# changhaonan/A3VLM

Measured on AMD Instinct MI355X. Metric: image-text samples/sec (train) + articulation-decode tok/s, higher is better.
Workload: dtype bf16

## Files before the change

### a3vlm_amd/csrc/a3v_attn_bwd.hip

```cpp
#include "a3v_common.h"
#include <type_traits>

namespace {

struct BwdArgs {
  const bf16_t* q; const bf16_t* k; const bf16_t* v; const bf16_t* dout;
  const float* lse; const float* D;
  bf16_t* dq; bf16_t* dk; bf16_t* dv;
  bf16_t* dqkv; int64_t ld_qkv; const float* cos_sin; int rope_pos0;
  int64_t k_sb, k_sh, v_sb, v_ss, v_sh;
  int B, S, Sp, H, Hkv, causal;
  float scale;
  int group_q, group_kv;
#ifdef AB_STAMP
  unsigned long long* stamps;
#endif
};
#ifdef AB_STAMP
#define AB_ST(kern, it, k) do { if (stamps && (it) < 64) stamps[((kern) * 64 + (it)) * 8 + (k)] = __builtin_amdgcn_s_memtime(); } while (0)
#else
#define AB_ST(kern, it, k) do {} while (0)
#endif

template <int HD>
__device__ __forceinline__ int tile_swz(int row) {
  return (HD == 128) ? (((row & 3) << 2) | ((row >> 2) & 3)) : ((row >> 1) & 7);
}

__device__ __forceinline__ void buf_dma16(__amdgpu_buffer_rsrc_t rs, char* lds_dst, unsigned voff) {
  __builtin_amdgcn_raw_ptr_buffer_load_lds(rs, (__attribute__((address_space(3))) void*)lds_dst, 16, voff, 0, 0, 0);
}
__device__ __forceinline__ void buf_dma4(__amdgpu_buffer_rsrc_t rs, void* lds_dst, unsigned voff) {
  __builtin_amdgcn_raw_ptr_buffer_load_lds(rs, (__attribute__((address_space(3))) void*)lds_dst, 4, voff, 0, 0, 0);
}
template <int HD>
__device__ __forceinline__ unsigned dma_lane_offset0(int64_t row_stride, int tid) {
  constexpr int KCH = HD / 8;
  const int row = tid / KCH, pc = tid % KCH;
  return (unsigned)((row * row_stride + ((pc ^ tile_swz<HD>(row)) << 3)) * 2);
}
template <int HD>
__device__ __forceinline__ unsigned dma_step(int64_t row_stride) { return (unsigned)((256 / (HD / 8)) * row_stride * 2); }
template <int HD>
__device__ __forceinline__ void stage_rows_dma(const bf16_t* base, int64_t row_stride, int row0, int nrows, char* lds, unsigned voff0, int wave) {
  const int64_t left = ((int64_t)(nrows - 1 - row0) * row_stride + HD) * 2;
  const auto rs = __builtin_amdgcn_make_buffer_rsrc((void*)(base + (int64_t)row0 * row_stride), 0, (int)(left < 0x7fffffff ? left : 0x7fffffff), 0x00020000);
  const unsigned step = dma_step<HD>(row_stride);
#pragma unroll
  for (int i = 0; i < 64 * (HD / 8) / 256; ++i) buf_dma16(rs, lds + (wave * 64 + i * 256) * 16, voff0 + i * step);
}

template <int HD>
__device__ __forceinline__ int frag_rows_base(int ql, int hh) { return ql * (HD * 2) + ((hh ^ tile_swz<HD>(ql)) << 4); }
template <int HD>
__device__ __forceinline__ bf16x8 frag_rows(const char* lds, int fbase, int tb, int ks) {
  return *reinterpret_cast<const bf16x8*>(lds + tb * 32 * (HD * 2) + (fbase ^ (ks << 5)));
}

typedef __attribute__((ext_vector_type(4))) short s16x4_t;
struct TrBase { int lo, hi; };
template <int HD>
__device__ __forceinline__ TrBase tr_bases(int lane) {
  const int hh = lane >> 5, ql = lane & 31, i = lane & 15;
  const int chunk16 = 2 * (ql >> 4) + ((i & 3) >> 1);
  const int row0 = 4 * hh + (i >> 2), row1 = row0 + 8;
  TrBase b;
  b.lo = row0 * (HD * 2) + ((chunk16 ^ tile_swz<HD>(row0)) << 4) + (i & 1) * 8;
  b.hi = row1 * (HD * 2) + ((chunk16 ^ tile_swz<HD>(row1)) << 4) + (i & 1) * 8;
  return b;
}
template <int HD>
__device__ __forceinline__ bf16x8 frag_rows_tr(const char* lds, TrBase tb0, int db, int tb, int c) {
  const char* blk = lds + (32 * tb + 16 * c) * (HD * 2);
  const s16x4_t lo = __builtin_amdgcn_ds_read_tr16_b64_v4i16((s16x4_t __attribute__((address_space(3)))*)(blk + (tb0.lo ^ (db << 6))));
  const s16x4_t hi = __builtin_amdgcn_ds_read_tr16_b64_v4i16((s16x4_t __attribute__((address_space(3)))*)(blk + (tb0.hi ^ (db << 6))));
  bf16x8 f;
  const short v[8] = {lo[0], lo[1], lo[2], lo[3], hi[0], hi[1], hi[2], hi[3]};
  __builtin_memcpy(&f, v, 16);
  return f;
}

template <int HD>
__device__ __forceinline__ void store_patch_rows(const char* patch, bf16_t* base, int64_t ld, int row0, int nrows, int lane) {
  constexpr int ROWB = HD * 2, NPAIR = HD / 8, RPI = 64 / NPAIR;
  asm volatile("s_waitcnt lgkmcnt(0)" ::: "memory");
  const int pr = lane % NPAIR, rr = lane / NPAIR;
#pragma unroll
  for (int it = 0; it < 32 / RPI; ++it) {
    const int r = it * RPI + rr;
    const bf16x8 v = *reinterpret_cast<const bf16x8*>(patch + r * ROWB + ((pr ^ (r & (NPAIR - 1))) << 4));
    if (row0 + r < nrows) *reinterpret_cast<bf16x8*>(base + (int64_t)(row0 + r) * ld + pr * 8) = v;
  }
}

template <int HD, bool PACKED>
__device__ __forceinline__ void store_grad_rows(const BwdArgs& p, f32x16 (&acc)[HD / 32], bf16_t* plain, int64_t prow, int slot, int pos,
                                                bool rotate, int hh) {
  if constexpr (!PACKED) {
    bf16_t* O = plain;
#pragma unroll
    for (int d = 0; d < HD / 32; ++d)
#pragma unroll
      for (int g4 = 0; g4 < 4; ++g4) {
        bf16x4 ov;
#pragma unroll
        for (int e = 0; e < 4; ++e) ov[e] = f2bf(acc[d][g4 * 4 + e]);
        *reinterpret_cast<bf16x4*>(O + d * 32 + g4 * 8 + hh * 4) = ov;
      }
    return;
  }
  bf16_t* O = p.dqkv + prow * p.ld_qkv + (int64_t)slot * HD;
  const float* CS = p.cos_sin + (int64_t)pos * HD;
#pragma unroll
  for (int d = 0; d < HD / 32; ++d)
#pragma unroll
    for (int g4 = 0; g4 < 4; ++g4) {
      const int dc = d * 32 + g4 * 8 + hh * 4;
      float v0 = acc[d][g4 * 4 + 0], v1 = acc[d][g4 * 4 + 1], v2 = acc[d][g4 * 4 + 2], v3 = acc[d][g4 * 4 + 3];
      if (rotate) {
        const f32x4 cs = *reinterpret_cast<const f32x4*>(CS + dc);
        const float a0 = v0 * cs[0] + v1 * cs[1], a1 = -v0 * cs[1] + v1 * cs[0];
        const float a2 = v2 * cs[2] + v3 * cs[3], a3 = -v2 * cs[3] + v3 * cs[2];
        v0 = a0; v1 = a1; v2 = a2; v3 = a3;
      }
      bf16x4 ov;
      ov[0] = f2bf(v0); ov[1] = f2bf(v1); ov[2] = f2bf(v2); ov[3] = f2bf(v3);
      *reinterpret_cast<bf16x4*>(O + dc) = ov;
    }
}

__device__ __forceinline__ void xcd_head_tile(int nt, int& head_slot, int& t, int G = 1) {
  const int total = gridDim.x, id = blockIdx.x;
  const int xcd = id & 7, q = total >> 3, r = total & 7;
  const int vb = (xcd < r ? xcd * (q + 1) : r * (q + 1) + (xcd - r) * q) + (id >> 3);
  if (G > 1) {
    const int per = G * nt, grp = vb / per, rr = vb - grp * per;
    head_slot = grp * G + rr % G;
    t = rr / G;
    return;
  }
  head_slot = vb / nt;
  t = vb - head_slot * nt;
}

template <int HD, bool PACKED>
__global__ __launch_bounds__(256, 2) void attn_bwd_dq_kernel(BwdArgs p) {
  constexpr int TILE = 64 * HD * 2;
  __shared__ __attribute__((aligned(1024))) char lds[4 * TILE];
  const int tid = threadIdx.x, lane = tid & 63, wave = __builtin_amdgcn_readfirstlane(tid >> 6);
  const int nqt = (p.S + 127) / 128;
  int head_slot, ti;
  xcd_head_tile(nqt, head_slot, ti, p.group_q);
  const int qt = nqt - 1 - ti, b = head_slot / p.H, h = head_slot - b * p.H;
  const int hk = h / (p.H / p.Hkv);
  const int ql = lane & 31, hh = lane >> 5;
  const int qrow = qt * 128 + wave * 32 + ql;
  const int qc = qrow < p.S ? qrow : p.S - 1;
  const bf16_t* Q = p.q + (((int64_t)b * p.S + qc) * p.H + h) * HD;
  const bf16_t* DO = p.dout + (((int64_t)b * p.S + qc) * p.H + h) * HD;
  const bf16_t* K = p.k + b * p.k_sb + hk * p.k_sh;
  const bf16_t* V = p.v + b * p.v_sb + hk * p.v_sh;
  bf16x8 qf[HD / 16], dof[HD / 16];
#pragma unroll
  for (int ks = 0; ks < HD / 16; ++ks) {
    qf[ks] = *reinterpret_cast<const bf16x8*>(Q + ks * 16 + hh * 8);
    dof[ks] = *reinterpret_cast<const bf16x8*>(DO + ks * 16 + hh * 8);
  }
  const float lse2 = p.lse[((int64_t)b * p.H + h) * p.S + qc] * 1.4426950408889634f;
  const float sl2 = p.scale * 1.4426950408889634f;
// ... 189 lines not shown
#pragma unroll
        for (int r = 0; r < 16; ++r) { s[r] = 0.f; dp[r] = 0.f; }
#pragma unroll
        for (int ks = 0; ks < HD / 16; ++ks) {
          s = __builtin_amdgcn_mfma_f32_32x32x16_bf16(frag_rows<HD>(Qs, fbase, tb, ks), kf[ks], s, 0, 0, 0);
          if (WHICH == 1) dp = __builtin_amdgcn_mfma_f32_32x32x16_bf16(frag_rows<HD>(T1, fbase, tb, ks), vf[ks], dp, 0, 0, 0);
        }
#pragma unroll
        for (int g4 = 0; g4 < 4; ++g4) {
          const int qb = tb * 32 + 8 * g4 + 4 * hh;
          f32x4 l4 = *reinterpret_cast<const f32x4*>(lse_s + qb);
#pragma unroll
          for (int e = 0; e < 4; ++e) l4[e] *= 1.4426950408889634f;
          f32x4 d4 = {0.f, 0.f, 0.f, 0.f};
          if (WHICH == 1) d4 = *reinterpret_cast<const f32x4*>(D_s + qb);
          if (interior) {
#pragma unroll
            for (int e = 0; e < 4; ++e) {
              const int r = g4 * 4 + e;
              const float pr = __builtin_amdgcn_exp2f(fmaf(s[r], sl2, -l4[e]));
              bf[tb][r >> 3][r & 7] = WHICH == 0 ? f2bf(pr) : f2bf(pr * (dp[r] - d4[e]));
            }
          } else {
#pragma unroll
            for (int e = 0; e < 4; ++e) {
              const int r = g4 * 4 + e;
              const int qg = q0 + qb + e;
              const bool ok = (qg < p.S) && (kvrow < p.S) && (!p.causal || kvrow <= qg);
              const float ev = __builtin_amdgcn_exp2f(fmaf(s[r], sl2, -l4[e]));
              const float val = WHICH == 0 ? ev : ev * (dp[r] - d4[e]);
              bf[tb][r >> 3][r & 7] = f2bf(ok ? val : 0.f);
            }
          }
        }
      }
      AB_ST(1 + WHICH, it, 4);
      const char* At = WHICH == 0 ? T1 : Qs;
#pragma unroll
      for (int tb = 0; tb < 2; ++tb)
#pragma unroll
        for (int c = 0; c < 2; ++c)
#pragma unroll
          for (int d = 0; d < HD / 32; ++d)
            acc[d] = __builtin_amdgcn_mfma_f32_32x32x16_bf16(frag_rows_tr<HD>(At, trb, d, tb, c), bf[tb][c], acc[d], 0, 0, 0);
      AB_ST(1 + WHICH, it, 5);
    }
  };
  {
    int it = 0;
    for (; it + 1 < total; it += 2) {
      body(it, std::integral_constant<int, 0>{});
      body(it + 1, std::integral_constant<int, 1>{});
    }
    if (it < total) body(it, std::integral_constant<int, 0>{});
  }
  if (WHICH == 1) {
#pragma unroll
    for (int d = 0; d < HD / 32; ++d)
#pragma unroll
      for (int r = 0; r < 16; ++r) acc[d][r] *= p.scale;
  }
  if (kvrow < p.S) {
    if constexpr (!PACKED) {
      bf16_t* O = (WHICH == 0 ? p.dv : p.dk) + (((int64_t)b * p.Hkv + hk) * p.S + kvrow) * HD;
#pragma unroll
      for (int d = 0; d < HD / 32; ++d)
#pragma unroll
        for (int g4 = 0; g4 < 4; ++g4) {
          bf16x4 a;
#pragma unroll
          for (int e = 0; e < 4; ++e) a[e] = f2bf(acc[d][g4 * 4 + e]);
          *reinterpret_cast<bf16x4*>(O + d * 32 + g4 * 8 + hh * 4) = a;
        }
    }
  }
  if constexpr (PACKED) {
    __syncthreads();
    char* patch = lds + wave * (32 * HD * 2);
    char* wrow = patch + kl * (HD * 2);
    const int wx = (kl & (HD / 8 - 1)) << 1;
    const float* CS = p.cos_sin + (int64_t)(p.rope_pos0 + kc) * HD;
#pragma unroll
    for (int d = 0; d < HD / 32; ++d)
#pragma unroll
      for (int g4 = 0; g4 < 4; ++g4) {
        const int dc = d * 32 + g4 * 8 + hh * 4;
        float v0 = acc[d][g4 * 4 + 0], v1 = acc[d][g4 * 4 + 1], v2 = acc[d][g4 * 4 + 2], v3 = acc[d][g4 * 4 + 3];
        if (WHICH == 1) {
          const f32x4 cs = *reinterpret_cast<const f32x4*>(CS + dc);
          const float a0 = v0 * cs[0] + v1 * cs[1], a1 = -v0 * cs[1] + v1 * cs[0];
          const float a2 = v2 * cs[2] + v3 * cs[3], a3 = -v2 * cs[3] + v3 * cs[2];
          v0 = a0; v1 = a1; v2 = a2; v3 = a3;
        }
        bf16x4 ov;
        ov[0] = f2bf(v0); ov[1] = f2bf(v1); ov[2] = f2bf(v2); ov[3] = f2bf(v3);
        *reinterpret_cast<bf16x4*>(wrow + (((d * 8 + g4 * 2 + hh) ^ wx) << 3)) = ov;
      }
    store_patch_rows<HD>(patch, p.dqkv + (int64_t)b * p.S * p.ld_qkv + (int64_t)(WHICH == 0 ? p.H + p.Hkv + hk : p.H + hk) * HD, p.ld_qkv,
                         kt_ * 128 + wave * 32, p.S, lane);
  }
}

template <int I, int N, typename F>
__device__ __forceinline__ void sfor(F&& f) {
  if constexpr (I < N) { f(std::integral_constant<int, I>{}); sfor<I + 1, N>(f); }
}
#define A3V_A16(b) "a" #b
#define A3V_CL8(p) "a" #p "0", "a" #p "1", "a" #p "2", "a" #p "3", "a" #p "4", "a" #p "5", "a" #p "6", "a" #p "7", "a" #p "8", "a" #p "9"
#define A3V_AGPR_0_255 "a0", "a1", "a2", "a3", "a4", "a5", "a6", "a7", "a8", "a9", A3V_CL8(1), A3V_CL8(2), A3V_CL8(3), A3V_CL8(4), A3V_CL8(5), A3V_CL8(6), \
    A3V_CL8(7), A3V_CL8(8), A3V_CL8(9), A3V_CL8(10), A3V_CL8(11), A3V_CL8(12), A3V_CL8(13), A3V_CL8(14), A3V_CL8(15), A3V_CL8(16), A3V_CL8(17), \
    A3V_CL8(18), A3V_CL8(19), A3V_CL8(20), A3V_CL8(21), A3V_CL8(22), A3V_CL8(23), A3V_CL8(24), "a250", "a251", "a252", "a253", "a254", "a255"
template <int ACC>
__device__ __forceinline__ void mfma_vv(const bf16x8& a, const bf16x8& b) {
  asm volatile("s_nop 1\n\tv_mfma_f32_32x32x16_bf16 a[%c2:%c3], %0, %1, a[%c2:%c3]" ::"v"(a), "v"(b), "i"(ACC), "i"(ACC + 15) : A3V_AGPR_0_255);
}
template <int ACC, int BR, bool ZERO>
__device__ __forceinline__ void mfma_va(const bf16x8& a) {
  if constexpr (ZERO)
    asm volatile("v_mfma_f32_32x32x16_bf16 a[%c1:%c2], %0, a[%c3:%c4], 0" ::"v"(a), "i"(ACC), "i"(ACC + 15), "i"(BR), "i"(BR + 3) : A3V_AGPR_0_255);
  else
    asm volatile("v_mfma_f32_32x32x16_bf16 a[%c1:%c2], %0, a[%c3:%c4], a[%c1:%c2]" ::"v"(a), "i"(ACC), "i"(ACC + 15), "i"(BR), "i"(BR + 3) : A3V_AGPR_0_255);
}
template <int BR, bool ZERO>
__device__ __forceinline__ void mfma_va_v(f32x16& acc, const bf16x8& a) {
  if constexpr (ZERO)
    asm volatile("v_mfma_f32_32x32x16_bf16 %0, %1, a[%c2:%c3], 0" : "=&v"(acc) : "v"(a), "i"(BR), "i"(BR + 3) : A3V_AGPR_0_255);
  else
    asm volatile("v_mfma_f32_32x32x16_bf16 %0, %1, a[%c2:%c3], %0" : "+v"(acc) : "v"(a), "i"(BR), "i"(BR + 3) : A3V_AGPR_0_255);
}
template <int R>
__device__ __forceinline__ float agpr_read() {
  float v;
  asm volatile("v_accvgpr_read_b32 %0, a[%c1]" : "=v"(v) : "i"(R) : A3V_AGPR_0_255);
  return v;
}
template <int R>
__device__ __forceinline__ void agpr_write(unsigned v) {
  asm volatile("v_accvgpr_write_b32 a[%c1], %0" ::"v"(v), "i"(R) : A3V_AGPR_0_255);
}
template <int R0>
__device__ __forceinline__ f32x16 agpr_read16() {
  f32x16 v;
  sfor<0, 16>([&](auto i) { v[decltype(i)::value] = agpr_read<R0 + decltype(i)::value>(); });
  return v;
}

typedef __attribute__((ext_vector_type(4))) int i32x4_t;
__device__ __forceinline__ void dma16_asm(i32x4_t rs, unsigned lds_addr, unsigned voff) {
  asm volatile("s_nop 4\n\ts_mov_b32 m0, %0\n\ts_nop 0\n\tbuffer_load_dwordx4 %1, %2, 0 offen lds" ::"s"(lds_addr), "v"(voff), "s"(rs) : "memory", A3V_AGPR_0_255);
}
__device__ __forceinline__ void dma4_asm(i32x4_t rs, unsigned lds_addr, unsigned voff) {
  asm volatile("s_nop 4\n\ts_mov_b32 m0, %0\n\ts_nop 0\n\tbuffer_load_dword %1, %2, 0 offen lds" ::"s"(lds_addr), "v"(voff), "s"(rs) : "memory", A3V_AGPR_0_255);
}
__device__ __forceinline__ i32x4_t make_rsrc(const void* base, int bytes) {
  const uint64_t a = (uint64_t)base;
  i32x4_t r;
  r[0] = __builtin_amdgcn_readfirstlane((int)(unsigned)a);
  r[1] = __builtin_amdgcn_readfirstlane((int)(unsigned)(a >> 32) & 0xffff);
  r[2] = __builtin_amdgcn_readfirstlane(bytes);
  r[3] = 0x00020000;
  return r;
}
template <int HD>
__device__ __forceinline__ void stage_rows_dma_asm(const bf16_t* base, int64_t row_stride, int row0, int nrows, unsigned lds_addr, unsigned voff0, int wave) {
  int64_t left = ((int64_t)(nrows - 1 - row0) * row_stride + HD) * 2;
  if (left < 0) left = 0;
  const i32x4_t rs = make_rsrc(base + (int64_t)(left ? row0 : 0) * row_stride, (int)(left < 0x7fffffff ? left : 0x7fffffff));
  const unsigned step = dma_step<HD>(row_stride);
#pragma unroll
  for (int i = 0; i < 64 * (HD / 8) / 256; ++i) dma16_asm(rs, lds_addr + (wave * 64 + i * 256) * 16, voff0 + i * step);
}
typedef __attribute__((ext_vector_type(8))) short s16x8_t;
template <int HD>
__device__ __forceinline__ bf16x8 frag_rows_tr2(const char* lds, TrBase tb0, int db, int tb, int c) {
  const char* blk = lds + (32 * tb + 16 * c) * (HD * 2);
  const s16x4_t lo = __builtin_amdgcn_ds_read_tr16_b64_v4i16((s16x4_t __attribute__((address_space(3)))*)(blk + (tb0.lo ^ (db << 6))));
  const s16x4_t hi = __builtin_amdgcn_ds_read_tr16_b64_v4i16((s16x4_t __attribute__((address_space(3)))*)(blk + (tb0.hi ^ (db << 6))));
  const s16x8_t v = __builtin_shufflevector(lo, hi, 0, 1, 2, 3, 4, 5, 6, 7);
  return __builtin_bit_cast(bf16x8, v);
}

template <int HD, bool PACKED>
__global__ __launch_bounds__(256, 1) void attn_bwd_dkv2_kernel(BwdArgs p) {
  constexpr int TILE = 64 * HD * 2;
  constexpr int BUFB = 2 * TILE + 1024;
  constexpr int NKS = HD / 16, NDB = HD / 32;
  constexpr int RV = 0, RK = 64, RKF = 128, RVF = 160, RS = 192, RDP = 208;
  constexpr int NB = 4;
  __shared__ __attribute__((aligned(1024))) char lds[NB * BUFB + 4096];
  const int tid = threadIdx.x, lane = tid & 63, wave = __builtin_amdgcn_readfirstlane(tid >> 6);
#ifdef AB_STAMP
  unsigned long long* tl = (p.stamps && tid == 0) ? p.stamps + 4096 + 8 * blockIdx.x : nullptr;
  if (tl) { tl[0] = __builtin_amdgcn_s_memrealtime(); tl[4] = __builtin_amdgcn_s_getreg(0x0004 | (0 << 6) | (31 << 11)); tl[5] = __builtin_amdgcn_s_getreg(20 | (0 << 6) | (31 << 11)); }
#endif
  int head_slot, kt_;
  xcd_head_tile((p.S + 127) / 128, head_slot, kt_, p.group_kv);
  const int b = head_slot / p.Hkv, hk = head_slot - b * p.Hkv;
  const int nrep = p.H / p.Hkv;
  const int kl = lane & 31, hh = lane >> 5;
  const int kv_lo = kt_ * 128 + wave * 32;
  const int kvrow = kv_lo + kl;
  const int kc = kvrow < p.S ? kvrow : p.S - 1;
  asm volatile("" ::: A3V_AGPR_0_255);
  const float sl2 = p.scale * 1.4426950408889634f;
  const int q_begin = p.causal ? kt_ * 2 : 0;
  const int n_qt = (p.S + 63) / 64;
  const int n_it = n_qt - q_begin, total = nrep * n_it;
  const unsigned qoff = dma_lane_offset0<HD>((int64_t)p.H * HD, tid);
  const int fbase = frag_rows_base<HD>(kl, hh);
  const TrBase trb = tr_bases<HD>(lane);

  int rep_n = 0, qi_n = 0, buf_n = 0;
  const unsigned lds0 = (unsigned)(size_t)((__attribute__((address_space(3))) char*)lds);
  constexpr int PP = HD / 16;
  i32x4_t rsQ, rsO, rsX;
  unsigned dmaQ, dmaO, dmaX, dma_step_i, voffX;
  const unsigned qstep = dma_step<HD>((int64_t)p.H * HD);
  const int64_t rstride = (int64_t)p.H * HD;
  const uint64_t pairB = (uint64_t)(64 * rstride * 2);
  uint64_t aQ = (uint64_t)(p.q + ((int64_t)b * p.S * p.H + hk * nrep) * HD + (int64_t)q_begin * 64 * rstride);
  uint64_t aO = (uint64_t)(p.dout + ((int64_t)b * p.S * p.H + hk * nrep) * HD + (int64_t)q_begin * 64 * rstride);
  uint64_t aL = (uint64_t)(p.lse + ((int64_t)b * p.H + hk * nrep) * p.S + q_begin * 64);
  uint64_t aD = (uint64_t)(p.D + ((int64_t)b * p.S + q_begin * 64) * p.H + hk * nrep);
  int64_t leftQ = ((int64_t)(p.S - 1 - q_begin * 64) * rstride + HD) * 2;
  int rowsL = p.S - q_begin * 64;
  voffX = (wave == 1) ? lane * p.H * 4 : lane * 4;
  auto mk = [&](uint64_t a, int bytes) __attribute__((always_inline)) {
    i32x4_t r;
    r[0] = (int)(unsigned)a; r[1] = (int)(unsigned)(a >> 32) & 0xffff; r[2] = bytes; r[3] = 0x00020000;
    return r;
  };
  auto prep_issue = [&](bool real) __attribute__((always_inline)) {
    const unsigned buf = lds0 + buf_n * BUFB, patch = lds0 + NB * BUFB + wave * 1024;
    const int nb = real ? (int)(leftQ < 0x7fffffff ? leftQ : 0x7fffffff) : 0;
    rsQ = mk(aQ, nb);
    rsO = mk(aO, nb);
    dmaQ = real ? buf + wave * 1024 : patch;
    dmaO = real ? buf + TILE + wave * 1024 : patch;
    dma_step_i = real ? 4096u : 0u;
    if (wave == 0) { rsX = mk(aL, real ? rowsL * 4 : 0); dmaX = real ? buf + 2 * TILE : patch; }
    else if (wave == 1) { rsX = mk(aD, real ? ((rowsL - 1) * p.H + 1) * 4 : 0); dmaX = real ? buf + 2 * TILE + 256 : patch; }
    else { rsX = mk(aL, 0); dmaX = patch; }
    if (real) {
      if (++buf_n == NB) buf_n = 0;
      if (++qi_n == n_it) {
        qi_n = 0; ++rep_n;
        const int64_t back = (int64_t)(n_it - 1) * 64;
        aQ += (uint64_t)(HD * 2) - (uint64_t)(back * rstride * 2); aO += (uint64_t)(HD * 2) - (uint64_t)(back * rstride * 2);
        aL += (uint64_t)((int64_t)p.S * 4) - (uint64_t)(back * 4); aD += 4 - (uint64_t)(back * p.H * 4);
        leftQ += back * rstride * 2; rowsL += (int)back;
      } else {
        aQ += pairB; aO += pairB; aL += 256; aD += (uint64_t)(64 * p.H * 4);
        leftQ -= (int64_t)pairB; rowsL -= 64;
      }
    }
  };
  auto piece = [&](auto i_) __attribute__((always_inline)) {
    constexpr int i = decltype(i_)::value;
    if constexpr (i < PP / 2) dma16_asm(rsQ, dmaQ + i * dma_step_i, qoff + i * qstep);
    else if constexpr (i < PP) dma16_asm(rsO, dmaO + (i - PP / 2) * dma_step_i, qoff + (i - PP / 2) * qstep);
    else dma4_asm(rsX, dmaX, voffX);
  };
  auto issue = [&](bool real) __attribute__((always_inline)) {
    prep_issue(real);
    sfor<0, PP + 1>([&](auto i_) { piece(i_); });
  };

  bf16x8 qa[NKS], da[NKS];
  auto fetch = [&](const char* buf, int tb) __attribute__((always_inline)) {
#pragma unroll
    for (int ks = 0; ks < NKS; ++ks) {
      qa[ks] = frag_rows<HD>(buf, fbase, tb, ks);
      da[ks] = frag_rows<HD>(buf + TILE, fbase, tb, ks);
    }
  };
  auto dead = [&](int qr0) { return qr0 >= p.S || (p.causal && qr0 + 31 < kv_lo); };
  auto interior = [&](int qr0) { return qr0 + 32 <= p.S && kv_lo + 31 < p.S && (!p.causal || qr0 >= kv_lo + 31); };

#ifdef AB_STAMP
  unsigned long long* stamps = (p.stamps && blockIdx.x == AB_STAMP && tid == 0) ? p.stamps : nullptr;
  int cur_it = 0;
#endif
  f32x16 dpv[2];
  auto step = [&](auto DA_, auto DBC_, auto MASK_, auto TBC_, const char* cb, int qr0, const char* fb, int tbf) __attribute__((always_inline)) {
    constexpr bool DA = decltype(DA_)::value, DBC = decltype(DBC_)::value, MASK = decltype(MASK_)::value;
    constexpr int tbc = decltype(TBC_)::value;
    constexpr int RSC = RS + 16 * tbc, RSN = RS + 16 * (1 - tbc);
    constexpr int EPK = 16 / NKS;
    bf16x8 trO[2][NDB], trQ[2][NDB], bP[2], bS[2];
    f32x4 l4[4], d4[4];
    float ex[EPK], dd[EPK];
    const float* sm = reinterpret_cast<const float*>(cb + 2 * TILE) + tbc * 32 + 4 * hh;
    if constexpr (DBC) {
      l4[0] = *reinterpret_cast<const f32x4*>(sm);
      d4[0] = *reinterpret_cast<const f32x4*>(sm + 64);
    }
    auto finish = [&](auto kp_) __attribute__((always_inline)) {
      constexpr int kp = decltype(kp_)::value;
#pragma unroll
      for (int j = 0; j < EPK; ++j) {
        const int r = kp * EPK + j;
        bP[r >> 3][r & 7] = f2bf(ex[j]);
        bS[r >> 3][r & 7] = f2bf(ex[j] * dd[j]);
      }
      u32x4 wP, wS;
      __builtin_memcpy(&wP, &bP[(kp * EPK) >> 3], 16);
      __builtin_memcpy(&wS, &bS[(kp * EPK) >> 3], 16);
      constexpr int w0 = ((kp * EPK) & 7) / 2;
      if constexpr (EPK == 2) asm volatile("" : "+v"(wP[w0]), "+v"(wS[w0]));
      else asm volatile("" : "+v"(wP[w0]), "+v"(wP[w0 + 1]), "+v"(wS[w0]), "+v"(wS[w0 + 1]));
      __builtin_memcpy(&bP[(kp * EPK) >> 3], &wP, 16);
      __builtin_memcpy(&bS[(kp * EPK) >> 3], &wS, 16);
    };
    sfor<0, NKS>([&](auto ks_) {
      constexpr int ks = decltype(ks_)::value;
      if constexpr (DA) mfma_va<RSN, RKF + 4 * ks, ks == 0>(qa[ks]);
      if constexpr (tbc == 0) piece(ks_);
      float en[EPK], dn[EPK];
      if constexpr (DBC) {
        constexpr int g4 = (ks * EPK) >> 2;
        sfor<0, EPK>([&](auto j_) {
          constexpr int j = decltype(j_)::value, r = ks * EPK + j, e = r & 3;
          const float sv = agpr_read<RSC + r>();
          const float dv = dpv[tbc][r];
          float a = fmaf(sv, sl2, l4[g4][e]);
          if constexpr (MASK) {
            const int qg = qr0 + 8 * g4 + 4 * hh + e;
            const bool ok = (qg < p.S) && (kvrow < p.S) && (!p.causal || kvrow <= qg);
            a = ok ? a : -INFINITY;
          }
          en[j] = __builtin_amdgcn_exp2f(a);
          dn[j] = dv - d4[g4][e];
        });
        if constexpr (EPK == 2) asm volatile("" : "+v"(en[0]), "+v"(en[1]), "+v"(dn[0]), "+v"(dn[1]));
        else asm volatile("" : "+v"(en[0]), "+v"(en[1]), "+v"(en[2]), "+v"(en[3]), "+v"(dn[0]), "+v"(dn[1]), "+v"(dn[2]), "+v"(dn[3]));
      }
      if constexpr (DA) mfma_va_v<RVF + 4 * ks, ks == 0>(dpv[1 - tbc], da[ks]);
      if constexpr (DBC) {
        if constexpr (ks > 0) finish(std::integral_constant<int, ks - 1>{});
#pragma unroll
        for (int j = 0; j < EPK; ++j) { ex[j] = en[j]; dd[j] = dn[j]; }
        if constexpr (ks < NDB) {
          trO[0][ks] = frag_rows_tr2<HD>(cb + TILE, trb, ks, tbc, 0);
          trQ[0][ks] = frag_rows_tr2<HD>(cb, trb, ks, tbc, 0);
        }
        constexpr int gn = ((ks * EPK) >> 2) + 1;
        if constexpr (((ks * EPK) & 3) == 0 && gn < 4) {
          l4[gn] = *reinterpret_cast<const f32x4*>(sm + 8 * gn);
          d4[gn] = *reinterpret_cast<const f32x4*>(sm + 64 + 8 * gn);
        }
        asm volatile("" ::: "memory");
      }
    });
    if constexpr (tbc == 0) piece(std::integral_constant<int, PP>{});
    if constexpr (DBC) finish(std::integral_constant<int, NKS - 1>{});
    asm volatile("" ::: "memory");
#ifdef AB_STAMP
    if (stamps && cur_it < 64) stamps[(64 + cur_it) * 8 + 6 + tbc] = __builtin_amdgcn_s_memtime();
#endif
    constexpr int FPD = NKS / NDB;
    sfor<0, NDB>([&](auto d_) {
      constexpr int d = decltype(d_)::value;
      if constexpr (DBC) {
        mfma_vv<RV + 16 * d>(trO[0][d], bP[0]);
        trO[1][d] = frag_rows_tr2<HD>(cb + TILE, trb, d, tbc, 1);
      }
      qa[d * FPD] = frag_rows<HD>(fb, fbase, tbf, d * FPD);
      asm volatile("" ::: "memory");
      if constexpr (DBC) {
        mfma_vv<RK + 16 * d>(trQ[0][d], bS[0]);
        trQ[1][d] = frag_rows_tr2<HD>(cb, trb, d, tbc, 1);
      }
      da[d * FPD] = frag_rows<HD>(fb + TILE, fbase, tbf, d * FPD);
      asm volatile("" ::: "memory");
    });
    sfor<0, NDB>([&](auto d_) {
      constexpr int d = decltype(d_)::value;
      if constexpr (DBC) mfma_vv<RV + 16 * d>(trO[1][d], bP[1]);
#pragma unroll
      for (int ks = d * FPD + 1; ks < (d + 1) * FPD; ++ks) qa[ks] = frag_rows<HD>(fb, fbase, tbf, ks);
      asm volatile("" ::: "memory");
      if constexpr (DBC) mfma_vv<RK + 16 * d>(trQ[1][d], bS[1]);
#pragma unroll
      for (int ks = d * FPD + 1; ks < (d + 1) * FPD; ++ks) da[ks] = frag_rows<HD>(fb + TILE, fbase, tbf, ks);
      asm volatile("" ::: "memory");
    });
    if constexpr (DA && !DBC) asm volatile("s_nop 15\n\ts_nop 15" ::: "memory", A3V_AGPR_0_255);
  };
  using T_ = std::true_type; using F_ = std::false_type;
  auto run = [&](bool lc, bool ln, bool mk, auto tbc, const char* cb, int qr0, const char* fb, int tbf) __attribute__((always_inline)) {
    if (lc) {
      if (mk) step(T_{}, T_{}, T_{}, tbc, cb, qr0, fb, tbf);
      else step(T_{}, T_{}, F_{}, tbc, cb, qr0, fb, tbf);
    } else if (ln) {
      step(T_{}, F_{}, F_{}, tbc, cb, qr0, fb, tbf);
    } else {
      step(F_{}, F_{}, F_{}, tbc, cb, qr0, fb, tbf);
    }
  };

  auto prescale_lse = [&](const char* buf) __attribute__((always_inline)) {
    if (wave == 3) {
      float* sm = const_cast<float*>(reinterpret_cast<const float*>(buf + 2 * TILE));
      sm[lane] = -1.4426950408889634f * sm[lane];
    }
  };
#ifdef AB_STAMP
#define AB_PE(k) do { if (stamps) stamps[2 * 64 * 8 + (k)] = __builtin_amdgcn_s_memtime(); } while (0)
#else
#define AB_PE(k) do {} while (0)
#endif
  AB_PE(0);
#ifdef AB_STAMP
  if (tl) tl[6] = __builtin_amdgcn_s_memrealtime();
#endif
  issue(true);
#ifdef AB_STAMP
  if (tl) tl[7] = __builtin_amdgcn_s_memrealtime();
#endif
  {
    const bf16_t* Kb = p.k + b * p.k_sb + hk * p.k_sh;
    const bf16_t* Vb = p.v + b * p.v_sb + hk * p.v_sh;
    const unsigned kvoffK = dma_lane_offset0<HD>(HD, tid), kvoffV = dma_lane_offset0<HD>(p.v_ss, tid);
#pragma unroll
    for (int t = 0; t < 2; ++t) {
      stage_rows_dma_asm<HD>(Kb, HD, kt_ * 128 + 64 * t, p.S, lds0 + 2 * BUFB + t * TILE, kvoffK, wave);
      stage_rows_dma_asm<HD>(Vb, p.v_ss, kt_ * 128 + 64 * t, p.S, lds0 + 3 * BUFB + t * TILE, kvoffV, wave);
    }
    sfor<0, 128>([&](auto i) { agpr_write<decltype(i)::value>(0u); });
    asm volatile("s_waitcnt vmcnt(0)" ::: "memory", A3V_AGPR_0_255);
    __syncthreads();
    prescale_lse(lds);
    const char* Kt = lds + 2 * BUFB + (wave >> 1) * TILE;
    const char* Vt = lds + 3 * BUFB + (wave >> 1) * TILE;
    sfor<0, NKS>([&](auto ks_) {
      constexpr int ks = decltype(ks_)::value;
      const bf16x8 kq = frag_rows<HD>(Kt, fbase, wave & 1, ks), vq = frag_rows<HD>(Vt, fbase, wave & 1, ks);
      u32x4 ku, vu;
      __builtin_memcpy(&ku, &kq, 16);
      __builtin_memcpy(&vu, &vq, 16);
      sfor<0, 4>([&](auto j) {
        agpr_write<RKF + 4 * ks + decltype(j)::value>(ku[decltype(j)::value]);
        agpr_write<RVF + 4 * ks + decltype(j)::value>(vu[decltype(j)::value]);
      });
    });
    __syncthreads();
  }
  AB_PE(1);
  AB_PE(2);
  issue(total > 1);
  AB_PE(3);
  fetch(lds, 0);
  prep_issue(total > 2);
  sfor<0, NKS>([&](auto ks_) {
    constexpr int ks = decltype(ks_)::value;
    mfma_va<RS, RKF + 4 * ks, ks == 0>(qa[ks]);
    piece(ks_);
    mfma_va_v<RVF + 4 * ks, ks == 0>(dpv[0], da[ks]);
  });
  piece(std::integral_constant<int, PP>{});
  asm volatile("s_nop 15\n\ts_nop 15" ::: "memory", A3V_AGPR_0_255);
  fetch(lds, 1);
  AB_PE(4);
  int qi_c = 0, buf_c = 0;
#ifdef AB_STAMP
  if (tl) tl[1] = __builtin_amdgcn_s_memrealtime();
#endif
  for (int it = 0; it < total; ++it) {
    const int q0 = (q_begin + qi_c) * 64;
    if (++qi_c == n_it) qi_c = 0;
    const int q0x = (q_begin + qi_c) * 64;
    const char* cb = lds + buf_c * BUFB;
    if (++buf_c == NB) buf_c = 0;
    const char* xb = lds + buf_c * BUFB;
    const bool more = it + 1 < total;
#ifdef AB_STAMP
    cur_it = it;
#endif
    AB_ST(1, it, 0);
    if constexpr (PP == 8) asm volatile("s_waitcnt vmcnt(9)" ::: "memory", A3V_AGPR_0_255); else asm volatile("s_waitcnt vmcnt(5)" ::: "memory", A3V_AGPR_0_255);
    AB_ST(1, it, 1);
    __syncthreads();
    AB_ST(1, it, 2);
    prep_issue(it + 3 < total);
    if (more) prescale_lse(xb);
    AB_ST(1, it, 3);
    const bool l0 = !dead(q0), l1 = !dead(q0 + 32), lx = more && !dead(q0x);
    run(l0, l1, !interior(q0), std::integral_constant<int, 0>{}, cb, q0, xb, 0);
    AB_ST(1, it, 4);
    run(l1, lx, !interior(q0 + 32), std::integral_constant<int, 1>{}, cb, q0 + 32, xb, 1);
    AB_ST(1, it, 5);
  }
#ifdef AB_STAMP
  if (tl) tl[2] = __builtin_amdgcn_s_memrealtime();
#endif
  asm volatile("s_nop 15\n\ts_nop 15" ::: "memory", A3V_AGPR_0_255);
  AB_PE(5);
  const float* CS = PACKED ? p.cos_sin + (int64_t)(p.rope_pos0 + kc) * HD : nullptr;
  f32x4 cs[NDB][4];
  if constexpr (PACKED) {
#pragma unroll
    for (int d = 0; d < NDB; ++d)
#pragma unroll
      for (int g4 = 0; g4 < 4; ++g4) cs[d][g4] = *reinterpret_cast<const f32x4*>(CS + d * 32 + g4 * 8 + hh * 4);
  }
  __syncthreads();
  AB_PE(6);
  char* patchV = lds + wave * (32 * HD * 2);
  char* patchK = lds + 4 * (32 * HD * 2) + wave * (32 * HD * 2);
  const int wx = (kl & (HD / 8 - 1)) << 1;
  sfor<0, NDB>([&](auto d_) {
    constexpr int d = decltype(d_)::value;
    const f32x16 av = agpr_read16<RV + 16 * d>();
#pragma unroll
    for (int g4 = 0; g4 < 4; ++g4) {
      bf16x4 ov;
#pragma unroll
      for (int e = 0; e < 4; ++e) ov[e] = f2bf(av[g4 * 4 + e]);
      *reinterpret_cast<bf16x4*>(patchV + kl * (HD * 2) + (((d * 8 + g4 * 2 + hh) ^ wx) << 3)) = ov;
    }
  });
  bf16_t* baseV = PACKED ? p.dqkv + (int64_t)b * p.S * p.ld_qkv + (int64_t)(p.H + p.Hkv + hk) * HD : p.dv + ((int64_t)b * p.Hkv + hk) * p.S * HD;
  bf16_t* baseK = PACKED ? p.dqkv + (int64_t)b * p.S * p.ld_qkv + (int64_t)(p.H + hk) * HD : p.dk + ((int64_t)b * p.Hkv + hk) * p.S * HD;
  const int64_t ldo = PACKED ? p.ld_qkv : HD;
  store_patch_rows<HD>(patchV, baseV, ldo, kv_lo, p.S, lane);
  AB_PE(7);
  sfor<0, NDB>([&](auto d_) {
    constexpr int d = decltype(d_)::value;
    f32x16 ak = agpr_read16<RK + 16 * d>();
#pragma unroll
    for (int r = 0; r < 16; ++r) ak[r] *= p.scale;
#pragma unroll
    for (int g4 = 0; g4 < 4; ++g4) {
      float v0 = ak[g4 * 4 + 0], v1 = ak[g4 * 4 + 1], v2 = ak[g4 * 4 + 2], v3 = ak[g4 * 4 + 3];
      bf16x4 ok;
      if constexpr (PACKED) {
        const f32x4 c4 = cs[d][g4];
        ok[0] = f2bf(v0 * c4[0] + v1 * c4[1]); ok[1] = f2bf(-v0 * c4[1] + v1 * c4[0]);
        ok[2] = f2bf(v2 * c4[2] + v3 * c4[3]); ok[3] = f2bf(-v2 * c4[3] + v3 * c4[2]);
      } else {
        ok[0] = f2bf(v0); ok[1] = f2bf(v1); ok[2] = f2bf(v2); ok[3] = f2bf(v3);
      }
      *reinterpret_cast<bf16x4*>(patchK + kl * (HD * 2) + (((d * 8 + g4 * 2 + hh) ^ wx) << 3)) = ok;
    }
  });
  store_patch_rows<HD>(patchK, baseK, ldo, kv_lo, p.S, lane);
  AB_PE(8);
#ifdef AB_STAMP
  if (tl) { asm volatile("s_waitcnt vmcnt(0)" ::: "memory"); tl[3] = __builtin_amdgcn_s_memrealtime(); }
#endif
}

}

extern "C" int a3v_transpose(const void* src, int64_t ld_src, int64_t bs_src, void* dst, int64_t ld_dst, int64_t bs_dst,
                             int R, int C, int Rpad, int batch, int dtype, void* stream);

extern "C" int64_t a3v_attention_bwd_workspace_bytes(int B, int S, int H, int Hkv, int hd) {
  (void)B; (void)S; (void)H; (void)Hkv; (void)hd;
  return 256;
}

#ifdef AB_STAMP
static unsigned long long* g_ab_stamps = nullptr;
extern "C" void a3v_debug_set_bwd_stamps(void* ptr) { g_ab_stamps = (unsigned long long*)ptr; }
#endif
static int attention_bwd_mfma_impl(const void* q, const void* k, int64_t k_sb, int64_t k_sh, const void* v, int64_t v_sb,
                                   int64_t v_ss, int64_t v_sh, const void* dout, const float* lse, const float* D, void* dq,
                                   void* dk, void* dv, void* dqkv, int64_t ld_qkv, const float* cos_sin, int rope_pos0, int B, int S, int H,
                                   int Hkv, int hd, int causal, void* stream) {
  if (hd != 64 && hd != 128) return A3V_ERR_ARG;
  if ((k_sb % 8) || (k_sh % 8) || (v_sb % 8) || (v_ss % 8) || (v_sh % 8)) return A3V_ERR_SHAPE;
  hipStream_t st = (hipStream_t)stream;
  const int Sp = (S + 63) / 64 * 64;
  BwdArgs p;
  p.q = (const bf16_t*)q; p.k = (const bf16_t*)k; p.v = (const bf16_t*)v; p.dout = (const bf16_t*)dout;
  p.lse = lse; p.D = D;
  p.dq = (bf16_t*)dq; p.dk = (bf16_t*)dk; p.dv = (bf16_t*)dv;
  p.dqkv = (bf16_t*)dqkv; p.ld_qkv = ld_qkv; p.cos_sin = cos_sin; p.rope_pos0 = rope_pos0;
  p.k_sb = k_sb; p.k_sh = k_sh; p.v_sb = v_sb; p.v_ss = v_ss; p.v_sh = v_sh;
  p.B = B; p.S = S; p.Sp = Sp; p.H = H; p.Hkv = Hkv; p.causal = causal;
  p.scale = 1.0f / sqrtf((float)hd);
#ifdef AB_STAMP
  p.stamps = g_ab_stamps;
#endif
  dim3 gq(((S + 127) / 128) * H * B), gk(((S + 127) / 128) * Hkv * B);
  auto group_of = [&](int heads, unsigned blocks) {
    if (!causal || (blocks & 7) || (heads & 7)) return 1;
    const int ge = A3V_ENV_INT("A3V_ATTN_HEAD_GROUP", 0);
    int want = 16;
    while (want > 1 && (int64_t)want * S * hd * 4 > (9 << 19)) want >>= 1;
    if (ge > 0) want = ge;
    int G = want < 1 ? 1 : want;
    while (G > 1 && (heads / 8) % G) G >>= 1;
    return G;
  };
  p.group_q = group_of(B * H, gq.x);
  p.group_kv = group_of(B * Hkv, gk.x);
  const int v2 = A3V_ENV_INT("A3V_ATTN_BWD_V2", 1);
#define A3V_BWD_LAUNCH(HDV, PK)                                                                  \
  do {                                                                                           \
    hipLaunchKernelGGL((attn_bwd_dq_kernel<HDV, PK>), gq, dim3(256), 0, st, p);                  \
    if (v2 & 1) {                                                                                \
      hipLaunchKernelGGL((attn_bwd_dkv2_kernel<HDV, PK>), gk, dim3(256), 0, st, p);              \
    } else {                                                                                     \
      hipLaunchKernelGGL((attn_bwd_dkv_kernel<HDV, 0, PK>), gk, dim3(256), 0, st, p);            \
      hipLaunchKernelGGL((attn_bwd_dkv_kernel<HDV, 1, PK>), gk, dim3(256), 0, st, p);            \
    }                                                                                            \
  } while (0)
  if (hd == 128) {
    if (dqkv) A3V_BWD_LAUNCH(128, true); else A3V_BWD_LAUNCH(128, false);
  } else {
    if (dqkv) A3V_BWD_LAUNCH(64, true); else A3V_BWD_LAUNCH(64, false);
  }
#undef A3V_BWD_LAUNCH
  A3V_LAUNCH_CHECK();
  return A3V_OK;
}

extern "C" int a3v_attention_bwd_mfma(const void* q, const void* k, int64_t k_sb, int64_t k_sh, const void* v, int64_t v_sb,
                                      int64_t v_ss, int64_t v_sh, const void* dout, const float* lse, const float* D, void* dq,
                                      void* dk, void* dv, void* workspace, int B, int S, int H, int Hkv, int hd, int causal,
                                      void* stream) {
  if (!workspace || !dq || !dk || !dv) return A3V_ERR_ARG;
  return attention_bwd_mfma_impl(q, k, k_sb, k_sh, v, v_sb, v_ss, v_sh, dout, lse, D, dq, dk, dv, nullptr, 0, nullptr, 0, B, S, H, Hkv, hd,
                                 causal, stream);
}

extern "C" __attribute__((visibility("hidden"))) int a3v_attention_bwd_mfma_packed(const void* q, const void* k, int64_t k_sb, int64_t k_sh, const void* v, int64_t v_sb,
                                             int64_t v_ss, int64_t v_sh, const void* dout, const float* lse, const float* D, void* dqkv,
                                             int64_t ld_qkv, const float* cos_sin, int rope_pos0, int B, int S, int H, int Hkv, int hd,
                                             int causal, void* stream) {
  if (!dqkv || !cos_sin || ld_qkv % 4 || rope_pos0 < 0) return A3V_ERR_ARG;
  return attention_bwd_mfma_impl(q, k, k_sb, k_sh, v, v_sb, v_ss, v_sh, dout, lse, D, nullptr, nullptr, nullptr, dqkv, ld_qkv, cos_sin, rope_pos0,
                                 B, S, H, Hkv, hd, causal, stream);
}
```

### a3vlm_amd/csrc/a3v_train.hip

```cpp
#include "a3v_common.h"

namespace {

template <typename T>
__global__ __launch_bounds__(256) void transpose_kernel(const T* __restrict__ src, int64_t lds_, int64_t bs_s,
                                                        T* __restrict__ dst, int64_t ldd, int64_t bs_d, int R, int C, int Rpad) {
  __shared__ T tile[64][64 + 2];
  const T* s = src + blockIdx.z * bs_s;
  T* d = dst + blockIdx.z * bs_d;
  const int r0 = blockIdx.y * 64, c0 = blockIdx.x * 64;
  const int tx = threadIdx.x & 63, ty = threadIdx.x >> 6;
  for (int i = ty; i < 64; i += 4) {
    const int r = r0 + i, c = c0 + tx;
    tile[i][tx] = (r < R && c < C) ? s[(int64_t)r * lds_ + c] : (T)0.f;
  }
  __syncthreads();
  for (int i = ty; i < 64; i += 4) {
    const int c = c0 + i, r = r0 + tx;
    if (c < C && r < Rpad) d[(int64_t)c * ldd + r] = tile[tx][i];
  }
}

__global__ __launch_bounds__(256) void transpose_bf16_vec_kernel(const bf16_t* __restrict__ src, int64_t lds_, int64_t bs_s,
                                                                 bf16_t* __restrict__ dst, int64_t ldd, int64_t bs_d, int R, int C, int Rpad,
// ... 701 lines not shown
    A3V_LAUNCH_CHECK();
    if (part) {
      hipLaunchKernelGGL(colsum_add_kernel, dim3((dim + 255) / 256, 16), dim3(256), 0, ST, dw_scratch, nb, dim, dw);
      A3V_LAUNCH_CHECK();
    }
    return A3V_OK;
  }
  constexpr int RPB = 16;
  dim3 g((rows + RPB - 1) / RPB);
  if (act_dtype == A3V_BF16) hipLaunchKernelGGL((rmsnorm_bwd_kernel<bf16_t, RPB, TS>), g, dim3(256), 0, ST, x, ldx, w, (const bf16_t*)dy, lddy, dh, lddh, dw, rows, dim, eps);
  else if (act_dtype == A3V_F32) hipLaunchKernelGGL((rmsnorm_bwd_kernel<float, RPB, TS>), g, dim3(256), 0, ST, x, ldx, w, (const float*)dy, lddy, dh, lddh, dw, rows, dim, eps);
  else return A3V_ERR_DTYPE;
  A3V_LAUNCH_CHECK();
  if (dh_bf) {
    if (sizeof(TS) != 4) return A3V_ERR_ARG;
    return a3v_cast(dh, lddh, A3V_F32, dh_bf, ld_bf, A3V_BF16, rows, dim, stream);
  }
  return A3V_OK;
}

extern "C" int a3v_rmsnorm_bwd(const float* x, int64_t ldx, const float* w, const void* dy, int64_t lddy, float* dh, int64_t lddh,
                               float* dw, float* dw_scratch, int rows, int dim, float eps, int act_dtype, void* stream) {
  return rmsnorm_bwd_impl<float>(x, ldx, w, dy, lddy, dh, lddh, dw, dw_scratch, rows, dim, eps, act_dtype, stream, nullptr, 0);
}

extern "C" int a3v_rmsnorm_bwd_cast(const float* x, int64_t ldx, const float* w, const void* dy, int64_t lddy, float* dh, int64_t lddh,
                                    float* dw, float* dw_scratch, int rows, int dim, float eps, int act_dtype, void* dh_bf16,
                                    int64_t ld_bf16, void* stream) {
  if (!dh_bf16 || (ld_bf16 & 3) || (reinterpret_cast<uintptr_t>(dh_bf16) & 7)) return A3V_ERR_ARG;
  return rmsnorm_bwd_impl<float>(x, ldx, w, dy, lddy, dh, lddh, dw, dw_scratch, rows, dim, eps, act_dtype, stream, (bf16_t*)dh_bf16, ld_bf16);
}

extern "C" int a3v_rmsnorm_bwd_bf16(const void* x, int64_t ldx, const float* w, const void* dy, int64_t lddy, void* dh, int64_t lddh,
                                    float* dw, float* dw_scratch, int rows, int dim, float eps, void* stream) {
  return rmsnorm_bwd_impl<bf16_t>((const bf16_t*)x, ldx, w, dy, lddy, (bf16_t*)dh, lddh, dw, dw_scratch, rows, dim, eps, A3V_BF16, stream, nullptr, 0);
}

static int layernorm_bwd_impl(const void* x, int64_t ldx, const float* w, const void* dy, int dy_dtype, int64_t lddy, const int32_t* row_map,
                              void* dx, int64_t lddx, float* dw, float* db, int rows, int dim, float eps, int act_dtype, void* stream) {
  if (!x || !w || !dy || !dx || !dw || !db || rows <= 0) return A3V_ERR_ARG;
  if (dim > 8192) return A3V_ERR_SHAPE;
  constexpr int RPB = 16;
  dim3 g((rows + RPB - 1) / RPB);
  if (dy_dtype == A3V_F32) {
    if (act_dtype == A3V_BF16) hipLaunchKernelGGL((layernorm_bwd_kernel<bf16_t, RPB, float>), g, dim3(256), 0, ST, (const bf16_t*)x, ldx, w, (const float*)dy, lddy, row_map, (bf16_t*)dx, lddx, dw, db, rows, dim, eps);
    else if (act_dtype == A3V_F32) hipLaunchKernelGGL((layernorm_bwd_kernel<float, RPB, float>), g, dim3(256), 0, ST, (const float*)x, ldx, w, (const float*)dy, lddy, row_map, (float*)dx, lddx, dw, db, rows, dim, eps);
    else return A3V_ERR_DTYPE;
  } else if (dy_dtype == A3V_BF16 && act_dtype == A3V_BF16) {
    hipLaunchKernelGGL((layernorm_bwd_kernel<bf16_t, RPB, bf16_t>), g, dim3(256), 0, ST, (const bf16_t*)x, ldx, w, (const bf16_t*)dy, lddy, row_map, (bf16_t*)dx, lddx, dw, db, rows, dim, eps);
  } else return A3V_ERR_DTYPE;
  A3V_LAUNCH_CHECK();
  return A3V_OK;
}

extern "C" int a3v_layernorm_bwd(const void* x, int64_t ldx, const float* w, const float* dy, int64_t lddy, const int32_t* row_map,
                                 void* dx, int64_t lddx, float* dw, float* db, int rows, int dim, float eps, int act_dtype, void* stream) {
  return layernorm_bwd_impl(x, ldx, w, dy, A3V_F32, lddy, row_map, dx, lddx, dw, db, rows, dim, eps, act_dtype, stream);
}

extern "C" int a3v_layernorm_bwd_bf16(const void* x, int64_t ldx, const float* w, const void* dy, int64_t lddy, const int32_t* row_map,
                                      void* dx, int64_t lddx, float* dw, float* db, int rows, int dim, float eps, void* stream) {
  return layernorm_bwd_impl(x, ldx, w, dy, A3V_BF16, lddy, row_map, dx, lddx, dw, db, rows, dim, eps, A3V_BF16, stream);
}

static int stream_nt() {
  return A3V_ENV_INT("A3V_STREAM_NT", 3) & 3;
}

extern "C" int a3v_swiglu_fwd(const void* gu, int64_t ldg, void* act, int64_t lda, int rows, int F, int interleaved, int dtype, void* stream) {
  const int inter = interleaved;
  if (!gu || !act || rows <= 0 || F <= 0 || (F % 16)) return A3V_ERR_ARG;
  if ((ldg % 8) || (lda % 8)) return A3V_ERR_SHAPE;
  int64_t n = (int64_t)rows * (F / 8);
  int blocks = (int)((n + 255) / 256 > 16384 ? 16384 : (n + 255) / 256);
  const int nt = stream_nt();
  if (dtype == A3V_BF16 && nt == 3) hipLaunchKernelGGL((swiglu_fwd_kernel<bf16_t, 3>), dim3(blocks), dim3(256), 0, ST, (const bf16_t*)gu, ldg, (bf16_t*)act, lda, rows, F, inter);
  else if (dtype == A3V_BF16 && nt == 1) hipLaunchKernelGGL((swiglu_fwd_kernel<bf16_t, 1>), dim3(blocks), dim3(256), 0, ST, (const bf16_t*)gu, ldg, (bf16_t*)act, lda, rows, F, inter);
  else if (dtype == A3V_BF16) hipLaunchKernelGGL(swiglu_fwd_kernel<bf16_t>, dim3(blocks), dim3(256), 0, ST, (const bf16_t*)gu, ldg, (bf16_t*)act, lda, rows, F, inter);
  else if (dtype == A3V_F32) hipLaunchKernelGGL(swiglu_fwd_kernel<float>, dim3(blocks), dim3(256), 0, ST, (const float*)gu, ldg, (float*)act, lda, rows, F, inter);
  else return A3V_ERR_DTYPE;
  A3V_LAUNCH_CHECK();
  return A3V_OK;
}

extern "C" int a3v_swiglu_bwd(const void* gu, int64_t ldg, const void* dact, int64_t lda, void* dgu, int64_t lddg, int rows, int F,
                              int interleaved, int dtype, void* stream) {
  const int inter = interleaved;
  if (!gu || !dact || !dgu || rows <= 0 || F <= 0 || (F % 16)) return A3V_ERR_ARG;
  if ((ldg % 8) || (lda % 8) || (lddg % 8)) return A3V_ERR_SHAPE;
  int64_t n = (int64_t)rows * (F / 8);
  int blocks = (int)((n + 255) / 256 > 16384 ? 16384 : (n + 255) / 256);
  const int nt = stream_nt();
  if (dtype == A3V_BF16 && nt == 3) hipLaunchKernelGGL((swiglu_bwd_kernel<bf16_t, 3>), dim3(blocks), dim3(256), 0, ST, (const bf16_t*)gu, ldg, (const bf16_t*)dact, lda, (bf16_t*)dgu, lddg, rows, F, inter);
  else if (dtype == A3V_BF16 && nt == 1) hipLaunchKernelGGL((swiglu_bwd_kernel<bf16_t, 1>), dim3(blocks), dim3(256), 0, ST, (const bf16_t*)gu, ldg, (const bf16_t*)dact, lda, (bf16_t*)dgu, lddg, rows, F, inter);
  else if (dtype == A3V_BF16) hipLaunchKernelGGL(swiglu_bwd_kernel<bf16_t>, dim3(blocks), dim3(256), 0, ST, (const bf16_t*)gu, ldg, (const bf16_t*)dact, lda, (bf16_t*)dgu, lddg, rows, F, inter);
  else if (dtype == A3V_F32) hipLaunchKernelGGL(swiglu_bwd_kernel<float>, dim3(blocks), dim3(256), 0, ST, (const float*)gu, ldg, (const float*)dact, lda, (float*)dgu, lddg, rows, F, inter);
  else return A3V_ERR_DTYPE;
  A3V_LAUNCH_CHECK();
  return A3V_OK;
}

extern "C" int a3v_rope_bwd_pack(const void* dq, const void* dk, const void* dv, void* dqkv, int64_t ld, const float* cos_sin,
                                 int B, int S, int H, int Hkv, int hd, int rope_pos0, int dtype, void* stream) {
  if (!dq || !dk || !dv || !dqkv || !cos_sin || B <= 0 || S <= 0 || (hd & 1)) return A3V_ERR_ARG;
  if (dtype == A3V_BF16) hipLaunchKernelGGL(rope_bwd_pack_kernel<bf16_t>, dim3(B * S), dim3(256), 0, ST, (const bf16_t*)dq, (const bf16_t*)dk, (const bf16_t*)dv, (bf16_t*)dqkv, ld, cos_sin, S, H, Hkv, hd, rope_pos0);
  else if (dtype == A3V_F32) hipLaunchKernelGGL(rope_bwd_pack_kernel<float>, dim3(B * S), dim3(256), 0, ST, (const float*)dq, (const float*)dk, (const float*)dv, (float*)dqkv, ld, cos_sin, S, H, Hkv, hd, rope_pos0);
  else return A3V_ERR_DTYPE;
  A3V_LAUNCH_CHECK();
  return A3V_OK;
}

extern "C" int a3v_attention_bwd_mfma(const void* q, const void* k, int64_t k_sb, int64_t k_sh, const void* v, int64_t v_sb,
                                      int64_t v_ss, int64_t v_sh, const void* dout, const float* lse, const float* D, void* dq,
                                      void* dk, void* dv, void* workspace, int B, int S, int H, int Hkv, int hd, int causal,
                                      void* stream);

extern "C" int a3v_attention_bwd(const void* q, const void* k, int64_t k_sb, int64_t k_sh, const void* v, int64_t v_sb, int64_t v_ss, int64_t v_sh,
                                 const void* out, const void* dout, const float* lse, float* D, void* dq, void* dk, void* dv,
                                 void* workspace, int B, int S, int H, int Hkv, int hd, int causal, int dtype, void* stream) {
  if (!q || !k || !v || !out || !dout || !lse || !D || !dq || !dk || !dv || B <= 0 || S <= 0) return A3V_ERR_ARG;
  if (hd > 256 || (H % Hkv)) return A3V_ERR_SHAPE;
  AttnBwdArgs p;
  p.q = q; p.k = k; p.v = v; p.dout = dout; p.lse = lse; p.D = D; p.dq = dq; p.dk = dk; p.dv = dv;
  p.v_sb = v_sb; p.v_ss = v_ss; p.v_sh = v_sh;
  p.k_sb = k_sb; p.k_sh = k_sh;
  p.B = B; p.S = S; p.H = H; p.Hkv = Hkv; p.hd = hd; p.causal = causal;
  p.scale = 1.0f / sqrtf((float)hd);
  if (dtype == A3V_BF16 && workspace && (hd == 64 || hd == 128)) {
    const int64_t rows = (int64_t)B * S * H;
    if (((reinterpret_cast<uintptr_t>(out) | reinterpret_cast<uintptr_t>(dout)) & 15) != 0)
      hipLaunchKernelGGL(attn_rowdot_kernel<bf16_t>, dim3(B * S * H), dim3(64), 0, ST, (const bf16_t*)out, (const bf16_t*)dout, D, hd);
    else if (hd == 128)
      hipLaunchKernelGGL(attn_rowdot_vec_kernel<128>, dim3((unsigned)((rows + 15) / 16)), dim3(256), 0, ST, (const bf16_t*)out, (const bf16_t*)dout, D, rows);
    else
      hipLaunchKernelGGL(attn_rowdot_vec_kernel<64>, dim3((unsigned)((rows + 31) / 32)), dim3(256), 0, ST, (const bf16_t*)out, (const bf16_t*)dout, D, rows);
    A3V_LAUNCH_CHECK();
    return a3v_attention_bwd_mfma(q, k, k_sb, k_sh, v, v_sb, v_ss, v_sh, dout, lse, D, dq, dk, dv, workspace, B, S, H, Hkv, hd, causal, stream);
  }
  if (dtype == A3V_BF16) {
    hipLaunchKernelGGL(attn_rowdot_kernel<bf16_t>, dim3(B * S * H), dim3(64), 0, ST, (const bf16_t*)out, (const bf16_t*)dout, D, hd);
    hipLaunchKernelGGL(attn_bwd_dq_generic<bf16_t>, dim3(S, H, B), dim3(64), 0, ST, p);
    hipLaunchKernelGGL(attn_bwd_dkv_generic<bf16_t>, dim3(S, Hkv, B), dim3(64), 0, ST, p);
  } else if (dtype == A3V_F32) {
    hipLaunchKernelGGL(attn_rowdot_kernel<float>, dim3(B * S * H), dim3(64), 0, ST, (const float*)out, (const float*)dout, D, hd);
    hipLaunchKernelGGL(attn_bwd_dq_generic<float>, dim3(S, H, B), dim3(64), 0, ST, p);
    hipLaunchKernelGGL(attn_bwd_dkv_generic<float>, dim3(S, Hkv, B), dim3(64), 0, ST, p);
  } else return A3V_ERR_DTYPE;
  A3V_LAUNCH_CHECK();
  return A3V_OK;
}

extern "C" __attribute__((visibility("hidden"))) int a3v_attention_bwd_mfma_packed(const void* q, const void* k, int64_t k_sb, int64_t k_sh, const void* v, int64_t v_sb,
                                             int64_t v_ss, int64_t v_sh, const void* dout, const float* lse, const float* D, void* dqkv,
                                             int64_t ld_qkv, const float* cos_sin, int rope_pos0, int B, int S, int H, int Hkv, int hd,
                                             int causal, void* stream);

extern "C" int a3v_attention_bwd_packed(const void* q, const void* k, int64_t k_sb, int64_t k_sh, const void* v, int64_t v_sb, int64_t v_ss,
                                        int64_t v_sh, const void* out, int64_t ld_out, const void* dout, const float* lse, float* D, void* dqkv,
                                        int64_t ld_qkv, const float* cos_sin, int rope_pos0, int B, int S, int H, int Hkv, int hd, int causal,
                                        int dtype, void* stream) {
  if (!q || !k || !v || !out || !dout || !lse || !D || !dqkv || !cos_sin || B <= 0 || S <= 0) return A3V_ERR_ARG;
  if (dtype != A3V_BF16) return A3V_ERR_DTYPE;
  if ((hd != 64 && hd != 128) || (H % Hkv) || ld_out < (int64_t)H * hd || ld_out % 8) return A3V_ERR_SHAPE;
  if (((reinterpret_cast<uintptr_t>(out) | reinterpret_cast<uintptr_t>(dout)) & 15) != 0) return A3V_ERR_SHAPE;
  const int64_t rows = (int64_t)B * S * H;
  if (hd == 128)
    hipLaunchKernelGGL(attn_rowdot_vec_kernel<128>, dim3((unsigned)((rows + 15) / 16)), dim3(256), 0, ST, (const bf16_t*)out, (const bf16_t*)dout, D, rows, H, ld_out);
  else
    hipLaunchKernelGGL(attn_rowdot_vec_kernel<64>, dim3((unsigned)((rows + 31) / 32)), dim3(256), 0, ST, (const bf16_t*)out, (const bf16_t*)dout, D, rows, H, ld_out);
  A3V_LAUNCH_CHECK();
  return a3v_attention_bwd_mfma_packed(q, k, k_sb, k_sh, v, v_sb, v_ss, v_sh, dout, lse, D, dqkv, ld_qkv, cos_sin, rope_pos0, B, S, H, Hkv, hd, causal,
                                       stream);
}

extern "C" int a3v_embed_bwd(const int64_t* tokens, int64_t ld_tok, const float* dh, float* dtable, int B, int T, int W, int dim,
                             int vocab, void* stream) {
  if (!tokens || !dh || !dtable || B <= 0 || T <= 0) return A3V_ERR_ARG;
  hipLaunchKernelGGL(embed_bwd_kernel<float>, dim3(B * (T + W)), dim3(256), 0, ST, tokens, ld_tok, dh, dtable, T, W, dim, vocab);
  A3V_LAUNCH_CHECK();
  return A3V_OK;
}

extern "C" int a3v_embed_bwd_bf16(const int64_t* tokens, int64_t ld_tok, const void* dh, float* dtable, int B, int T, int W, int dim,
                                  int vocab, void* stream) {
  if (!tokens || !dh || !dtable || B <= 0 || T <= 0) return A3V_ERR_ARG;
  hipLaunchKernelGGL(embed_bwd_kernel<bf16_t>, dim3(B * (T + W)), dim3(256), 0, ST, tokens, ld_tok, (const bf16_t*)dh, dtable, T, W, dim, vocab);
  A3V_LAUNCH_CHECK();
  return A3V_OK;
}

extern "C" int a3v_rows_sum(const void* src, int64_t ld, const int32_t* row_idx, int n_rows, int dim, float* out, int dtype, void* stream) {
  if (!src || !out || n_rows <= 0 || dim <= 0) return A3V_ERR_ARG;
  dim3 g((dim + 255) / 256, (n_rows + 63) / 64);
  if (dtype == A3V_BF16) hipLaunchKernelGGL(rows_sum_kernel<bf16_t>, g, dim3(256), 0, ST, (const bf16_t*)src, ld, row_idx, n_rows, dim, out);
  else if (dtype == A3V_F32) hipLaunchKernelGGL(rows_sum_kernel<float>, g, dim3(256), 0, ST, (const float*)src, ld, row_idx, n_rows, dim, out);
  else return A3V_ERR_DTYPE;
  A3V_LAUNCH_CHECK();
  return A3V_OK;
}

namespace {
template <int NT>
__global__ __launch_bounds__(256) void adamw_kernel(float* __restrict__ p, const float* __restrict__ g, float* __restrict__ m,
                                                    float* __restrict__ v, int64_t n4, int64_t n, float decay, float b1, float b2,
                                                    float step_size, float inv_bc2_sqrt, float eps, bf16_t* __restrict__ img,
                                                    const float* __restrict__ gscale) {
  const float gs = gscale ? *gscale : 1.f;
  if (!(gs >= 0.f)) return;
  const int64_t stride = (int64_t)gridDim.x * 256;
  for (int64_t i = (int64_t)blockIdx.x * 256 + threadIdx.x; i < n4; i += stride) {
    f32x4 pp = (NT & 1) ? __builtin_nontemporal_load(reinterpret_cast<const f32x4*>(p) + i) : reinterpret_cast<const f32x4*>(p)[i];
    f32x4 gg = (NT & 1) ? __builtin_nontemporal_load(reinterpret_cast<const f32x4*>(g) + i) : reinterpret_cast<const f32x4*>(g)[i];
#pragma unroll
    for (int e = 0; e < 4; ++e) gg[e] = __fmul_rn(gg[e], gs);
    f32x4 mm = (NT & 1) ? __builtin_nontemporal_load(reinterpret_cast<const f32x4*>(m) + i) : reinterpret_cast<const f32x4*>(m)[i];
    f32x4 vv = (NT & 1) ? __builtin_nontemporal_load(reinterpret_cast<const f32x4*>(v) + i) : reinterpret_cast<const f32x4*>(v)[i];
#pragma unroll
    for (int e = 0; e < 4; ++e) {
      pp[e] *= decay;
      mm[e] += (1.f - b1) * (gg[e] - mm[e]);
      vv[e] = b2 * vv[e] + (1.f - b2) * gg[e] * gg[e];
      pp[e] -= step_size * mm[e] / (sqrtf(vv[e]) * inv_bc2_sqrt + eps);
    }
    if (NT & 2) {
      __builtin_nontemporal_store(pp, reinterpret_cast<f32x4*>(p) + i);
      __builtin_nontemporal_store(mm, reinterpret_cast<f32x4*>(m) + i);
      __builtin_nontemporal_store(vv, reinterpret_cast<f32x4*>(v) + i);
    } else {
      reinterpret_cast<f32x4*>(p)[i] = pp;
      reinterpret_cast<f32x4*>(m)[i] = mm;
      reinterpret_cast<f32x4*>(v)[i] = vv;
    }
    if (img) {
      bf16x4 o;
#pragma unroll
      for (int e = 0; e < 4; ++e) o[e] = f2bf(pp[e]);
      if (NT & 2) __builtin_nontemporal_store(o, reinterpret_cast<bf16x4*>(img) + i);
      else reinterpret_cast<bf16x4*>(img)[i] = o;
    }
  }
  if (blockIdx.x == 0 && threadIdx.x < (int)(n - n4 * 4)) {
    const int64_t i = n4 * 4 + threadIdx.x;
    float pp = p[i] * decay;
    const float gg = __fmul_rn(g[i], gs);
    const float mm = m[i] + (1.f - b1) * (gg - m[i]);
    const float vv = b2 * v[i] + (1.f - b2) * gg * gg;
    pp -= step_size * mm / (sqrtf(vv) * inv_bc2_sqrt + eps);
    p[i] = pp; m[i] = mm; v[i] = vv;
    if (img) img[i] = f2bf(pp);
  }
}
}

extern "C" int a3v_adamw_scaled(float* param, const float* grad, float* exp_avg, float* exp_avg_sq, int64_t n, float lr, float beta1,
                                float beta2, float eps, float weight_decay, int64_t step, void* bf16_image, const float* grad_scale,
                                void* stream);
extern "C" int a3v_adamw(float* param, const float* grad, float* exp_avg, float* exp_avg_sq, int64_t n, float lr, float beta1,
                         float beta2, float eps, float weight_decay, int64_t step, void* bf16_image, void* stream) {
  return a3v_adamw_scaled(param, grad, exp_avg, exp_avg_sq, n, lr, beta1, beta2, eps, weight_decay, step, bf16_image, nullptr, stream);
}

extern "C" int a3v_adamw_scaled(float* param, const float* grad, float* exp_avg, float* exp_avg_sq, int64_t n, float lr, float beta1,
                                float beta2, float eps, float weight_decay, int64_t step, void* bf16_image, const float* grad_scale,
                                void* stream) {
  if (!param || !grad || !exp_avg || !exp_avg_sq || n <= 0 || step < 1) return A3V_ERR_ARG;
  if (((uintptr_t)param | (uintptr_t)grad | (uintptr_t)exp_avg | (uintptr_t)exp_avg_sq) & 15) return A3V_ERR_SHAPE;
  if (bf16_image && ((uintptr_t)bf16_image & 7)) return A3V_ERR_SHAPE;
  const double bc1 = 1.0 - pow((double)beta1, (double)step), bc2 = 1.0 - pow((double)beta2, (double)step);
  const float step_size = (float)((double)lr / bc1), inv_bc2_sqrt = (float)(1.0 / sqrt(bc2));
  const float decay = (float)(1.0 - (double)lr * (double)weight_decay);
  const int64_t n4 = n / 4;
  int64_t blocks = (n4 + 255) / 256;
  if (blocks > 256 * 16) blocks = 256 * 16;
  if (blocks < 1) blocks = 1;
  const int nt = A3V_ENV_INT("A3V_ADAMW_NT", 3);
#define A3V_ADAMW_LAUNCH(V) hipLaunchKernelGGL(adamw_kernel<V>, dim3((unsigned)blocks), dim3(256), 0, (hipStream_t)stream, param, grad, exp_avg, exp_avg_sq, n4, n, decay, \
                     beta1, beta2, step_size, inv_bc2_sqrt, eps, (bf16_t*)bf16_image, grad_scale)
  switch (nt & 3) {
    case 1: A3V_ADAMW_LAUNCH(1); break;
    case 2: A3V_ADAMW_LAUNCH(2); break;
    case 3: A3V_ADAMW_LAUNCH(3); break;
    default: A3V_ADAMW_LAUNCH(0); break;
  }
#undef A3V_ADAMW_LAUNCH
  A3V_LAUNCH_CHECK();
  return A3V_OK;
}

namespace {
template <int TR>
__global__ __launch_bounds__(256) void adamw_tile_t_kernel(float* __restrict__ p, const float* __restrict__ g, float* __restrict__ m,
                                                           float* __restrict__ v, int rows, int cols, float decay, float b1, float b2,
                                                           float step_size, float inv_bc2_sqrt, float eps, bf16_t* __restrict__ img,
                                                           bf16_t* __restrict__ imgt, int64_t ldt, const float* __restrict__ gscale) {
  const float gs = gscale ? *gscale : 1.f;
  if (!(gs >= 0.f)) return;
  constexpr int PITCH = TR + 2;
  __shared__ bf16_t patch2[2][64 * PITCH];
  int flip = 0;
  const int tid = threadIdx.x, tr = tid >> 4, tc = tid & 15;
  const int tiles_c = cols >> 6, ntiles = (rows / TR) * tiles_c;
  for (int t = blockIdx.x; t < ntiles; t += gridDim.x) {
    const int r0 = (t / tiles_c) * TR, c0 = (t % tiles_c) << 6;
    bf16_t* patch = patch2[flip];
    flip ^= 1;
#pragma unroll
    for (int ps = 0; ps < TR / 16; ++ps) {
      const int r = ps * 16 + tr;
      const int64_t i = ((int64_t)(r0 + r) * cols + c0 + tc * 4) >> 2;
      f32x4 pp = __builtin_nontemporal_load(reinterpret_cast<const f32x4*>(p) + i);
      f32x4 gg = __builtin_nontemporal_load(reinterpret_cast<const f32x4*>(g) + i);
#pragma unroll
      for (int e = 0; e < 4; ++e) gg[e] = __fmul_rn(gg[e], gs);
      f32x4 mm = __builtin_nontemporal_load(reinterpret_cast<const f32x4*>(m) + i);
      f32x4 vv = __builtin_nontemporal_load(reinterpret_cast<const f32x4*>(v) + i);
#pragma unroll
      for (int e = 0; e < 4; ++e) {
        pp[e] *= decay;
        mm[e] += (1.f - b1) * (gg[e] - mm[e]);
        vv[e] = b2 * vv[e] + (1.f - b2) * gg[e] * gg[e];
        pp[e] -= step_size * mm[e] / (sqrtf(vv[e]) * inv_bc2_sqrt + eps);
      }
      __builtin_nontemporal_store(pp, reinterpret_cast<f32x4*>(p) + i);
      __builtin_nontemporal_store(mm, reinterpret_cast<f32x4*>(m) + i);
      __builtin_nontemporal_store(vv, reinterpret_cast<f32x4*>(v) + i);
// ... 174 lines not shown
```

### a3vlm_amd/lib.py

```python
from __future__ import annotations

import ctypes
import os
from ctypes import c_float, c_int, c_int64, c_void_p

_HERE = os.path.dirname(os.path.abspath(__file__))
LIB_PATH = os.environ.get("A3V_LIB_PATH") or os.path.join(_HERE, "liba3vlm_hip.so")

BF16, F32 = 0, 1
EPI_NONE, EPI_BIAS, EPI_GELU, EPI_QUICKGELU, EPI_RESIDUAL, EPI_SWIGLU, EPI_OUT_F32, EPI_RES_F32 = 0, 1, 2, 4, 8, 16, 32, 64
EPI_SWIGLU_BWD = 128

EPI_TILE_128, EPI_TILE_256, EPI_TILE_256PP = 1 << 16, 1 << 17, 1 << 18
EPI_TILE_192PP = 1 << 23

P, I, L, F = c_void_p, c_int, c_int64, c_float

SIGNATURES = {
    "a3v_version": (I, []),
    "a3v_reload_env": (I, []),
    "a3v_gemm_nt": (I, [P, L, P, L, P, L, I, I, I, P, P, L, I, I, P]),
    "a3v_gemm_qkv_rope": (I, [P, L, P, L, I, P, L, P, P, P, L, P, L, P, I, I, I, I, I, I, I, I, P]),
    "a3v_gemm_nt_fp8": (I, [P, L, P, P, L, P, P, L, I, I, I, P, P, L, I, P]),
    "a3v_gemm_qkv_rope_fp8": (I, [P, L, P, P, L, P, I, P, L, P, P, P, I, I, I, I, I, I, I, I, P]),
    "a3v_quantize_rows_fp8": (I, [P, L, P, F, P, L, P, I, I, I, P]),
    "a3v_gemm_tn_splitk": (I, [P, L, P, L, P, I, I, I, I, P]),
    "a3v_attention_bwd_packed": (I, [P, P, L, L, P, L, L, L, P, L, P, P, P, P, L, P, I, I, I, I, I, I, I, I, P]),
    "a3v_lora_refresh": (I, [P, P, I, I, I, P, L, P, L, P, L, P, L, I, I, P]),
    "a3v_adamw": (I, [P, P, P, P, L, F, F, F, F, F, L, P, P]),
    "a3v_adamw_scaled": (I, [P, P, P, P, L, F, F, F, F, F, L, P, P, P]),
    "a3v_adamw_scaled_t": (I, [P, P, P, P, I, I, F, F, F, F, F, L, P, P, L, P, P]),
    "a3v_gemm_tn_strip": (I, [P, L, P, L, P, I, I, I, I, P]),
    "a3v_lora_gb_scatter": (I, [P, L, I, I, P, P, P, P]),
    "a3v_adamw_multi": (I, [P, I, L, F, F, F, F, F, L, P, P]),
    "a3v_scale_cast": (I, [P, I, P, I, L, F, P]),
    "a3v_sumsq_partials": (I, [P, L, P, P]),
    "a3v_grad_bucket_allreduce": (I, [P, P, L, P, I, P]),
    "a3v_grad_bucket_reduce_scatter": (I, [P, P, L, P, P, P, I, P]),
    "a3v_param_shard_all_gather": (I, [P, P, P, L, P]),
    "a3v_rccl_comm_count": (I, [P]),
    "a3v_rccl_available": (I, []),
    "a3v_gemm_nn": (I, [P, L, P, L, P, L, I, I, I, P, L, I, P]),
    "a3v_gemm_tn": (I, [P, L, P, L, P, L, I, I, I, P, L, I, P]),
    "a3v_gemm_tn_sumsq": (I, [P, L, P, L, P, L, I, I, I, P, L, I, P, L, P]),
    "a3v_gemm_tn_sumsq_slots": (L, [I, I]),
    "a3v_gemm_set_workspace": (I, [P, L]),
    "a3v_gemm_set_workspace_for": (I, [P, P, L]),
    "a3v_gemm_nt_splitk": (I, [P, L, P, L, P, I, I, I, I, P]),
    "a3v_splitk_reduce": (I, [P, I, I, I, P, L, I, I, P]),
    "a3v_gemm_skinny_split": (I, [I, I, I]),
    "a3v_gemm_skinny_ws_bytes": (L, [I, I, I]),
    "a3v_gemm_skinny_fp8": (I, [P, L, P, L, P, P, L, I, I, I, P, L, I, P, P]),
    "a3v_quantize_nf4_ws_bytes": (L, [I, I]),
    "a3v_quantize_nf4": (I, [P, I, I, P, P, P, P]),
    "a3v_dequantize_nf4": (I, [P, P, P, L, I, I, P]),
    "a3v_gemm_skinny_nf4": (I, [P, L, P, L, P, P, L, I, I, I, P, L, I, P, P]),
    "a3v_gemm_skinny": (I, [P, L, P, L, P, L, I, I, I, P, L, I, P, P]),
    "a3v_rmsnorm": (I, [P, L, P, P, L, I, I, F, I, I, I, P]),
    "a3v_layernorm": (I, [P, L, P, P, P, L, P, I, I, F, I, I, I, P]),
    "a3v_rope_kvcache": (I, [P, L, P, L, P, P, P, I, I, I, I, I, I, I, I, I, P]),
    "a3v_vt_pack": (I, [P, L, P, I, I, I, I, I, I, P]),
    "a3v_attention_scratch_floats": (L, [I, I, I, I]),
    "a3v_attention": (I, [P, P, P, P, I, I, I, I, I, I, ctypes.POINTER(c_int64), I, P, I, P]),
    "a3v_embed_assemble": (I, [P, L, P, P, I, I, I, I, I, I, I, P]),
    "a3v_fill_rows": (I, [P, P, L, P, I, I, I, I, P]),
    "a3v_patch_im2col": (I, [P, P, I, I, I, I, I, I, I, P]),
    "a3v_split_views": (I, [P, P, I, I, I, I, P]),
    "a3v_vit_embed": (I, [P, P, P, P, I, I, I, I, P]),
    "a3v_argmax": (I, [P, L, P, I, I, P]),
    "a3v_sample_top_p": (I, [P, L, I, I, F, F, P, P, P]),
    "a3v_preprocess_image": (I, [P, I, I, I, I, I, P, P, P, I, P, P, I, I, P, P, I, P, P, P]),
    "a3v_preprocess_batch": (I, [P, I, P, I, P, L, P, L, I, P, P, P]),
    "a3v_generate_step": (I, [P, L, P, I, I, P, L, P, L, I, P, P, I, P, P, P, P]),
    "a3v_count_valid": (I, [P, I, P, P]),
    "a3v_cross_entropy": (I, [P, L, P, P, P, L, P, F, I, I, I, P]),
    "a3v_attention_lse": (I, [P, P, P, P, P, I, I, I, I, I, I, ctypes.POINTER(c_int64), I, I, P]),
    "a3v_transpose": (I, [P, L, L, P, L, L, I, I, I, I, I, P]),
    "a3v_rmsnorm_bwd_scratch_floats": (L, [I, I]),
    "a3v_rmsnorm_bwd": (I, [P, L, P, P, L, P, L, P, P, I, I, F, I, P]),
    "a3v_rmsnorm_bwd_cast": (I, [P, L, P, P, L, P, L, P, P, I, I, F, I, P, L, P]),
    "a3v_rmsnorm_bwd_bf16": (I, [P, L, P, P, L, P, L, P, P, I, I, F, P]),
    "a3v_layernorm_bwd_bf16": (I, [P, L, P, P, L, P, P, L, P, P, I, I, F, P]),
    "a3v_embed_bwd_bf16": (I, [P, L, P, P, I, I, I, I, I, P]),
    "a3v_layernorm_bwd": (I, [P, L, P, P, L, P, P, L, P, P, I, I, F, I, P]),
    "a3v_swiglu_fwd": (I, [P, L, P, L, I, I, I, I, P]),
    "a3v_swiglu_bwd": (I, [P, L, P, L, P, L, I, I, I, I, P]),
    "a3v_cast": (I, [P, L, I, P, L, I, I, I, P]),
    "a3v_add2d": (I, [P, L, P, L, I, I, I, P]),
    "a3v_rope_bwd_pack": (I, [P, P, P, P, L, P, I, I, I, I, I, I, I, P]),
    "a3v_attention_bwd": (I, [P, P, L, L, P, L, L, L, P, P, P, P, P, P, P, P, I, I, I, I, I, I, I, P]),
    "a3v_attention_bwd_workspace_bytes": (L, [I, I, I, I, I]),
    "a3v_attention_bwd_mfma": (I, [P, P, L, L, P, L, L, L, P, P, P, P, P, P, P, I, I, I, I, I, I, P]),
    "a3v_embed_bwd": (I, [P, L, P, P, I, I, I, I, I, P]),
    "a3v_rows_sum": (I, [P, L, P, I, I, P, I, P]),
}

class LlamaLayer(ctypes.Structure):
    _fields_ = [(n, c_void_p) for n in ("attn_norm_w", "wqkv", "wo", "ffn_norm_w", "w13", "w2", "k_cache", "vt_cache",
                                        "wqkv_q", "wqkv_s", "wo_q", "wo_s", "w13_q", "w13_s", "w2_q", "w2_s",
                                        "wqkv_n4", "wqkv_n4s", "wo_n4", "wo_n4s", "w13_n4", "w13_n4s", "w2_n4", "w2_n4s")]


class ImageDesc(ctypes.Structure):
    _fields_ = [("src", c_void_p), ("coeffs", c_void_p), ("bounds", c_void_p), ("H", c_int), ("W", c_int), ("side", c_int), ("pad_x", c_int),
                ("pad_y", c_int), ("ksize", c_int)]


SIGNATURES["a3v_llama_decode_step"] = (I, [ctypes.POINTER(LlamaLayer), I, P, P, P, P, P, P, P, P, I, I, I, I, I, I, I, I, F, P])
SIGNATURES["a3v_llama_decode_step_form"] = (I, [I, I, I, I, I, I, I])

_lib = None


def load() -> ctypes.CDLL:
    global _lib
    if _lib is not None:
        return _lib
    if not os.path.isfile(LIB_PATH):
        raise RuntimeError(
            f"{LIB_PATH} not found: the HIP extension is not built. Run "
            "`python -c 'import __graft_entry__ as g; g.build()'` (or `make -C a3vlm_amd/csrc`). "
            "a3vlm_amd has no non-HIP fallback.")
    import torch
    lib = ctypes.CDLL(LIB_PATH)
    for name, (res, args) in SIGNATURES.items():
        fn = getattr(lib, name)
        fn.restype = res
        fn.argtypes = args
    _lib = lib
    return lib


class env:

    def __init__(self, **kw):
        self.kw = {k: str(v) for k, v in kw.items()}
        self.old = {}

    def __enter__(self):
        for k, v in self.kw.items():
            self.old[k] = os.environ.get(k)
            os.environ[k] = v
        load().a3v_reload_env()
        return self

    def __exit__(self, *exc):
        for k, v in self.old.items():
            if v is None:
                os.environ.pop(k, None)
            else:
                os.environ[k] = v
        load().a3v_reload_env()
        return False


class A3VError(RuntimeError):
    pass


_ERR = {-1: "A3V_ERR_SHAPE (unsupported size/alignment)", -2: "A3V_ERR_DTYPE", -3: "A3V_ERR_ARG"}


def check(rc: int, what: str) -> None:
    if rc != 0:
        raise A3VError(f"{what} failed: {_ERR.get(rc, f'hipError_t {rc}')}")
```

### a3vlm_amd/ops.py

```python
from __future__ import annotations

import ctypes
from typing import Optional

import torch

from . import lib as _l
from .lib import BF16, F32, EPI_BIAS, EPI_GELU, EPI_QUICKGELU, EPI_RESIDUAL, EPI_SWIGLU, EPI_OUT_F32, EPI_RES_F32, EPI_SWIGLU_BWD

_DT = {torch.bfloat16: BF16, torch.float32: F32}


def dt(t: torch.Tensor) -> int:
    try:
        return _DT[t.dtype]
    except KeyError:
        raise TypeError(f"a3vlm_amd supports bf16/fp32 tensors, got {t.dtype}")


def _p(t: Optional[torch.Tensor]):
    return None if t is None else t.data_ptr()


def _stream() -> int:
# ... 351 lines not shown
    _dev(logits, u, out)
    assert logits.dtype == torch.float32 and logits.stride(1) == 1 and u.dtype == torch.float32 and out.dtype == torch.int64
    B, V = logits.shape
    assert u.numel() >= B and out.numel() >= B and u.is_contiguous() and out.is_contiguous()
    rc = _l.load().a3v_sample_top_p(_p(logits), logits.stride(0), B, V, float(temperature), float(top_p), _p(u), _p(out), _stream())
    _l.check(rc, "a3v_sample_top_p")
    return out


def argmax(logits, out):
    _dev(logits, out)
    assert logits.dtype == torch.float32 and out.dtype == torch.int64
    B, V = logits.shape
    rc = _l.load().a3v_argmax(_p(logits), logits.stride(0), _p(out), B, V, _stream())
    _l.check(rc, "a3v_argmax")
    return out


def count_valid(labels, n_valid):
    _dev(labels, n_valid)
    rc = _l.load().a3v_count_valid(_p(labels), labels.numel(), _p(n_valid), _stream())
    _l.check(rc, "a3v_count_valid")


def cross_entropy(logits, labels, row_loss, dlogits=None, n_valid=None, grad_scale: float = 1.0):
    _dev(logits, labels, row_loss, dlogits, n_valid)
    rows, V = logits.shape
    rc = _l.load().a3v_cross_entropy(_p(logits), logits.stride(0), _p(labels), _p(row_loss), _p(dlogits),
                                     dlogits.stride(0) if dlogits is not None else 0, _p(n_valid), grad_scale,
                                     rows, V, dt(logits), _stream())
    _l.check(rc, "a3v_cross_entropy")


def attention_lse(q, k, vt, out, lse, B, Sq, Sk, H, Hkv, hd, strides, causal: bool):
    _dev(q, k, vt, out, lse)
    rc = _l.load().a3v_attention_lse(_p(q), _p(k), _p(vt), _p(out), _p(lse), B, Sq, Sk, H, Hkv, hd, _Strides(*strides),
                                     1 if causal else 0, dt(q), _stream())
    _l.check(rc, "a3v_attention_lse")


def transpose(src, dst, R, C, Rpad, batch=1, bs_src=0, bs_dst=0):
    _dev(src, dst)
    rc = _l.load().a3v_transpose(_p(src), src.stride(-2), bs_src, _p(dst), dst.stride(-2), bs_dst, R, C, Rpad, batch,
                                 dt(src), _stream())
    _l.check(rc, "a3v_transpose")
    return dst


def cast(src, dst):
    _dev(src, dst)
    rows, cols = src.shape
    rc = _l.load().a3v_cast(_p(src), src.stride(0), dt(src), _p(dst), dst.stride(0), dt(dst), rows, cols, _stream())
    _l.check(rc, "a3v_cast")
    return dst


def scale_cast(src, dst, scale: float = 1.0):
    _dev(src, dst)
    assert src.is_contiguous() and dst.is_contiguous() and src.numel() == dst.numel()
    rc = _l.load().a3v_scale_cast(_p(src), dt(src), _p(dst), dt(dst), src.numel(), float(scale), _stream())
    _l.check(rc, "a3v_scale_cast")
    return dst


SUMSQ_SLOTS = 1024


def sumsq_partials(x: torch.Tensor, out: torch.Tensor) -> torch.Tensor:
    _dev(x, out)
    assert x.dtype == torch.float32 and out.dtype == torch.float32 and out.numel() >= SUMSQ_SLOTS and x.is_contiguous() and out.is_contiguous()
    rc = _l.load().a3v_sumsq_partials(_p(x), x.numel(), _p(out), _stream())
    _l.check(rc, "a3v_sumsq_partials")
    return out


def add2d(dst, src):
    _dev(dst, src)
    assert dst.dtype == src.dtype and dst.shape == src.shape
    rows, cols = dst.shape
    rc = _l.load().a3v_add2d(_p(dst), dst.stride(0), _p(src), src.stride(0), rows, cols, dt(dst), _stream())
    _l.check(rc, "a3v_add2d")
    return dst


_rb_scratch = {}


def rmsnorm_bwd(x, w, dy, dh, dw, eps, dh_lowp=None):
    _dev(x, w, dy, dh, dw, dh_lowp)
    assert w.dtype == torch.float32 and x.dtype == dh.dtype and x.dtype in (torch.float32, torch.bfloat16)
    rows, dim = x.shape
    scratch = None
    if dw is not None:
        need = int(_l.load().a3v_rmsnorm_bwd_scratch_floats(rows, dim))
        scratch = _rb_scratch.get(x.device)
        if scratch is None or scratch.numel() < need:
            scratch = torch.empty(need, dtype=torch.float32, device=x.device)
            _rb_scratch[x.device] = scratch
    if x.dtype == torch.bfloat16:
        assert dh_lowp is None and dy.dtype == torch.bfloat16
        rc = _l.load().a3v_rmsnorm_bwd_bf16(_p(x), x.stride(0), _p(w), _p(dy), dy.stride(0), _p(dh), dh.stride(0), _p(dw), _p(scratch), rows,
                                            dim, eps, _stream())
        _l.check(rc, "a3v_rmsnorm_bwd_bf16")
        return
    if dh_lowp is not None:
        assert dh_lowp.dtype == torch.bfloat16 and dh_lowp.shape == dh.shape
        rc = _l.load().a3v_rmsnorm_bwd_cast(_p(x), x.stride(0), _p(w), _p(dy), dy.stride(0), _p(dh), dh.stride(0), _p(dw), _p(scratch), rows,
                                            dim, eps, dt(dy), _p(dh_lowp), dh_lowp.stride(0), _stream())
        _l.check(rc, "a3v_rmsnorm_bwd_cast")
        return
    rc = _l.load().a3v_rmsnorm_bwd(_p(x), x.stride(0), _p(w), _p(dy), dy.stride(0), _p(dh), dh.stride(0), _p(dw), _p(scratch), rows, dim,
                                   eps, dt(dy), _stream())
    _l.check(rc, "a3v_rmsnorm_bwd")


def layernorm_bwd(x, w, dy, row_map, dx, dw, db, eps=1e-5):
    _dev(x, w, dy, row_map, dx, dw, db)
    rows, dim = x.shape
    if dy.dtype == torch.bfloat16:
        rc = _l.load().a3v_layernorm_bwd_bf16(_p(x), x.stride(0), _p(w), _p(dy), dy.stride(0), _p(row_map), _p(dx), dx.stride(0),
                                              _p(dw), _p(db), rows, dim, eps, _stream())
        _l.check(rc, "a3v_layernorm_bwd_bf16")
        return
    rc = _l.load().a3v_layernorm_bwd(_p(x), x.stride(0), _p(w), _p(dy), dy.stride(0), _p(row_map), _p(dx), dx.stride(0),
                                     _p(dw), _p(db), rows, dim, eps, dt(x), _stream())
    _l.check(rc, "a3v_layernorm_bwd")


def swiglu_fwd(gu, act, F, interleaved: bool):
    _dev(gu, act)
    rc = _l.load().a3v_swiglu_fwd(_p(gu), gu.stride(0), _p(act), act.stride(0), gu.shape[0], F, 1 if interleaved else 0,
                                  dt(gu), _stream())
    _l.check(rc, "a3v_swiglu_fwd")


def swiglu_bwd(gu, dact, dgu, F, interleaved: bool):
    _dev(gu, dact, dgu)
    rc = _l.load().a3v_swiglu_bwd(_p(gu), gu.stride(0), _p(dact), dact.stride(0), _p(dgu), dgu.stride(0), gu.shape[0], F,
                                  1 if interleaved else 0, dt(gu), _stream())
    _l.check(rc, "a3v_swiglu_bwd")


def rope_bwd_pack(dq, dk, dv, dqkv, cos_sin, B, S, H, Hkv, hd, rope_pos0=0):
    _dev(dq, dk, dv, dqkv, cos_sin)
    rc = _l.load().a3v_rope_bwd_pack(_p(dq), _p(dk), _p(dv), _p(dqkv), dqkv.stride(0), _p(cos_sin), B, S, H, Hkv, hd,
                                     rope_pos0, dt(dq), _stream())
    _l.check(rc, "a3v_rope_bwd_pack")


def attention_bwd_workspace_bytes(B, S, H, Hkv, hd) -> int:
    return _l.load().a3v_attention_bwd_workspace_bytes(B, S, H, Hkv, hd)


def attention_bwd(q, k, k_sb, k_sh, v, v_sb, v_ss, v_sh, out, dout, lse, D, dq, dk, dv, B, S, H, Hkv, hd, causal: bool,
                  workspace=None):
    _dev(q, k, v, out, dout, lse, D, dq, dk, dv, workspace)
    rc = _l.load().a3v_attention_bwd(_p(q), _p(k), k_sb, k_sh, _p(v), v_sb, v_ss, v_sh, _p(out), _p(dout), _p(lse), _p(D),
                                     _p(dq), _p(dk), _p(dv), _p(workspace), B, S, H, Hkv, hd, 1 if causal else 0, dt(q), _stream())
    _l.check(rc, "a3v_attention_bwd")


def attention_bwd_packed(q, k, k_sb, k_sh, v, v_sb, v_ss, v_sh, out, dout, lse, D, dqkv, cos_sin, B, S, H, Hkv, hd, causal: bool,
                         rope_pos0: int = 0):
    _dev(q, k, v, out, dout, lse, D, dqkv, cos_sin)
    ld_out = out.stride(-2) if out.dim() == 2 else out.stride(1)
    rc = _l.load().a3v_attention_bwd_packed(_p(q), _p(k), k_sb, k_sh, _p(v), v_sb, v_ss, v_sh, _p(out), ld_out, _p(dout), _p(lse), _p(D),
                                            _p(dqkv), dqkv.stride(0), _p(cos_sin), rope_pos0, B, S, H, Hkv, hd, 1 if causal else 0,
                                            dt(q), _stream())
    _l.check(rc, "a3v_attention_bwd_packed")


def embed_bwd(tokens, dh, dtable, B, T, W, dim):
    _dev(tokens, dh, dtable)
    assert dh.is_contiguous()
    fn = _l.load().a3v_embed_bwd_bf16 if dh.dtype == torch.bfloat16 else _l.load().a3v_embed_bwd
    rc = fn(_p(tokens), tokens.stride(0), _p(dh), _p(dtable), B, T, W, dim, dtable.shape[0], _stream())
    _l.check(rc, "a3v_embed_bwd")


def rows_sum(src, row_idx, n_rows, out):
    _dev(src, row_idx, out)
    rc = _l.load().a3v_rows_sum(_p(src), src.stride(0), _p(row_idx), n_rows, src.shape[1], _p(out), dt(src), _stream())
    _l.check(rc, "a3v_rows_sum")


def lora_gb_scatter(gbt, r: int, views, row0s):
    import ctypes
    _dev(gbt, *views)
    n = len(views)
    assert gbt.dtype == torch.float32 and gbt.stride(1) == 1 and all(v.dtype == torch.float32 and v.is_contiguous() and v.shape[1] == r for v in views)
    dst = (ctypes.c_void_p * n)(*[v.data_ptr() for v in views])
    r0 = (ctypes.c_int * n)(*[int(x) for x in row0s])
    nj = (ctypes.c_int * n)(*[int(v.shape[0]) for v in views])
    rc = _l.load().a3v_lora_gb_scatter(_p(gbt), gbt.stride(0), int(r), n, ctypes.cast(dst, ctypes.c_void_p), ctypes.cast(r0, ctypes.c_void_p),
                                       ctypes.cast(nj, ctypes.c_void_p), _stream())
    _l.check(rc, "a3v_lora_gb_scatter")


def lora_refresh(wa, wb, A, At, B, Bt, col0: int, row0: int):
    _dev(wa, wb, A, At, B, Bt)
    assert wa.dtype == torch.float32 and wb.dtype == torch.float32 and wa.is_contiguous() and wb.is_contiguous()
    assert all(t.dtype == torch.bfloat16 and t.stride(1) == 1 for t in (A, At, B, Bt))
    r, in_f = wa.shape
    nj = wb.shape[0]
    assert wb.shape[1] == r and col0 + r <= A.shape[0] and in_f <= A.shape[1] and row0 + nj <= B.shape[0]
    rc = _l.load().a3v_lora_refresh(_p(wa), _p(wb), r, in_f, nj, _p(A), A.stride(0), _p(At), At.stride(0), _p(B), B.stride(0), _p(Bt),
                                    Bt.stride(0), col0, row0, _stream())
    _l.check(rc, "a3v_lora_refresh")
```

### a3vlm_amd/train.py

```python
from __future__ import annotations

import os

from typing import Callable, Dict, List, Optional, Tuple

import torch

from . import ops
from .util import install_param_epoch_hook, optimizer_steps, param_state_key


def _pad64(n: int) -> int:
    return (n + 63) // 64 * 64


def skinny_slices(M: int, N: int, K: int, cus: int) -> int:
    blocks = ((M + 127) // 128) * ((N + 127) // 128)
    nk = K // 64
    S = 1
    while blocks * S < 512 and S * 2 <= nk and S < 32:
        S *= 2
    if N <= 64 and M >= 2048 and cus > 0 and os.environ.get("A3V_SKINNY_LEGACY", "0") != "1":
        S = max(1, min(cus // ((M + 255) // 256), nk // 2, 32))
    elif N <= 64 and M >= 512 and S > 4:
# ... 562 lines not shown
        elif kx:
            self._skinny(xn, li[f"qkv.{i}.A"], t_qkv)
            ops.gemm_qkv_rope(xn_full, im[f"qkv.{i}.x"], qrot, kc, vc, m._cos_sin_dev(), B, S, H, Hkv, hd, 0, 0,
                              v_rows=qkv[:, (H + Hkv) * hd:])
            lt["qkv"] = t_qkv
        elif self.lora and self.act == torch.bfloat16 and hd in (64, 128) and rows > 16 and self.fuse_qkv_rope:
            li = self._lora_step_images()
            A, Bm = li[f"qkv.{i}.A"], li[f"qkv.{i}.B"]
            t = self._buf("lora_t.qkv" + tag, (rows, A.shape[0]))
            self._skinny(xn, A, t)
            ops.gemm_nt(t, Bm, qkv)
            ops.gemm_qkv_rope(xn, im[f"qkv.{i}"], qrot, kc, vc, m._cos_sin_dev(), B, S, H, Hkv, hd, 0, 0,
                              v_rows=qkv[:, (H + Hkv) * hd:], delta=qkv)
            lt["qkv"] = t
        else:
            ops.gemm_nt(xn, im[f"qkv.{i}"], qkv)
            if self.lora:
                lt["qkv"] = self._lora_fwd(f"qkv.{i}", xn, qkv, tag)
            ops.rope_kvcache(qkv, qrot, kc, vc, m._cos_sin_dev(), B, S, H, Hkv, hd, 0, 0)
        ldo = att.stride(0)
        strides = (S * H * hd, H * hd, hd, Hkv * spad * hd, spad * hd, hd, Hkv * hd * spad, hd * spad, spad, S * ldo, ldo, hd)
        ops.attention_lse(qrot, kc, vc, att, lse, B, S, S, H, Hkv, hd, strides, True)
        res_flag = ops.EPI_RES_F32 if (self.act == torch.bfloat16 and self.stream == torch.float32) else 0
        h_mid = self._buf("h_mid" + tag, (rows, dim), self.stream) if keep else h
        if kx:
            self._skinny(att, li[f"wo.{i}.A"], t_wo)
            ops.gemm_nt(att_full, im[f"wo.{i}.x"], h_mid, residual=h, epilogue=res_flag)
            lt["wo"] = t_wo
        else:
            ops.gemm_nt(att, im[f"wo.{i}"], h_mid, residual=h, epilogue=res_flag)
            if self.lora:
                lt["wo"] = self._lora_fwd(f"wo.{i}", att, h_mid, tag)
        gu = self._buf("gu" + tag, (rows, 2 * F))
        if kx:
            xn2_full, xn2, t_w13 = xbuf("xn2", dim, f"w13.{i}")
            act_full, actb, t_w2 = xbuf("act", F, f"w2.{i}")
        else:
            xn2 = self._buf("xn2" + tag, (rows, dim))
            actb = self._buf("act" + tag, (rows, F))
        ops.rmsnorm(h_mid, l.ffn_norm.weight, xn2, a.norm_eps)
        if kx:
            self._skinny(xn2, li[f"w13.{i}.A"], t_w13)
            ops.gemm_nt(xn2_full, im[f"w13.{i}.x"], gu)
            lt["w13"] = t_w13
        else:
            ops.gemm_nt(xn2, im[f"w13.{i}"], gu)
            if self.lora:
                lt["w13"] = self._lora_fwd(f"w13.{i}", xn2, gu, tag)
        ops.swiglu_fwd(gu, actb, F, interleaved=False)
        if kx:
            self._skinny(actb, li[f"w2.{i}.A"], t_w2)
            lt["w2"] = t_w2
        elif self.lora:
            li2 = self._lora_step_images()
            lt["w2"] = self._buf("lora_t.w2" + tag, (rows, li2[f"w2.{i}.A"].shape[0]))
            self._skinny(actb, li2[f"w2.{i}.A"], lt["w2"])
        kept = dict(xn=xn, qkv=qkv, qrot=qrot, kc=kc, att=att, lse=lse, h_mid=h_mid, xn2=xn2, gu=gu, act=actb, spad=spad, lt=lt)
        if keep and h_out is None:
            return kept
        out = h_out if keep else h
        if kx:
            ops.gemm_nt(act_full, im[f"w2.{i}.x"], out, residual=h_mid, epilogue=res_flag)
            return kept
        ops.gemm_nt(actb, im[f"w2.{i}"], out, residual=h_mid, epilogue=res_flag)
        if self.lora:
            f32 = out.dtype == torch.float32 and self.act == torch.bfloat16
            ops.gemm_nt(lt["w2"], self._lora_step_images()[f"w2.{i}.B"], out, residual=out, epilogue=ops.EPI_RES_F32 if f32 else 0)
        return kept

    def _block_backward(self, i: int, h_in: torch.Tensor, dh: torch.Tensor, B: int, S: int):
        m, a, im = self.m, self.m.args, self._images()
        H, Hkv, hd, dim, F = m.n_heads, m.n_kv_heads, m.head_dim, a.dim, m.ffn
        rows = B * S
        l = m.layers[i]
        pre = f"layers.{i}."
        k = self._saved["kept"][i] if self._saved.get("kept") else self._block_forward(i, h_in, B, S, keep=True)
        lt = k.get("lt", {})
        kx = self._kext() > 0 and rows > 16 and hd in (64, 128) and self.fuse_qkv_rope
        li = self._lora_step_images() if kx else None

        def ybuf(name, cols, key):
            full = self._buf(name, (rows, cols + li[key + ".A"].shape[0]))
            return full, full[:, :cols]
        stream_lp = self.stream == torch.bfloat16 and self.act == torch.bfloat16
        if stream_lp:
            dha = dh
            dha_full = self._dh_full if kx else None
        elif kx:
            dha_full, dha = ybuf("dh_act.x", dim, f"w2.{i}")
        else:
            dha = self._buf("dh_act", (rows, dim))
        fuse_cast = self.act == torch.bfloat16 and not stream_lp
        if not stream_lp and not (fuse_cast and getattr(self, "_dha_ready", False)):
            ops.cast(dh, dha)
        self._dha_ready = False
        if self._has(pre + "feed_forward.w2.weight"):
            self._wgrad(dha, k["act"], self._views[pre + "feed_forward.w2.weight"], "w2", (pre + "feed_forward.w2.weight",))
        if kx and self.fuse_swiglu_bwd and self._nt_dgrad(f"w2.{i}") and F % 8 == 0:
            dgu_full, dgu = ybuf("dgu.x", 2 * F, f"w13.{i}")
            self._kx_group_bwd(i, f"w2.{i}", dha_full, dim, k["act"], lt["w2"], dgu, swiglu_gu=k["gu"])
        elif (not self.lora and self.fuse_swiglu_bwd and self.nn_dgrad and self.act == torch.bfloat16 and dim % 64 == 0 and F % 8 == 0 and F >= 256
              and dha.stride(0) % 8 == 0 and 2 * rows * dha.stride(0) < 2 ** 31 and 2 * F * dim < 2 ** 31
              and tuple(im[f"w2.{i}"].shape) == (dim, F)):
            dgu = self._buf("dgu", (rows, 2 * F))
            ops.gemm_nn(dha, im[f"w2.{i}"], dgu, residual=k["gu"], epilogue=ops.EPI_SWIGLU_BWD)
        elif (not self.lora and self.fuse_swiglu_bwd and not self.nn_dgrad and self.act == torch.bfloat16 and dim % 64 == 0 and F % 8 == 0
              and dha.stride(0) % 8 == 0 and tuple(im[f"w2.{i}.t"].shape) == (F, dim)):
            dgu = self._buf("dgu", (rows, 2 * F))
            ops.gemm_nt(dha, im[f"w2.{i}.t"], dgu, residual=k["gu"], epilogue=ops.EPI_SWIGLU_BWD)
        else:
            dact = self._buf("dact", (rows, F))
            if kx:
                self._kx_group_bwd(i, f"w2.{i}", dha_full, dim, k["act"], lt["w2"], dact)
                dgu_full, dgu = ybuf("dgu.x", 2 * F, f"w13.{i}")
            else:
                self._dgrad_w(dha, f"w2.{i}", dact)
                if self.lora:
                    self._lora_bwd(i, f"w2.{i}", dha, k["act"], lt["w2"], dact)
                dgu = self._buf("dgu", (rows, 2 * F))
            ops.swiglu_bwd(k["gu"], dact, dgu, F, interleaved=False)
        if self._has(pre + "feed_forward.w1.weight", pre + "feed_forward.w3.weight"):
            self._wgrad(dgu, k["xn2"], self._gview(pre + "feed_forward.w1.weight", pre + "feed_forward.w3.weight"), "w13",
                        (pre + "feed_forward.w1.weight", pre + "feed_forward.w3.weight"))
        dxn = self._buf("dxn", (rows, dim))
        if kx:
            self._kx_group_bwd(i, f"w13.{i}", dgu_full, 2 * F, k["xn2"], lt["w13"], dxn)
        else:
            self._dgrad_w(dgu, f"w13.{i}", dxn)
            if self.lora:
                self._lora_bwd(i, f"w13.{i}", dgu, k["xn2"], lt["w13"], dxn)
        ops.rmsnorm_bwd(k["h_mid"], l.ffn_norm.weight, dxn, dh, self._views.get(pre + "ffn_norm.weight"), a.norm_eps,
                        dh_lowp=dha if fuse_cast else None)
        if not fuse_cast and not stream_lp:
            ops.cast(dh, dha)
        if self._has(pre + "attention.wo.weight"):
            self._wgrad(dha, k["att"], self._views[pre + "attention.wo.weight"], "wo", (pre + "attention.wo.weight",))
        datt = self._buf("datt", (rows, H * hd))
        if kx:
            self._kx_group_bwd(i, f"wo.{i}", dha_full, dim, k["att"], lt["wo"], datt)
        else:
            self._dgrad_w(dha, f"wo.{i}", datt)
            if self.lora:
                self._lora_bwd(i, f"wo.{i}", dha, k["att"], lt["wo"], datt)
        D = self._buf("attn_D", (B, S, H), torch.float32)
        qkv = k["qkv"]
        ld = qkv.stride(0)
        vrows = qkv[:, (H + Hkv) * hd:]
        spad = k["spad"]
        if kx:
            dqkv_full, dqkv = ybuf("dqkv.x", (H + 2 * Hkv) * hd, f"qkv.{i}")
        else:
            dqkv = self._buf("dqkv", (rows, (H + 2 * Hkv) * hd))
        if self.act == torch.bfloat16 and hd in (64, 128) and self.packed_attn_bwd:
            ops.attention_bwd_packed(k["qrot"], k["kc"], Hkv * spad * hd, spad * hd, vrows, S * ld, ld, hd, k["att"], datt, k["lse"], D,
                                     dqkv, m._cos_sin_dev(), B, S, H, Hkv, hd, True, 0)
        else:
            dq = self._buf("dq", (rows, H * hd))
            dk = self._buf("dk", (B, Hkv, S, hd))
            dv = self._buf("dv", (B, Hkv, S, hd))
            wsp = None
            if self.act == torch.bfloat16 and hd in (64, 128):
                wsp = self._buf("attn_bwd_ws", (ops.attention_bwd_workspace_bytes(B, S, H, Hkv, hd),), torch.uint8)
            att_c = k["att"] if k["att"].is_contiguous() else k["att"].contiguous()
            ops.attention_bwd(k["qrot"], k["kc"], Hkv * spad * hd, spad * hd, vrows, S * ld, ld, hd, att_c, datt, k["lse"], D,
                              dq, dk, dv, B, S, H, Hkv, hd, True, workspace=wsp)
            ops.rope_bwd_pack(dq, dk, dv, dqkv, m._cos_sin_dev(), B, S, H, Hkv, hd, 0)
        if self._has(pre + "attention.wq.weight", pre + "attention.wk.weight", pre + "attention.wv.weight"):
            self._wgrad(dqkv, k["xn"], self._gview(pre + "attention.wq.weight", pre + "attention.wv.weight"), "qkv",
                        (pre + "attention.wq.weight", pre + "attention.wk.weight", pre + "attention.wv.weight"))
        if kx:
            self._kx_group_bwd(i, f"qkv.{i}", dqkv_full, (H + 2 * Hkv) * hd, k["xn"], lt["qkv"], dxn)
        else:
            self._dgrad_w(dqkv, f"qkv.{i}", dxn)
            if self.lora:
                self._lora_bwd(i, f"qkv.{i}", dqkv, k["xn"], lt["qkv"], dxn)
        ops.rmsnorm_bwd(h_in, l.attention_norm.weight, dxn, dh, self._views.get(pre + "attention_norm.weight"), a.norm_eps,
                        dh_lowp=dha if fuse_cast else None)
        self._dha_ready = fuse_cast

    @torch.no_grad()
    def forward_loss(self, examples: torch.Tensor, labels: torch.Tensor, image: Optional[torch.Tensor] = None,
                     qformer_feats=None, extra_feats=None) -> torch.Tensor:
        self._check_dtypes()
        self._li_checked = False
        m, a = self.m, self.m.args
        im = self._images()
        B, T = examples.shape
        n_img = 0 if image is None else (len(image) if isinstance(image, (list, tuple)) else 1)
        W = m.words_per_image * n_img if n_img else 0
        S = T + W
        rows = B * S
        dim, V = a.dim, a.vocab_size
        h = self._buf("h", (rows, dim), self.stream)
        if self.lora or self.act != torch.bfloat16:
            self.sync_optimizer()
        self.await_weights("embed")
        ops.embed_assemble(examples.contiguous(), m.tok_embeddings.weight, h, B, T, W, dim)
        vis = None
        if image is not None:
            self.await_weights("vision_proj")
            vis = self._encode_image_train(h, image, B, S, qformer_feats, extra_feats)
        hs = self._buf("h_saved", (m.n_layers + 1, rows, dim), self.stream)
        if self.recompute is None:
            F_, Hq = m.ffn, (m.n_heads + 2 * m.n_kv_heads) * m.head_dim
            esz = 2 if self.act == torch.bfloat16 else 4
            need = m.n_layers * rows * ((2 * dim + Hq + 2 * m.n_heads * m.head_dim + 3 * F_) * esz + dim * (4 if self.stream == torch.float32 else 2)) * 1.1
            free, _ = torch.cuda.mem_get_info(m._device)
            self.recompute = need > 0.5 * free
        kept = []
        if self.recompute:
            for i in range(m.n_layers):
                hs[i].copy_(h)
                self.await_weights(f"layer{i}")
                self._block_forward(i, h, B, S, keep=False)
        else:
            hs[0].copy_(h)
            for i in range(m.n_layers):
                self.await_weights(f"layer{i}")
                kept.append(self._block_forward(i, hs[i], B, S, keep=True, tag=f".L{i}", h_out=hs[i + 1]))
            h = hs[m.n_layers]
        self.sync_optimizer()
        xt = self._buf("xn_text", (B * T, dim))
        hv = h.view(B, S, dim)
        for b in range(B):
            ops.rmsnorm(hv[b, W:], m.norm.weight, xt[b * T:(b + 1) * T], a.norm_eps)
        logits = self._buf("logits", (B * T, V))
        ops.gemm_nt(xt, im["out"], logits)
        lab = self._buf("lab", (B, T), torch.int64, zero=True)
        lab[:, :T - 1].copy_(labels[:, 1:])
        lab = lab.view(-1)
        n_valid = self._buf("n_valid", (1,), torch.int32)
        ops.count_valid(lab, n_valid)
        row_loss = self._buf("row_loss", (B * T,), torch.float32)
        ops.cross_entropy(logits, lab, row_loss)
        nv = n_valid.to(torch.float32)[0]
        loss = torch.where(nv > 0, row_loss.sum() / torch.clamp(nv, min=1.0), torch.zeros_like(nv))
        self._saved = dict(B=B, T=T, W=W, S=S, h=h, hs=hs, xt=xt, logits=logits, lab=lab, n_valid=n_valid, tokens=examples.contiguous(), vis=vis,
                           kept=kept if not self.recompute else None)
        return loss

    @torch.no_grad()
    def backward(self, grad_scale: float = 1.0) -> None:
        s = self._saved
        self._dha_ready = False
        self._li_checked = False
        assert s is not None, "backward() without forward_loss()"
        m, a = self.m, self.m.args
        self.sync_optimizer()
        im = self._images()
        self.ensure_grads()
        if not self.nn_dgrad and not self.lora and not getattr(self, "_nt_mem_checked", False):
            self._nt_mem_checked = True
            need = 2 * sum(q.numel() for g_ in im.groups() if g_ != "vp" for q in im._params(g_)[0])
            if not getattr(self, "_opt_stepped", False):
                need += 8 * sum(q.numel() for q in m.parameters() if q.requires_grad)
            free, _ = torch.cuda.mem_get_info(m._device)
            free += torch.cuda.memory_reserved(m._device) - torch.cuda.memory_allocated(m._device)
            if free - need < 8 * 2 ** 30 or (self.recompute and "A3V_NN_DGRAD" not in os.environ):
                self.nn_dgrad = True
        if self.lora and not getattr(self, "_nt_mem_checked", False):
            self._nt_mem_checked = True
            if not self.nn_dgrad or self.lora_nt_dgrad not in ("", "0"):
                need = 2 * sum(q.numel() for g_ in im.groups() if g_ != "vp" for q in im._params(g_)[0])
                free, _ = torch.cuda.mem_get_info(m._device)
                free += torch.cuda.memory_reserved(m._device) - torch.cuda.memory_allocated(m._device)
                if free - need < 8 * 2 ** 30:
                    self.nn_dgrad = True
                    self.lora_nt_dgrad = "0"
        if self.sumsq_sink is not None:
            self.sumsq_sink.begin_backward()
        B, T, W, S = s["B"], s["T"], s["W"], s["S"]
        rows, dim, V = B * S, a.dim, a.vocab_size
        dlog = self._buf("dlogits", (B * T, V))
        ops.cross_entropy(s["logits"], s["lab"], self._buf("row_loss", (B * T,), torch.float32), dlog, s["n_valid"], grad_scale)
        if self._has("output.weight"):
            self._wgrad(dlog, s["xt"], self._views["output.weight"], "out", ("output.weight",))
        dxt = self._buf("dxn_text", (B * T, dim))
        self._dgrad_w(dlog, "out", dxt)
        kx = self._kext() > 0 and rows > 16 and m.head_dim in (64, 128) and self.fuse_qkv_rope
        self._dh_full = None
        if self.stream == torch.bfloat16 and self.act == torch.bfloat16 and kx:
            self._dh_full = self._buf("dh.x", (rows, dim + self._kext_cols("w2.0")), self.stream, zero=True)
            dh = self._dh_full[:, :dim]
        else:
            dh = self._buf("dh", (rows, dim), self.stream, zero=True)
        hv, dhv = s["h"].view(B, S, dim), dh.view(B, S, dim)
        for b in range(B):
            ops.rmsnorm_bwd(hv[b, W:], m.norm.weight, dxt[b * T:(b + 1) * T], dhv[b, W:], self._views.get("norm.weight"), a.norm_eps)
        self._notify("head")
        for i in range(m.n_layers - 1, -1, -1):
            self._block_backward(i, s["hs"][i], dh, B, S)
            self._notify(f"layer{i}")
        if self._has("tok_embeddings.weight"):
            ops.embed_bwd(s["tokens"], dh, self._views["tok_embeddings.weight"], B, T, W, dim)
        self._notify("embed")
        if s["vis"] is not None:
            self._encode_image_backward(dh, s["vis"], B, S)
        self._notify("vision_proj")
        self._saved = None

    def _notify(self, bucket: str):
        if self.on_layer_grads_ready is None:
            return
        for name, st, en in self._ranges:
            if name == bucket:
                self.on_layer_grads_ready(name, st, en)

    def _encode_image_train(self, h, image, B, S, qformer_feats, extra_feats):
# ... 89 lines not shown
        v = self.eng._pview(list(ps)) if self.eng.zero1_world and not self.eng.lora else None
        if v is not None:
            return v
        return torch.cat(list(ps), dim=0) if len(ps) > 1 else ps[0]

    def _both(self, key, w):
        ext = self.eng._kext_cols(key)
        if ext:
            N, K = w.shape
            full = torch.zeros(N + ext, K + ext, dtype=self.eng.act, device=w.device)
            full[:N, :K] = w.to(self.eng.act)
            self.store[key] = full[:N, :K]
            self.store[key + ".x"] = full[:N]
            self.store[key + ".y"] = full[:, :K]
            if self.eng._nt_dgrad(key):
                ft = torch.zeros(K, N + ext, dtype=self.eng.act, device=w.device)
                ft[:, :N] = full[:N, :K].t()
                self.store[key + ".yT"] = ft
        else:
            self.store[key] = w.to(self.eng.act).contiguous()

    def _transposed(self, key: str, ver) -> torch.Tensor:
        if self.tver.get(key) != ver:
            act = self.eng.act
            wa = self.store[key[:-2]]
            N, K = wa.shape
            Np = _pad64(N)
            if Np != N:
                wp = torch.zeros(Np, K, dtype=act, device=wa.device)
                wp[:N] = wa
            else:
                wp = wa
            wt = self.store.get(key)
            if wt is None or wt.shape != (K, Np) or wt.dtype != act:
                ld = Np + 64 if (Np * wa.element_size()) % 4096 == 0 else Np
                wt = torch.empty(K, ld, dtype=act, device=wa.device)[:, :Np]
            ops.transpose(wp, wt, Np, K, Np)
            self.store[key] = wt
            self.tver[key] = ver
        return self.store[key]

    def _params(self, g: str):
        m = self.eng.m
        if g.startswith("L"):
            i = int(g[1:])
            a, f = m.layers[i].attention, m.layers[i].feed_forward
            H, Hkv, hd, F = m.n_heads, m.n_kv_heads, m.head_dim, m.ffn
            return ((a.wq.weight, a.wk.weight, a.wv.weight, a.wo.weight, f.w1.weight, f.w3.weight, f.w2.weight),
                    ((f"qkv.{i}", 0), (f"qkv.{i}", H * hd), (f"qkv.{i}", (H + Hkv) * hd), (f"wo.{i}", 0), (f"w13.{i}", 0), (f"w13.{i}", F),
                     (f"w2.{i}", 0)))
        if g == "out":
            return (m.output.weight,), (("out", 0),)
        vp0 = getattr(m.visual_proj, "0")
        if getattr(m.args, "qformer_tokens", 0):
            qp0 = getattr(m.qformer_proj, "0")
            return (vp0.weight, vp0.bias, qp0.weight, qp0.bias), (("vp", 0), ("vp.b", 0), ("vq", 0), ("vq.b", 0))
        return (vp0.weight, vp0.bias), (("vp", 0), ("vp.b", 0))

    def _key(self, ps) -> tuple:
        return tuple(param_state_key(q) for q in ps) + (self.eng.act, str(self.eng.m._device))

    def groups(self):
        m = self.eng.m
        return [f"L{i}" for i in range(m.n_layers)] + ["out"] + (["vp"] if getattr(m, "visual_proj", None) is not None else [])

    def sink(self, p) -> Optional[torch.Tensor]:
        if self.eng.act != torch.bfloat16:
            return None
        if self._sinks is None:
            self._sinks = {}
            for g in self.groups():
                ps, where = self._params(g)
                for q, (key, row) in zip(ps, where):
                    self._sinks[id(q)] = (key, row)
        ent = self._sinks.get(id(p))
        if ent is None:
            return None
        img = self.store.get(ent[0])
        if img is None or img.dtype != torch.bfloat16:
            return None
        return img[ent[1]:ent[1] + p.shape[0]] if img.dim() == 2 else img

    def sink_t(self, p):
        if self.eng.act != torch.bfloat16 or p.dim() != 2 or (p.shape[0] & 63) or (p.shape[1] & 63):
            return None
        self.sink(p)
        ent = self._sinks.get(id(p))
        if ent is None or ent[0].endswith(".b"):
            return None
        wt = self.store.get(ent[0] + ".t")
        if wt is None or wt.dtype != torch.bfloat16 or wt.dim() != 2 or wt.shape[0] != p.shape[1] or ent[1] + p.shape[0] > wt.shape[1] \
                or (ent[1] & 3) or self.tver.get(ent[0] + ".t") is None:
            return None
        return wt[:, ent[1]:ent[1] + p.shape[0]], int(wt.stride(0))

    def adopted(self, written_ids, written_t_ids=()) -> None:
        for g in self.groups():
            ps, where = self._params(g)
            if g in self.ver and all(id(q) in written_ids for q in ps):
                old = self.ver[g]
                self.ver[g] = self._key(ps)
                for key in {k for k, _ in where}:
                    if self.tver.get(key + ".t") == old and all(id(q) in written_t_ids for q, (k, _) in zip(ps, where) if k == key):
                        self.tver[key + ".t"] = self.ver[g]

    def __getitem__(self, key: str) -> torch.Tensor:
        eng, m = self.eng, self.eng.m
        g = self._group(key)
        ps, _ = self._params(g)
        if g.startswith("L"):
            i = int(g[1:])
        ver = self._key(ps)
        if self.ver.get(g) != ver:
            with torch.no_grad():
                if g.startswith("L"):
                    self._both(f"qkv.{i}", self._fused(ps[0:3]))
                    self._both(f"wo.{i}", self._fused(ps[3:4]))
                    self._both(f"w13.{i}", self._fused(ps[4:6]))
                    self._both(f"w2.{i}", self._fused(ps[6:7]))
                elif g == "out":
                    self._both("out", self._fused(ps[0:1]))
                else:
                    self._both("vp", ps[0])
                    self.store["vp.b"] = ps[1].to(eng.act)
                    if len(ps) == 4:
                        self._both("vq", ps[2])
                        self.store["vq.b"] = ps[3].to(eng.act)
            self.ver[g] = ver
        if key.endswith(".t"):
            return self._transposed(key, ver)
        return self.store[key]


class _StepLoss(torch.autograd.Function):

    @staticmethod
    def forward(ctx, anchor, engine, examples, labels, image):
        ctx.engine = engine
        return engine.forward_loss(examples, labels, image)

    @staticmethod
    def backward(ctx, grad_out):
        hint = getattr(ctx.engine, "static_grad_scale", None)
        ctx.engine.backward(float(grad_out) if hint is None else float(hint))
        return torch.zeros((), device=grad_out.device), None, None, None, None


def step_loss(engine: TrainEngine, anchor: torch.Tensor, examples, labels, image=None) -> torch.Tensor:
    return _StepLoss.apply(anchor, engine, examples, labels, image)


def hbm_budget(dim: int, n_layers: int, n_heads: int, ffn: int, vocab: int, batch: int, seq: int, text: int, n_kv_heads: Optional[int] = None,
               vit_params: int = 304_000_000, proj_in: int = 1024, world: int = 1, wire_bytes: int = 2, recompute: bool = False,
               stream_bytes: int = 2, zero1: bool = False, transposed_images: bool = False) -> Dict[str, int]:
    hkv = n_kv_heads or n_heads
    hd = dim // n_heads
    qkv = (n_heads + 2 * hkv) * hd
    p_layer = dim * qkv + dim * dim + 3 * dim * ffn
    p_mat = n_layers * p_layer + dim * vocab
    p_train = p_mat + dim * vocab + (2 * n_layers + 1) * dim + proj_in * dim + 4 * dim
    rows = batch * seq
    spad = (seq + 63) // 64 * 64
    sb = stream_bytes
    block = rows * (2 * dim * 2 + qkv * 2 + 2 * n_heads * hd * 2 + 3 * ffn * 2 + dim * sb) + batch * hkv * spad * hd * 2 + batch * n_heads * seq * 4
    bwd_ws = rows * ((dim * 2 if sb == 4 else 0) + ffn * 2 + 2 * ffn * 2 + dim * 2 + n_heads * hd * 2 + qkv * 2 + dim * sb) + batch * hkv * hd * spad * 2
    if zero1:
        p_big = p_mat + dim * vocab
        p_small = p_train - p_big
        layer_big = p_layer if n_layers else 0
        out = {"masters_fp32": 4 * p_small + 4 * p_big // world, "grads_fp32": 4 * p_train + 4 * p_big // world,
               "adamw_moments_fp32": 8 * p_small + 8 * p_big // world, "images_bf16": 2 * p_big + 2 * p_big // world,
               "vit_bf16": 2 * vit_params,
               "wire_buckets": (wire_bytes * max(layer_big, dim * vocab) + wire_bytes * max(layer_big, dim * vocab) // world) if wire_bytes != 4 else 0}
    else:
        out = {
            "masters_fp32": 4 * p_train, "grads_fp32": 4 * p_train, "adamw_moments_fp32": 8 * p_train, "images_bf16": 2 * p_mat,
            "vit_bf16": 2 * vit_params,
            "wire_buckets": wire_bytes * p_train if world > 1 and wire_bytes != 4 else 0}
    if transposed_images and not zero1:
        out["images_t_bf16"] = 2 * p_mat
    out.update({
        "stream_checkpoints": (n_layers + 1) * rows * dim * sb + rows * dim * sb,
        "block_activations": block * (1 if recompute else n_layers),
        "backward_workspace": bwd_ws,
        "ce_buffers": batch * text * vocab * 2 * 2 + batch * text * dim * 2 * 2,
    })
    out["total"] = sum(out.values())
    return out
```

### include/a3vlm_hip.h

```cpp
#ifndef A3VLM_HIP_H
#define A3VLM_HIP_H

#include <stdint.h>

#ifdef __cplusplus
extern "C" {
#endif

enum { A3V_BF16 = 0, A3V_F32 = 1 };

enum {
  A3V_OK = 0,
  A3V_ERR_SHAPE = -1,
  A3V_ERR_DTYPE = -2,
  A3V_ERR_ARG = -3
};

enum {
  A3V_EPI_NONE = 0,
  A3V_EPI_BIAS = 1,
  A3V_EPI_GELU = 2,
  A3V_EPI_QUICKGELU = 4,
  A3V_EPI_RESIDUAL = 8,
  A3V_EPI_SWIGLU = 16,
// ... 41 lines not shown
                       int S, void* stream);

int a3v_gemm_set_workspace_for(void* stream, void* ptr, int64_t bytes);
int a3v_gemm_set_workspace(void* ptr, int64_t bytes);

int a3v_gemm_nt_splitk(const void* A, int64_t lda, const void* W, int64_t ldw, float* partial, int M, int N,
                       int K, int S, void* stream);
int a3v_splitk_reduce(const float* partial, int S, int M, int N, void* out, int64_t ldo, int out_dtype,
                      int accumulate, void* stream);

int a3v_gemm_skinny_split(int M, int N, int K);
int64_t a3v_gemm_skinny_ws_bytes(int M, int N, int K);
int a3v_gemm_skinny_fp8(const void* A, int64_t lda, const void* Wq, int64_t ldw, const float* wscale, void* C,
                        int64_t ldc, int M, int N, int K, const void* residual, int64_t ldr, int epilogue,
                        void* workspace, void* stream);
int64_t a3v_quantize_nf4_ws_bytes(int N, int K);
int a3v_quantize_nf4(const void* W, int N, int K, void* q, float* scales, float* ws, void* stream);
int a3v_dequantize_nf4(const void* q, const float* scales, void* Wd, int64_t ldd, int N, int K, void* stream);
int a3v_gemm_skinny_nf4(const void* A, int64_t lda, const void* Wq, int64_t ldw, const float* scales, void* C, int64_t ldc,
                        int M, int N, int K, const void* residual, int64_t ldr, int epilogue, void* workspace, void* stream);
int a3v_gemm_skinny(const void* A, int64_t lda, const void* W, int64_t ldw, void* C, int64_t ldc,
                    int M, int N, int K, const void* residual, int64_t ldr, int epilogue,
                    void* partial, void* stream);

int a3v_rmsnorm(const void* x, int64_t ldx, const void* w, void* y, int64_t ldy, int rows, int dim,
                float eps, int x_dtype, int w_dtype, int y_dtype, void* stream);

int a3v_layernorm(const void* x, int64_t ldx, const void* w, const void* b, void* y, int64_t ldy,
                  const int32_t* row_map, int rows, int dim, float eps, int x_dtype, int p_dtype,
                  int y_dtype, void* stream);

int a3v_rope_kvcache(const void* qkv, int64_t ldqkv, void* q_out, int64_t ldq, void* k_cache,
                     void* vt_cache, const float* cos_sin, int B, int S, int H, int Hkv, int hd,
                     int Smax, int start_pos, int rope_pos0, int dtype, void* stream);

int a3v_vt_pack(const void* v, int64_t ldv, void* vt, int N, int L, int H, int hd, int Lpad,
                int dtype, void* stream);

int64_t a3v_attention_scratch_floats(int B, int H, int hd, int Sk);
int a3v_attention(const void* q, const void* k, const void* vt, void* out, int B, int Sq, int Sk,
                  int H, int Hkv, int hd, const int64_t* strides, int causal, float* scratch,
                  int dtype, void* stream);

int a3v_embed_assemble(const int64_t* tokens, int64_t ld_tok, const void* table, void* h, int B,
                       int T, int W, int dim, int vocab, int table_dtype, int h_dtype, void* stream);

int a3v_fill_rows(const void* src, void* dst, int64_t ldd, const int32_t* row_idx, int n_rows,
                  int dim, int src_dtype, int dst_dtype, void* stream);

int a3v_patch_im2col(const void* img, void* cols, int N, int Hi, int Wi, int P, int Kpad,
                     int in_dtype, int out_dtype, void* stream);

int a3v_split_views(const void* img, void* out, int B, int crop, int in_dtype, int out_dtype,
                    void* stream);

int a3v_vit_embed(const void* patch, const void* cls, const void* pos, void* x, int N, int T,
                  int width, int dtype, void* stream);

int a3v_preprocess_image(const uint8_t* src, int H, int W, int side, int pad_x, int pad_y, const int* fill_rgb,
                         const int32_t* kx, const int32_t* bx, int ksize_x, const int32_t* ky, const int32_t* by, int ksize_y,
                         int out_size, uint8_t* tmp, void* dst, int dst_dtype, const float* mean, const float* std, void* stream);

typedef struct {
  const uint8_t* src;
  const int32_t* coeffs;
  const int32_t* bounds;
  int H, W, side, pad_x, pad_y, ksize;
} a3v_image_desc;
int a3v_preprocess_batch(const a3v_image_desc* images, int n, const int* fill_rgb, int out_size, uint8_t* tmp, int64_t tmp_stride,
                         void* dst, int64_t dst_stride, int dst_dtype, const float* mean, const float* std, void* stream);

int a3v_generate_step(const float* logits, int64_t ld, const int64_t* sampled, int B, int V, int64_t* tokens, int64_t ld_tok,
                      const uint8_t* text_mask, int64_t ld_mask, int cur_pos, const int64_t* stop_seq, const int32_t* stop_off,
                      int n_stop, uint8_t* stopped, int64_t* stop_pos, int32_t* live, void* stream);

int a3v_sample_top_p(const float* logits, int64_t ld, int B, int V, float temperature, float top_p, const float* u,
                     int64_t* out, void* stream);

int a3v_argmax(const float* logits, int64_t ld, int64_t* out, int B, int V, void* stream);

int a3v_count_valid(const int64_t* labels, int rows, int32_t* n_valid_dev, void* stream);
int a3v_cross_entropy(const void* logits, int64_t ld, const int64_t* labels, float* row_loss,
                      void* dlogits, int64_t ldd, const int32_t* n_valid_dev, float grad_scale,
                      int rows, int V, int dtype, void* stream);

typedef struct a3v_llama_layer {
  const void* attn_norm_w;
  const void* wqkv;
  const void* wo;
  const void* ffn_norm_w;
  const void* w13;
  const void* w2;
  void* k_cache;
  void* vt_cache;
  const void* wqkv_q; const float* wqkv_s;
  const void* wo_q;   const float* wo_s;
  const void* w13_q;  const float* w13_s;
  const void* w2_q;   const float* w2_s;
  const void* wqkv_n4; const float* wqkv_n4s;
  const void* wo_n4;   const float* wo_n4s;
  const void* w13_n4;  const float* w13_n4s;
  const void* w2_n4;   const float* w2_n4s;
} a3v_llama_layer;
int a3v_llama_decode_step(const a3v_llama_layer* layers, int n_layers, void* h, void* xn, void* qkv,
                          void* att, void* act, float* attn_scratch, void* skinny_ws, const float* cos_sin, int B,
                          int dim, int H, int Hkv, int hd, int ffn, int Smax, int pos, float eps,
                          void* stream);
int a3v_llama_decode_step_form(int B, int dim, int H, int Hkv, int hd, int ffn, int w8);


int a3v_attention_lse(const void* q, const void* k, const void* vt, void* out, float* lse, int B,
                      int Sq, int Sk, int H, int Hkv, int hd, const int64_t* strides, int causal,
                      int dtype, void* stream);

int a3v_transpose(const void* src, int64_t ld_src, int64_t bs_src, void* dst, int64_t ld_dst,
                  int64_t bs_dst, int R, int C, int Rpad, int batch, int dtype, void* stream);

int64_t a3v_rmsnorm_bwd_scratch_floats(int rows, int dim);
int a3v_rmsnorm_bwd(const float* x, int64_t ldx, const float* w, const void* dy, int64_t lddy,
                    float* dh, int64_t lddh, float* dw, float* dw_scratch, int rows, int dim, float eps,
                    int act_dtype, void* stream);
int a3v_rmsnorm_bwd_cast(const float* x, int64_t ldx, const float* w, const void* dy, int64_t lddy,
                         float* dh, int64_t lddh, float* dw, float* dw_scratch, int rows, int dim, float eps,
                         int act_dtype, void* dh_bf16, int64_t ld_bf16, void* stream);

int a3v_rmsnorm_bwd_bf16(const void* x, int64_t ldx, const float* w, const void* dy, int64_t lddy, void* dh, int64_t lddh,
                         float* dw, float* dw_scratch, int rows, int dim, float eps, void* stream);
int a3v_layernorm_bwd_bf16(const void* x, int64_t ldx, const float* w, const void* dy, int64_t lddy, const int32_t* row_map,
                           void* dx, int64_t lddx, float* dw, float* db, int rows, int dim, float eps, void* stream);
int a3v_embed_bwd_bf16(const int64_t* tokens, int64_t ld_tok, const void* dh, float* dtable, int B, int T, int W, int dim,
                       int vocab, void* stream);

int a3v_layernorm_bwd(const void* x, int64_t ldx, const float* w, const float* dy, int64_t lddy,
                      const int32_t* row_map, void* dx, int64_t lddx, float* dw, float* db, int rows,
                      int dim, float eps, int act_dtype, void* stream);

int a3v_swiglu_fwd(const void* gu, int64_t ldg, void* act, int64_t lda, int rows, int F,
                   int interleaved, int dtype, void* stream);
int a3v_swiglu_bwd(const void* gu, int64_t ldg, const void* dact, int64_t lda, void* dgu,
                   int64_t lddg, int rows, int F, int interleaved, int dtype, void* stream);

int a3v_rope_bwd_pack(const void* dq, const void* dk, const void* dv, void* dqkv, int64_t ld,
                      const float* cos_sin, int B, int S, int H, int Hkv, int hd, int rope_pos0,
                      int dtype, void* stream);

int a3v_attention_bwd(const void* q, const void* k, int64_t k_sb, int64_t k_sh, const void* v,
                      int64_t v_sb, int64_t v_ss, int64_t v_sh, const void* out, const void* dout,
                      const float* lse, float* D, void* dq, void* dk, void* dv, void* workspace,
                      int B, int S, int H, int Hkv, int hd, int causal, int dtype, void* stream);
int a3v_attention_bwd_packed(const void* q, const void* k, int64_t k_sb, int64_t k_sh, const void* v, int64_t v_sb,
                             int64_t v_ss, int64_t v_sh, const void* out, int64_t ld_out, const void* dout, const float* lse, float* D,
                             void* dqkv, int64_t ld_qkv, const float* cos_sin, int rope_pos0, int B, int S, int H, int Hkv,
                             int hd, int causal, int dtype, void* stream);
int64_t a3v_attention_bwd_workspace_bytes(int B, int S, int H, int Hkv, int hd);
int a3v_attention_bwd_mfma(const void* q, const void* k, int64_t k_sb, int64_t k_sh, const void* v,
                           int64_t v_sb, int64_t v_ss, int64_t v_sh, const void* dout, const float* lse,
                           const float* D, void* dq, void* dk, void* dv, void* workspace, int B, int S,
                           int H, int Hkv, int hd, int causal, void* stream);

int a3v_add2d(void* dst, int64_t ld_dst, const void* src, int64_t ld_src, int rows, int cols, int dtype, void* stream);
int a3v_cast(const void* src, int64_t ld_src, int src_dtype, void* dst, int64_t ld_dst, int dst_dtype,
             int rows, int cols, void* stream);

int a3v_embed_bwd(const int64_t* tokens, int64_t ld_tok, const float* dh, float* dtable, int B, int T,
                  int W, int dim, int vocab, void* stream);

int a3v_rows_sum(const void* src, int64_t ld, const int32_t* row_idx, int n_rows, int dim, float* out,
                 int dtype, void* stream);

int a3v_adamw(float* param, const float* grad, float* exp_avg, float* exp_avg_sq, int64_t n, float lr, float beta1, float beta2,
              float eps, float weight_decay, int64_t step, void* bf16_image, void* stream);

int a3v_adamw_scaled(float* param, const float* grad, float* exp_avg, float* exp_avg_sq, int64_t n, float lr, float beta1, float beta2,
                     float eps, float weight_decay, int64_t step, void* bf16_image, const float* grad_scale, void* stream);

int a3v_lora_gb_scatter(const float* gbt, int64_t ld, int r, int n_mods, float* const* dst, const int* row0, const int* nj, void* stream);

int a3v_gemm_tn_strip(const void* T, int64_t ldt, const void* X, int64_t ldx, float* partial, int R, int N, int Kt, int S, void* stream);

int a3v_adamw_scaled_t(float* param, const float* grad, float* exp_avg, float* exp_avg_sq, int rows, int cols, float lr, float beta1,
                       float beta2, float eps, float weight_decay, int64_t step, void* bf16_image, void* bf16_image_t, int64_t ldt,
                       const float* grad_scale, void* stream);

typedef struct {
  float* p; const float* g; float* m; float* v;
  int64_t n, cols;
  void* d1; int64_t s1r, s1c;
  void* d2; int64_t s2r, s2c;
} a3v_adamw_tensor;
int a3v_adamw_multi(const a3v_adamw_tensor* table, int n_tensors, int64_t max_n, float lr, float beta1, float beta2, float eps,
                    float weight_decay, int64_t step, const float* grad_scale, void* stream);

int a3v_scale_cast(const void* src, int src_dtype, void* dst, int dst_dtype, int64_t n, float scale, void* stream);

int a3v_grad_bucket_allreduce(void* comm, float* grad, int64_t n, void* wire_bf16, int average, void* stream);

int a3v_grad_bucket_reduce_scatter(void* comm, const float* grad, int64_t n_per_rank, float* shard, void* wire_bf16, void* wire_shard_bf16,
                                   int average, void* stream);
int a3v_param_shard_all_gather(void* comm, const void* shard_bf16, void* flat_bf16, int64_t n_per_rank, void* stream);
int a3v_rccl_comm_count(void* comm);
int a3v_rccl_available(void);

#define A3V_SUMSQ_SLOTS 1024
int a3v_sumsq_partials(const float* x, int64_t n, float* out, void* stream);

int a3v_lora_refresh(const float* lora_a, const float* lora_b, int r, int in_f, int nj, void* A, int64_t lda, void* At, int64_t ldat,
                     void* B, int64_t ldb, void* Bt, int64_t ldbt, int col0, int row0, void* stream);

#ifdef __cplusplus
}
#endif
#endif
```

Before: 35.38.

## Hand dS tiles from dK/dV kernel to a dQ kernel via workspace

The dK/dV backward kernel body moves into a shared include, and a new variant writes the computed dS tiles to a global workspace at head dim 128. A separate dQ kernel then reads K and the stored dS tiles and accumulates dQ with MFMA, so dQ no longer has to recompute P and dS. The workspace is plumbed through a new _ws API entry point and allocated in the training step. This adds a large per-head dS buffer (extra HBM traffic and memory) in exchange for avoiding the recomputation.

```diff
diff --git a/a3vlm_amd/csrc/a3v_attn_bwd.hip b/a3vlm_amd/csrc/a3v_attn_bwd.hip
--- a/a3vlm_amd/csrc/a3v_attn_bwd.hip
+++ b/a3vlm_amd/csrc/a3v_attn_bwd.hip
@@ -15,6 +15,10 @@
 #ifdef AB_STAMP
   unsigned long long* stamps;
 #endif
+};
+struct DsArgs {
+  char* ws;
+  int64_t head_bytes, qt_bytes;
 };
 #ifdef AB_STAMP
 #define AB_ST(kern, it, k) do { if (stamps && (it) < 64) stamps[((kern) * 64 + (it)) * 8 + (k)] = __builtin_amdgcn_s_memtime(); } while (0)
@@ -510,6 +514,10 @@
 __device__ __forceinline__ void dma4_asm(i32x4_t rs, unsigned lds_addr, unsigned voff) {
   asm volatile("s_nop 4\n\ts_mov_b32 m0, %0\n\ts_nop 0\n\tbuffer_load_dword %1, %2, 0 offen lds" ::"s"(lds_addr), "v"(voff), "s"(rs) : "memory", A3V_AGPR_0_255);
 }
+template <int OFF>
+__device__ __forceinline__ void ds_store16(uint64_t base, unsigned voff, const bf16x8& v) {
+  asm volatile("global_store_dwordx4 %0, %1, %2 offset:%c3" ::"v"(voff), "v"(v), "s"(base), "i"(OFF) : "memory", A3V_AGPR_0_255);
+}
 __device__ __forceinline__ i32x4_t make_rsrc(const void* base, int bytes) {
   const uint64_t a = (uint64_t)base;
   i32x4_t r;
@@ -540,373 +548,134 @@
 
 template <int HD, bool PACKED>
 __global__ __launch_bounds__(256, 1) void attn_bwd_dkv2_kernel(BwdArgs p) {
-  constexpr int TILE = 64 * HD * 2;
-  constexpr int BUFB = 2 * TILE + 1024;
-  constexpr int NKS = HD / 16, NDB = HD / 32;
-  constexpr int RV = 0, RK = 64, RKF = 128, RVF = 160, RS = 192, RDP = 208;
-  constexpr int NB = 4;
-  __shared__ __attribute__((aligned(1024))) char lds[NB * BUFB + 4096];
+  constexpr bool EMIT_DS = false;
+  const DsArgs dsa{};
+#include "a3v_attn_bwd_dkv2.inc"
+}
+template <int HD, bool PACKED>
+__global__ __launch_bounds__(256, 1) void attn_bwd_dkv2_emit_kernel(BwdArgs p, DsArgs dsa) {
+  static_assert(HD == 128, "the dS hand-over exists at hd 128 only");
+  constexpr bool EMIT_DS = true;
+#include "a3v_attn_bwd_dkv2.inc"
+}
+
+__device__ __forceinline__ void dma16_lds(i32x4_t rs, unsigned lds_addr, unsigned voff) {
+  asm volatile("s_nop 4\n\ts_mov_b32 m0, %0\n\ts_nop 0\n\tbuffer_load_dwordx4 %1, %2, 0 offen lds" ::"s"(lds_addr), "v"(voff), "s"(rs) : "memory");
+}
+__device__ __forceinline__ bf16x8 frag_ds_tr(const char* sub, int base, int tb, int c) {
+  const char* blk = sub + (32 * tb + 16 * c) * 64;
+  const s16x4_t lo = __builtin_amdgcn_ds_read_tr16_b64_v4i16((s16x4_t __attribute__((address_space(3)))*)(blk + base));
+  const s16x4_t hi = __builtin_amdgcn_ds_read_tr16_b64_v4i16((s16x4_t __attribute__((address_space(3)))*)(blk + base + 8 * 64));
+  bf16x8 f;
+  const short v[8] = {lo[0], lo[1], lo[2], lo[3], hi[0], hi[1], hi[2], hi[3]};
+  __builtin_memcpy(&f, v, 16);
+  return f;
+}
+
+template <bool PACKED>
+__global__ __launch_bounds__(256, 2) void attn_bwd_dq_ds_kernel(BwdArgs p, DsArgs dsa) {
+  constexpr int HD = 128, TILE = 64 * HD * 2, STAGE = 2 * TILE;
+  __shared__ __attribute__((aligned(1024))) char lds[2 * STAGE];
   const int tid = threadIdx.x, lane = tid & 63, wave = __builtin_amdgcn_readfirstlane(tid >> 6);
-#ifdef AB_STAMP
-  unsigned long long* tl = (p.stamps && tid == 0) ? p.stamps + 4096 + 8 * blockIdx.x : nullptr;
-  if (tl) { tl[0] = __builtin_amdgcn_s_memrealtime(); tl[4] = __builtin_amdgcn_s_getreg(0x0004 | (0 << 6) | (31 << 11)); tl[5] = __builtin_amdgcn_s_getreg(20 | (0 << 6) | (31 << 11)); }
-#endif
-  int head_slot, kt_;
-  xcd_head_tile((p.S + 127) / 128, head_slot, kt_, p.group_kv);
-  const int b = head_slot / p.Hkv, hk = head_slot - b * p.Hkv;
-  const int nrep = p.H / p.Hkv;
-  const int kl = lane & 31, hh = lane >> 5;
-  const int kv_lo = kt_ * 128 + wave * 32;
-  const int kvrow = kv_lo + kl;
-  const int kc = kvrow < p.S ? kvrow : p.S - 1;
-  asm volatile("" ::: A3V_AGPR_0_255);
-  const float sl2 = p.scale * 1.4426950408889634f;
-  const int q_begin = p.causal ? kt_ * 2 : 0;
-  const int n_qt = (p.S + 63) / 64;
-  const int n_it = n_qt - q_begin, total = nrep * n_it;
-  const unsigned qoff = dma_lane_offset0<HD>((int64_t)p.H * HD, tid);
-  const int fbase = frag_rows_base<HD>(kl, hh);
+  const int nqt = (p.S + 127) / 128;
+  int head_slot, ti;
+  xcd_head_tile(nqt, head_slot, ti, p.group_q);
+  const int qt = nqt - 1 - ti, b = head_slot / p.H, h = head_slot - b * p.H;
+  const int hk = h / (p.H / p.Hkv);
+  const int ql = lane & 31, hh = lane >> 5;
+  const int qrow = qt * 128 + wave * 32 + ((ql & 19) | ((ql & 4) << 1) | ((ql & 8) >> 1));
+  const bf16_t* K = p.k + b * p.k_sb + hk * p.k_sh;
+  f32x16 acc[HD / 32];
+#pragma unroll
+  for (int d = 0; d < HD / 32; ++d)
+#pragma unroll
+    for (int r = 0; r < 16; ++r) acc[d][r] = 0.f;
+  int kv_end = p.S;
+  if (p.causal) kv_end = min(p.S, qt * 128 + 128);
+  const int n_tiles = (kv_end + 63) / 64;
+  const int q32 = qt * 4 + wave;
+  const bool wave_live = q32 * 32 < p.S;
+  const unsigned koff = dma_lane_offset0<HD>(HD, tid);
   const TrBase trb = tr_bases<HD>(lane);
-
-  int rep_n = 0, qi_n = 0, buf_n = 0;
+  const unsigned dsoff = wave * 4096 + (lane & 2) * 512 + (lane & 1) * 512 + (lane >> 2) * 16;
+  const int i16 = lane & 15;
+  const int dsb = (4 * hh + (i16 >> 2)) * 64 + (2 * (ql >> 4) + ((i16 & 3) >> 1)) * 16 + (i16 & 1) * 8;
+  const char* ds_tiles = dsa.ws + ((int64_t)b * p.H + h) * dsa.head_bytes + (int64_t)qt * dsa.qt_bytes;
+  auto live = [&](int t, int tb) { return wave_live && (!p.causal || 2 * t + tb <= q32); };
   const unsigned lds0 = (unsigned)(size_t)((__attribute__((address_space(3))) char*)lds);
-  constexpr int PP = HD / 16;
-  i32x4_t rsQ, rsO, rsX;
-  unsigned dmaQ, dmaO, dmaX, dma_step_i, voffX;
-  const unsigned qstep = dma_step<HD>((int64_t)p.H * HD);
-  const int64_t rstride = (int64_t)p.H * HD;
-  const uint64_t pairB = (uint64_t)(64 * rstride * 2);
-  uint64_t aQ = (uint64_t)(p.q + ((int64_t)b * p.S * p.H + hk * nrep) * HD + (int64_t)q_begin * 64 * rstride);
-  uint64_t aO = (uint64_t)(p.dout + ((int64_t)b * p.S * p.H + hk * nrep) * HD + (int64_t)q_begin * 64 * rstride);
-  uint64_t aL = (uint64_t)(p.lse + ((int64_t)b * p.H + hk * nrep) * p.S + q_begin * 64);
-  uint64_t aD = (uint64_t)(p.D + ((int64_t)b * p.S + q_begin * 64) * p.H + hk * nrep);
-  int64_t leftQ = ((int64_t)(p.S - 1 - q_begin * 64) * rstride + HD) * 2;
-  int rowsL = p.S - q_begin * 64;
-  voffX = (wave == 1) ? lane * p.H * 4 : lane * 4;
-  auto mk = [&](uint64_t a, int bytes) __attribute__((always_inline)) {
-    i32x4_t r;
-    r[0] = (int)(unsigned)a; r[1] = (int)(unsigned)(a >> 32) & 0xffff; r[2] = bytes; r[3] = 0x00020000;
-    return r;
+  const unsigned kstep = dma_step<HD>(HD);
+  auto stage = [&](int t, unsigned st) {
+    const i32x4_t rk = make_rsrc(K + (int64_t)t * 64 * HD, (p.S - t * 64) * HD * 2);
+#pragma unroll
+    for (int i = 0; i < 4; ++i) dma16_lds(rk, st + (wave * 64 + i * 256) * 16, koff + i * kstep);
+    if (!live(t, 0)) return;
+    const i32x4_t rs = make_rsrc(ds_tiles + (int64_t)t * 16384, 16384);
+    const unsigned sub = st + TILE + wave * 4096;
+    dma16_lds(rs, sub, dsoff);
+    dma16_lds(rs, sub + 1024, dsoff + 256);
+    if (live(t, 1)) {
+      dma16_lds(rs, sub + 2048, dsoff + 2048);
+      dma16_lds(rs, sub + 3072, dsoff + 2048 + 256);
+    }
   };
-  auto prep_issue = [&](bool real) __attribute__((always_inline)) {
-    const unsigned buf = lds0 + buf_n * BUFB, patch = lds0 + NB * BUFB + wave * 1024;
-    const int nb = real ? (int)(leftQ < 0x7fffffff ? leftQ : 0x7fffffff) : 0;
-    rsQ = mk(aQ, nb);
-    rsO = mk(aO, nb);
-    dmaQ = real ? buf + wave * 1024 : patch;
-    dmaO = real ? buf + TILE + wave * 1024 : patch;
-    dma_step_i = real ? 4096u : 0u;
-    if (wave == 0) { rsX = mk(aL, real ? rowsL * 4 : 0); dmaX = real ? buf + 2 * TILE : patch; }
-    else if (wave == 1) { rsX = mk(aD, real ? ((rowsL - 1) * p.H + 1) * 4 : 0); dmaX = real ? buf + 2 * TILE + 256 : patch; }
-    else { rsX = mk(aL, 0); dmaX = patch; }
-    if (real) {
-      if (++buf_n == NB) buf_n = 0;
-      if (++qi_n == n_it) {
-        qi_n = 0; ++rep_n;
-        const int64_t back = (int64_t)(n_it - 1) * 64;
-        aQ += (uint64_t)(HD * 2) - (uint64_t)(back * rstride * 2); aO += (uint64_t)(HD * 2) - (uint64_t)(back * rstride * 2);
-        aL += (uint64_t)((int64_t)p.S * 4) - (uint64_t)(back * 4); aD += 4 - (uint64_t)(back * p.H * 4);
-        leftQ += back * rstride * 2; rowsL += (int)back;
-      } else {
-        aQ += pairB; aO += pairB; aL += 256; aD += (uint64_t)(64 * p.H * 4);
-        leftQ -= (int64_t)pairB; rowsL -= 64;
+  stage(0, lds0);
+  auto body = [&](int t, auto bufc) {
+    constexpr int BUF = decltype(bufc)::value;
+    const char* Ks = lds + BUF * STAGE;
+    const char* sub = Ks + TILE + wave * 4096;
+    asm volatile("s_waitcnt vmcnt(0)" ::: "memory");
+    __syncthreads();
+    if (t + 1 < n_tiles) stage(t + 1, lds0 + (1 - BUF) * STAGE);
+    if (!live(t, 0)) return;
+    const bool both = live(t, 1);
+#pragma unroll
+    for (int tb = 0; tb < 2; ++tb) {
+      if (tb == 1 && !both) break;
+#pragma unroll
+      for (int c = 0; c < 2; ++c) {
+        const bf16x8 dsf = frag_ds_tr(sub, dsb, tb, c);
+#pragma unroll
+        for (int d = 0; d < HD / 32; ++d)
+          acc[d] = __builtin_amdgcn_mfma_f32_32x32x16_bf16(frag_rows_tr<HD>(Ks, trb, d, tb, c), dsf, acc[d], 0, 0, 0);
       }
     }
   };
-  auto piece = [&](auto i_) __attribute__((always_inline)) {
-    constexpr int i = decltype(i_)::value;
-    if constexpr (i < PP / 2) dma16_asm(rsQ, dmaQ + i * dma_step_i, qoff + i * qstep);
-    else if constexpr (i < PP) dma16_asm(rsO, dmaO + (i - PP / 2) * dma_step_i, qoff + (i - PP / 2) * qstep);
-    else dma4_asm(rsX, dmaX, voffX);
-  };
-  auto issue = [&](bool real) __attribute__((always_inline)) {
-    prep_issue(real);
-    sfor<0, PP + 1>([&](auto i_) { piece(i_); });
-  };
-
-  bf16x8 qa[NKS], da[NKS];
-  auto fetch = [&](const char* buf, int tb) __attribute__((always_inline)) {
-#pragma unroll
-    for (int ks = 0; ks < NKS; ++ks) {
-      qa[ks] = frag_rows<HD>(buf, fbase, tb, ks);
-      da[ks] = frag_rows<HD>(buf + TILE, fbase, tb, ks);
-    }
-  };
-  auto dead = [&](int qr0) { return qr0 >= p.S || (p.causal && qr0 + 31 < kv_lo); };
-  auto interior = [&](int qr0) { return qr0 + 32 <= p.S && kv_lo + 31 < p.S && (!p.causal || qr0 >= kv_lo + 31); };
-
-#ifdef AB_STAMP
-  unsigned long long* stamps = (p.stamps && blockIdx.x == AB_STAMP && tid == 0) ? p.stamps : nullptr;
-  int cur_it = 0;
-#endif
-  f32x16 dpv[2];
-  auto step = [&](auto DA_, auto DBC_, auto MASK_, auto TBC_, const char* cb, int qr0, const char* fb, int tbf) __attribute__((always_inline)) {
-    constexpr bool DA = decltype(DA_)::value, DBC = decltype(DBC_)::value, MASK = decltype(MASK_)::value;
-    constexpr int tbc = decltype(TBC_)::value;
-    constexpr int RSC = RS + 16 * tbc, RSN = RS + 16 * (1 - tbc);
-    constexpr int EPK = 16 / NKS;
-    bf16x8 trO[2][NDB], trQ[2][NDB], bP[2], bS[2];
-    f32x4 l4[4], d4[4];
-    float ex[EPK], dd[EPK];
-    const float* sm = reinterpret_cast<const float*>(cb + 2 * TILE) + tbc * 32 + 4 * hh;
-    if constexpr (DBC) {
-      l4[0] = *reinterpret_cast<const f32x4*>(sm);
-      d4[0] = *reinterpret_cast<const f32x4*>(sm + 64);
-    }
-    auto finish = [&](auto kp_) __attribute__((always_inline)) {
-      constexpr int kp = decltype(kp_)::value;
-#pragma unroll
-      for (int j = 0; j < EPK; ++j) {
-        const int r = kp * EPK + j;
-        bP[r >> 3][r & 7] = f2bf(ex[j]);
-        bS[r >> 3][r & 7] = f2bf(ex[j] * dd[j]);
-      }
-      u32x4 wP, wS;
-      __builtin_memcpy(&wP, &bP[(kp * EPK) >> 3], 16);
-      __builtin_memcpy(&wS, &bS[(kp * EPK) >> 3], 16);
-      constexpr int w0 = ((kp * EPK) & 7) / 2;
-      if constexpr (EPK == 2) asm volatile("" : "+v"(wP[w0]), "+v"(wS[w0]));
-      else asm volatile("" : "+v"(wP[w0]), "+v"(wP[w0 + 1]), "+v"(wS[w0]), "+v"(wS[w0 + 1]));
-      __builtin_memcpy(&bP[(kp * EPK) >> 3], &wP, 16);
-      __builtin_memcpy(&bS[(kp * EPK) >> 3], &wS, 16);
-    };
-    sfor<0, NKS>([&](auto ks_) {
-      constexpr int ks = decltype(ks_)::value;
-      if constexpr (DA) mfma_va<RSN, RKF + 4 * ks, ks == 0>(qa[ks]);
-      if constexpr (tbc == 0) piece(ks_);
-      float en[EPK], dn[EPK];
-      if constexpr (DBC) {
-        constexpr int g4 = (ks * EPK) >> 2;
-        sfor<0, EPK>([&](auto j_) {
-          constexpr int j = decltype(j_)::value, r = ks * EPK + j, e = r & 3;
-          const float sv = agpr_read<RSC + r>();
-          const float dv = dpv[tbc][r];
-          float a = fmaf(sv, sl2, l4[g4][e]);
-          if constexpr (MASK) {
-            const int qg = qr0 + 8 * g4 + 4 * hh + e;
-            const bool ok = (qg < p.S) && (kvrow < p.S) && (!p.causal || kvrow <= qg);
-            a = ok ? a : -INFINITY;
-          }
-          en[j] = __builtin_amdgcn_exp2f(a);
-          dn[j] = dv - d4[g4][e];
-        });
-        if constexpr (EPK == 2) asm volatile("" : "+v"(en[0]), "+v"(en[1]), "+v"(dn[0]), "+v"(dn[1]));
-        else asm volatile("" : "+v"(en[0]), "+v"(en[1]), "+v"(en[2]), "+v"(en[3]), "+v"(dn[0]), "+v"(dn[1]), "+v"(dn[2]), "+v"(dn[3]));
-      }
-      if constexpr (DA) mfma_va_v<RVF + 4 * ks, ks == 0>(dpv[1 - tbc], da[ks]);
-      if constexpr (DBC) {
-        if constexpr (ks > 0) finish(std::integral_constant<int, ks - 1>{});
-#pragma unroll
-        for (int j = 0; j < EPK; ++j) { ex[j] = en[j]; dd[j] = dn[j]; }
-        if constexpr (ks < NDB) {
-          trO[0][ks] = frag_rows_tr2<HD>(cb + TILE, trb, ks, tbc, 0);
-          trQ[0][ks] = frag_rows_tr2<HD>(cb, trb, ks, tbc, 0);
-        }
-        constexpr int gn = ((ks * EPK) >> 2) + 1;
-        if constexpr (((ks * EPK) & 3) == 0 && gn < 4) {
-          l4[gn] = *reinterpret_cast<const f32x4*>(sm + 8 * gn);
-          d4[gn] = *reinterpret_cast<const f32x4*>(sm + 64 + 8 * gn);
-        }
-        asm volatile("" ::: "memory");
-      }
-    });
-    if constexpr (tbc == 0) piece(std::integral_constant<int, PP>{});
-    if constexpr (DBC) finish(std::integral_constant<int, NKS - 1>{});
-    asm volatile("" ::: "memory");
-#ifdef AB_STAMP
-    if (stamps && cur_it < 64) stamps[(64 + cur_it) * 8 + 6 + tbc] = __builtin_amdgcn_s_memtime();
-#endif
-    constexpr int FPD = NKS / NDB;
-    sfor<0, NDB>([&](auto d_) {
-      constexpr int d = decltype(d_)::value;
-      if constexpr (DBC) {
-        mfma_vv<RV + 16 * d>(trO[0][d], bP[0]);
-        trO[1][d] = frag_rows_tr2<HD>(cb + TILE, trb, d, tbc, 1);
-      }
-      qa[d * FPD] = frag_rows<HD>(fb, fbase, tbf, d * FPD);
-      asm volatile("" ::: "memory");
-      if constexpr (DBC) {
-        mfma_vv<RK + 16 * d>(trQ[0][d], bS[0]);
-        trQ[1][d] = frag_rows_tr2<HD>(cb, trb, d, tbc, 1);
-      }
-      da[d * FPD] = frag_rows<HD>(fb + TILE, fbase, tbf, d * FPD);
-      asm volatile("" ::: "memory");
-    });
-    sfor<0, NDB>([&](auto d_) {
-      constexpr int d = decltype(d_)::value;
-      if constexpr (DBC) mfma_vv<RV + 16 * d>(trO[1][d], bP[1]);
-#pragma unroll
-      for (int ks = d * FPD + 1; ks < (d + 1) * FPD; ++ks) qa[ks] = frag_rows<HD>(fb, fbase, tbf, ks);
-      asm volatile("" ::: "memory");
-      if constexpr (DBC) mfma_vv<RK + 16 * d>(trQ[1][d], bS[1]);
-#pragma unroll
-      for (int ks = d * FPD + 1; ks < (d + 1) * FPD; ++ks) da[ks] = frag_rows<HD>(fb + TILE, fbase, tbf, ks);
-      asm volatile("" ::: "memory");
-    });
-    if constexpr (DA && !DBC) asm volatile("s_nop 15\n\ts_nop 15" ::: "memory", A3V_AGPR_0_255);
-  };
-  using T_ = std::true_type; using F_ = std::false_type;
-  auto run = [&](bool lc, bool ln, bool mk, auto tbc, const char* cb, int qr0, const char* fb, int tbf) __attribute__((always_inline)) {
-    if (lc) {
-      if (mk) step(T_{}, T_{}, T_{}, tbc, cb, qr0, fb, tbf);
-      else step(T_{}, T_{}, F_{}, tbc, cb, qr0, fb, tbf);
-    } else if (ln) {
-      step(T_{}, F_{}, F_{}, tbc, cb, qr0, fb, tbf);
-    } else {
-      step(F_{}, F_{}, F_{}, tbc, cb, qr0, fb, tbf);
-    }
-  };
-
-  auto prescale_lse = [&](const char* buf) __attribute__((always_inline)) {
-    if (wave == 3) {
-      float* sm = const_cast<float*>(reinterpret_cast<const float*>(buf + 2 * TILE));
-      sm[lane] = -1.4426950408889634f * sm[lane];
-    }
-  };
-#ifdef AB_STAMP
-#define AB_PE(k) do { if (stamps) stamps[2 * 64 * 8 + (k)] = __builtin_amdgcn_s_memtime(); } while (0)
-#else
-#define AB_PE(k) do {} while (0)
-#endif
-  AB_PE(0);
-#ifdef AB_STAMP
-  if (tl) tl[6] = __builtin_amdgcn_s_memrealtime();
-#endif
-  issue(true);
-#ifdef AB_STAMP
-  if (tl) tl[7] = __builtin_amdgcn_s_memrealtime();
-#endif
   {
-    const bf16_t* Kb = p.k + b * p.k_sb + hk * p.k_sh;
-    const bf16_t* Vb = p.v + b * p.v_sb + hk * p.v_sh;
-    const unsigned kvoffK = dma_lane_offset0<HD>(HD, tid), kvoffV = dma_lane_offset0<HD>(p.v_ss, tid);
-#pragma unroll
-    for (int t = 0; t < 2; ++t) {
-      stage_rows_dma_asm<HD>(Kb, HD, kt_ * 128 + 64 * t, p.S, lds0 + 2 * BUFB + t * TILE, kvoffK, wave);
-      stage_rows_dma_asm<HD>(Vb, p.v_ss, kt_ * 128 + 64 * t, p.S, lds0 + 3 * BUFB + t * TILE, kvoffV, wave);
-    }
-    sfor<0, 128>([&](auto i) { agpr_write<decltype(i)::value>(0u); });
-    asm volatile("s_waitcnt vmcnt(0)" ::: "memory", A3V_AGPR_0_255);
+    int t = 0;
+    for (; t + 1 < n_tiles; t += 2) {
+      body(t, std::integral_constant<int, 0>{});
+      body(t + 1, std::integral_constant<int, 1>{});
+    }
+    if (t < n_tiles) body(t, std::integral_constant<int, 0>{});
+  }
+#pragma unroll
+  for (int d = 0; d < HD / 32; ++d)
+#pragma unroll
+    for (int r = 0; r < 16; ++r) acc[d][r] *= p.scale;
+  if constexpr (PACKED) {
     __syncthreads();
-    prescale_lse(lds);
-    const char* Kt = lds + 2 * BUFB + (wave >> 1) * TILE;
-    const char* Vt = lds + 3 * BUFB + (wave >> 1) * TILE;
-    sfor<0, NKS>([&](auto ks_) {
-      constexpr int ks = decltype(ks_)::value;
-      const bf16x8 kq = frag_rows<HD>(Kt, fbase, wave & 1, ks), vq = frag_rows<HD>(Vt, fbase, wave & 1, ks);
-      u32x4 ku, vu;
-      __builtin_memcpy(&ku, &kq, 16);
-      __builtin_memcpy(&vu, &vq, 16);
-      sfor<0, 4>([&](auto j) {
-        agpr_write<RKF + 4 * ks + decltype(j)::value>(ku[decltype(j)::value]);
-        agpr_write<RVF + 4 * ks + decltype(j)::value>(vu[decltype(j)::value]);
-      });
-    });
-    __syncthreads();
-  }
-  AB_PE(1);
-  AB_PE(2);
-  issue(total > 1);
-  AB_PE(3);
-  fetch(lds, 0);
-  prep_issue(total > 2);
-  sfor<0, NKS>([&](auto ks_) {
-    constexpr int ks = decltype(ks_)::value;
-    mfma_va<RS, RKF + 4 * ks, ks == 0>(qa[ks]);
-    piece(ks_);
-    mfma_va_v<RVF + 4 * ks, ks == 0>(dpv[0], da[ks]);
-  });
-  piece(std::integral_constant<int, PP>{});
-  asm volatile("s_nop 15\n\ts_nop 15" ::: "memory", A3V_AGPR_0_255);
-  fetch(lds, 1);
-  AB_PE(4);
-  int qi_c = 0, buf_c = 0;
-#ifdef AB_STAMP
-  if (tl) tl[1] = __builtin_amdgcn_s_memrealtime();
-#endif
-  for (int it = 0; it < total; ++it) {
-    const int q0 = (q_begin + qi_c) * 64;
-    if (++qi_c == n_it) qi_c = 0;
-    const int q0x = (q_begin + qi_c) * 64;
-    const char* cb = lds + buf_c * BUFB;
-    if (++buf_c == NB) buf_c = 0;
-    const char* xb = lds + buf_c * BUFB;
-    const bool more = it + 1 < total;
-#ifdef AB_STAMP
-    cur_it = it;
-#endif
-    AB_ST(1, it, 0);
-    if constexpr (PP == 8) asm volatile("s_waitcnt vmcnt(9)" ::: "memory", A3V_AGPR_0_255); else asm volatile("s_waitcnt vmcnt(5)" ::: "memory", A3V_AGPR_0_255);
-    AB_ST(1, it, 1);
-    __syncthreads();
-    AB_ST(1, it, 2);
-    prep_issue(it + 3 < total);
-    if (more) prescale_lse(xb);
-    AB_ST(1, it, 3);
-    const bool l0 = !dead(q0), l1 = !dead(q0 + 32), lx = more && !dead(q0x);
-    run(l0, l1, !interior(q0), std::integral_constant<int, 0>{}, cb, q0, xb, 0);
-    AB_ST(1, it, 4);
-    run(l1, lx, !interior(q0 + 32), std::integral_constant<int, 1>{}, cb, q0 + 32, xb, 1);
-    AB_ST(1, it, 5);
-  }
-#ifdef AB_STAMP
-  if (tl) tl[2] = __builtin_amdgcn_s_memrealtime();
-#endif
-  asm volatile("s_nop 15\n\ts_nop 15" ::: "memory", A3V_AGPR_0_255);
-  AB_PE(5);
-  const float* CS = PACKED ? p.cos_sin + (int64_t)(p.rope_pos0 + kc) * HD : nullptr;
-  f32x4 cs[NDB][4];
-  if constexpr (PACKED) {
-#pragma unroll
-    for (int d = 0; d < NDB; ++d)
-#pragma unroll
-      for (int g4 = 0; g4 < 4; ++g4) cs[d][g4] = *reinterpret_cast<const f32x4*>(CS + d * 32 + g4 * 8 + hh * 4);
-  }
-  __syncthreads();
-  AB_PE(6);
-  char* patchV = lds + wave * (32 * HD * 2);
-  char* patchK = lds + 4 * (32 * HD * 2) + wave * (32 * HD * 2);
-  const int wx = (kl & (HD / 8 - 1)) << 1;
-  sfor<0, NDB>([&](auto d_) {
-    constexpr int d = decltype(d_)::value;
-    const f32x16 av = agpr_read16<RV + 16 * d>();
-#pragma unroll
-    for (int g4 = 0; g4 < 4; ++g4) {
-      bf16x4 ov;
-#pragma unroll
-      for (int e = 0; e < 4; ++e) ov[e] = f2bf(av[g4 * 4 + e]);
-      *reinterpret_cast<bf16x4*>(patchV + kl * (HD * 2) + (((d * 8 + g4 * 2 + hh) ^ wx) << 3)) = ov;
-    }
-  });
-  bf16_t* baseV = PACKED ? p.dqkv + (int64_t)b * p.S * p.ld_qkv + (int64_t)(p.H + p.Hkv + hk) * HD : p.dv + ((int64_t)b * p.Hkv + hk) * p.S * HD;
-  bf16_t* baseK = PACKED ? p.dqkv + (int64_t)b * p.S * p.ld_qkv + (int64_t)(p.H + hk) * HD : p.dk + ((int64_t)b * p.Hkv + hk) * p.S * HD;
-  const int64_t ldo = PACKED ? p.ld_qkv : HD;
-  store_patch_rows<HD>(patchV, baseV, ldo, kv_lo, p.S, lane);
-  AB_PE(7);
-  sfor<0, NDB>([&](auto d_) {
-    constexpr int d = decltype(d_)::value;
-    f32x16 ak = agpr_read16<RK + 16 * d>();
-#pragma unroll
-    for (int r = 0; r < 16; ++r) ak[r] *= p.scale;
-#pragma unroll
-    for (int g4 = 0; g4 < 4; ++g4) {
-      float v0 = ak[g4 * 4 + 0], v1 = ak[g4 * 4 + 1], v2 = ak[g4 * 4 + 2], v3 = ak[g4 * 4 + 3];
-      bf16x4 ok;
-      if constexpr (PACKED) {
-        const f32x4 c4 = cs[d][g4];
-        ok[0] = f2bf(v0 * c4[0] + v1 * c4[1]); ok[1] = f2bf(-v0 * c4[1] + v1 * c4[0]);
-        ok[2] = f2bf(v2 * c4[2] + v3 * c4[3]); ok[3] = f2bf(-v2 * c4[3] + v3 * c4[2]);
-      } else {
-        ok[0] = f2bf(v0); ok[1] = f2bf(v1); ok[2] = f2bf(v2); ok[3] = f2bf(v3);
-      }
-      *reinterpret_cast<bf16x4*>(patchK + kl * (HD * 2) + (((d * 8 + g4 * 2 + hh) ^ wx) << 3)) = ok;
-    }
-  });
-  store_patch_rows<HD>(patchK, baseK, ldo, kv_lo, p.S, lane);
-  AB_PE(8);
-#ifdef AB_STAMP
-  if (tl) { asm volatile("s_waitcnt vmcnt(0)" ::: "memory"); tl[3] = __builtin_amdgcn_s_memrealtime(); }
-#endif
+    const int ql_e = qrow - (qt * 128 + wave * 32);
+    char* patch = lds + wave * (32 * HD * 2);
+    char* wrow = patch + ql_e * (HD * 2);
+    const int wx = (ql_e & (HD / 8 - 1)) << 1;
+    const float* CS = p.cos_sin + (int64_t)(p.rope_pos0 + (qrow < p.S ? qrow : p.S - 1)) * HD;
+#pragma unroll
+    for (int d = 0; d < HD / 32; ++d)
+#pragma unroll
+      for (int g4 = 0; g4 < 4; ++g4) {
+        const int dc = d * 32 + g4 * 8 + hh * 4;
+        const f32x4 cs = *reinterpret_cast<const f32x4*>(CS + dc);
+        const float v0 = acc[d][g4 * 4 + 0], v1 = acc[d][g4 * 4 + 1], v2 = acc[d][g4 * 4 + 2], v3 = acc[d][g4 * 4 + 3];
+        bf16x4 ov;
+        ov[0] = f2bf(v0 * cs[0] + v1 * cs[1]); ov[1] = f2bf(-v0 * cs[1] + v1 * cs[0]);
+        ov[2] = f2bf(v2 * cs[2] + v3 * cs[3]); ov[3] = f2bf(-v2 * cs[3] + v3 * cs[2]);
+        *reinterpret_cast<bf16x4*>(wrow + (((d * 8 + g4 * 2 + hh) ^ wx) << 3)) = ov;
+      }
+    store_patch_rows<HD>(patch, p.dqkv + (int64_t)b * p.S * p.ld_qkv + (int64_t)h * HD, p.ld_qkv, qt * 128 + wave * 32, p.S, lane);
+  } else {
+    if (qrow < p.S)
+      store_grad_rows<HD, PACKED>(p, acc, p.dq + (((int64_t)b * p.S + qrow) * p.H + h) * HD, (int64_t)b * p.S + qrow, h, p.rope_pos0 + qrow, true, hh);
+  }
 }
 
 }
@@ -914,9 +683,13 @@
 extern "C" int a3v_transpose(const void* src, int64_t ld_src, int64_t bs_src, void* dst, int64_t ld_dst, int64_t bs_dst,
                              int R, int C, int Rpad, int batch, int dtype, void* stream);
 
+static bool attn_bwd_ds_enabled(int hd) { return hd == 128 && A3V_ENV_INT("A3V_ATTN_BWD_DS", 0) != 0; }
+
 extern "C" int64_t a3v_attention_bwd_workspace_bytes(int B, int S, int H, int Hkv, int hd) {
-  (void)B; (void)S; (void)H; (void)Hkv; (void)hd;
-  return 256;
+  (void)Hkv;
+  if (!attn_bwd_ds_enabled(hd) || B <= 0 || S <= 0 || H <= 0) return 256;
+  const int64_t nqt = (S + 127) / 128;
+  return (int64_t)B * H * nqt * (2 * nqt) * 16384;
 }
 
 #ifdef AB_STAMP
@@ -925,7 +698,7 @@
 #endif
 static int attention_bwd_mfma_impl(const void* q, const void* k, int64_t k_sb, int64_t k_sh, const void* v, int64_t v_sb,
                                    int64_t v_ss, int64_t v_sh, const void* dout, const float* lse, const float* D, void* dq,
-                                   void* dk, void* dv, void* dqkv, int64_t ld_qkv, const float* cos_sin, int rope_pos0, int B, int S, int H,
+                                   void* dk, void* dv, void* dqkv, int64_t ld_qkv, const float* cos_sin, int rope_pos0, void* ds_ws, int B, int S, int H,
                                    int Hkv, int hd, int causal, void* stream) {
   if (hd != 64 && hd != 128) return A3V_ERR_ARG;
   if ((k_sb % 8) || (k_sh % 8) || (v_sb % 8) || (v_ss % 8) || (v_sh % 8)) return A3V_ERR_SHAPE;
@@ -956,6 +729,21 @@
   p.group_q = group_of(B * H, gq.x);
   p.group_kv = group_of(B * Hkv, gk.x);
   const int v2 = A3V_ENV_INT("A3V_ATTN_BWD_V2", 1);
+  if (ds_ws && (v2 & 1) && attn_bwd_ds_enabled(hd)) {
+    DsArgs dsa;
+    dsa.ws = (char*)ds_ws;
+    dsa.qt_bytes = (int64_t)2 * ((S + 127) / 128) * 16384;
+    dsa.head_bytes = (int64_t)((S + 127) / 128) * dsa.qt_bytes;
+    if (dqkv) {
+      hipLaunchKernelGGL((attn_bwd_dkv2_emit_kernel<128, true>), gk, dim3(256), 0, st, p, dsa);
+      hipLaunchKernelGGL((attn_bwd_dq_ds_kernel<true>), gq, dim3(256), 0, st, p, dsa);
+    } else {
+      hipLaunchKernelGGL((attn_bwd_dkv2_emit_kernel<128, false>), gk, dim3(256), 0, st, p, dsa);
+      hipLaunchKernelGGL((attn_bwd_dq_ds_kernel<false>), gq, dim3(256), 0, st, p, dsa);
+    }
+    A3V_LAUNCH_CHECK();
+    return A3V_OK;
+  }
 #define A3V_BWD_LAUNCH(HDV, PK)                                                                  \
   do {                                                                                           \
     hipLaunchKernelGGL((attn_bwd_dq_kernel<HDV, PK>), gq, dim3(256), 0, st, p);                  \
@@ -981,15 +769,15 @@
                                       void* dk, void* dv, void* workspace, int B, int S, int H, int Hkv, int hd, int causal,
                                       void* stream) {
   if (!workspace || !dq || !dk || !dv) return A3V_ERR_ARG;
-  return attention_bwd_mfma_impl(q, k, k_sb, k_sh, v, v_sb, v_ss, v_sh, dout, lse, D, dq, dk, dv, nullptr, 0, nullptr, 0, B, S, H, Hkv, hd,
+  return attention_bwd_mfma_impl(q, k, k_sb, k_sh, v, v_sb, v_ss, v_sh, dout, lse, D, dq, dk, dv, nullptr, 0, nullptr, 0, workspace, B, S, H, Hkv, hd,
                                  causal, stream);
 }
 
 extern "C" __attribute__((visibility("hidden"))) int a3v_attention_bwd_mfma_packed(const void* q, const void* k, int64_t k_sb, int64_t k_sh, const void* v, int64_t v_sb,
                                              int64_t v_ss, int64_t v_sh, const void* dout, const float* lse, const float* D, void* dqkv,
-                                             int64_t ld_qkv, const float* cos_sin, int rope_pos0, int B, int S, int H, int Hkv, int hd,
+                                             int64_t ld_qkv, const float* cos_sin, int rope_pos0, void* workspace, int B, int S, int H, int Hkv, int hd,
                                              int causal, void* stream) {
   if (!dqkv || !cos_sin || ld_qkv % 4 || rope_pos0 < 0) return A3V_ERR_ARG;
   return attention_bwd_mfma_impl(q, k, k_sb, k_sh, v, v_sb, v_ss, v_sh, dout, lse, D, nullptr, nullptr, nullptr, dqkv, ld_qkv, cos_sin, rope_pos0,
-                                 B, S, H, Hkv, hd, causal, stream);
-}
+                                 workspace, B, S, H, Hkv, hd, causal, stream);
+}
diff --git a/a3vlm_amd/csrc/a3v_attn_bwd_dkv2.inc b/a3vlm_amd/csrc/a3v_attn_bwd_dkv2.inc
--- /dev/null
+++ b/a3vlm_amd/csrc/a3v_attn_bwd_dkv2.inc
@@ -0,0 +1,386 @@
+  constexpr int TILE = 64 * HD * 2;
+  constexpr int BUFB = 2 * TILE + 1024;
+  constexpr int NKS = HD / 16, NDB = HD / 32;
+  constexpr int RV = 0, RK = 64, RKF = 128, RVF = 160, RS = 192, RDP = 208;
+  constexpr int NB = 4;
+  __shared__ __attribute__((aligned(1024))) char lds[NB * BUFB + 4096];
+  const int tid = threadIdx.x, lane = tid & 63, wave = __builtin_amdgcn_readfirstlane(tid >> 6);
+#ifdef AB_STAMP
+  unsigned long long* tl = (p.stamps && tid == 0) ? p.stamps + 4096 + 8 * blockIdx.x : nullptr;
+  if (tl) { tl[0] = __builtin_amdgcn_s_memrealtime(); tl[4] = __builtin_amdgcn_s_getreg(0x0004 | (0 << 6) | (31 << 11)); tl[5] = __builtin_amdgcn_s_getreg(20 | (0 << 6) | (31 << 11)); }
+#endif
+  int head_slot, kt_;
+  xcd_head_tile((p.S + 127) / 128, head_slot, kt_, p.group_kv);
+  const int b = head_slot / p.Hkv, hk = head_slot - b * p.Hkv;
+  const int nrep = p.H / p.Hkv;
+  const int kl = lane & 31, hh = lane >> 5;
+  const int kv_lo = kt_ * 128 + wave * 32;
+  const int kvrow = kv_lo + kl;
+  const int kc = kvrow < p.S ? kvrow : p.S - 1;
+  asm volatile("" ::: A3V_AGPR_0_255);
+  const float sl2 = p.scale * 1.4426950408889634f;
+  const int q_begin = p.causal ? kt_ * 2 : 0;
+  const int n_qt = (p.S + 63) / 64;
+  const int n_it = n_qt - q_begin, total = nrep * n_it;
+  const unsigned qoff = dma_lane_offset0<HD>((int64_t)p.H * HD, tid);
+  const int fbase = frag_rows_base<HD>(kl, hh);
+  const TrBase trb = tr_bases<HD>(lane);
+
+  int rep_n = 0, qi_n = 0, buf_n = 0;
+  const unsigned lds0 = (unsigned)(size_t)((__attribute__((address_space(3))) char*)lds);
+  constexpr int PP = HD / 16;
+  i32x4_t rsQ, rsO, rsX;
+  unsigned dmaQ, dmaO, dmaX, dma_step_i, voffX;
+  const unsigned qstep = dma_step<HD>((int64_t)p.H * HD);
+  const int64_t rstride = (int64_t)p.H * HD;
+  const uint64_t pairB = (uint64_t)(64 * rstride * 2);
+  uint64_t aQ = (uint64_t)(p.q + ((int64_t)b * p.S * p.H + hk * nrep) * HD + (int64_t)q_begin * 64 * rstride);
+  uint64_t aO = (uint64_t)(p.dout + ((int64_t)b * p.S * p.H + hk * nrep) * HD + (int64_t)q_begin * 64 * rstride);
+  uint64_t aL = (uint64_t)(p.lse + ((int64_t)b * p.H + hk * nrep) * p.S + q_begin * 64);
+  uint64_t aD = (uint64_t)(p.D + ((int64_t)b * p.S + q_begin * 64) * p.H + hk * nrep);
+  int64_t leftQ = ((int64_t)(p.S - 1 - q_begin * 64) * rstride + HD) * 2;
+  int rowsL = p.S - q_begin * 64;
+  voffX = (wave == 1) ? lane * p.H * 4 : lane * 4;
+  auto mk = [&](uint64_t a, int bytes) __attribute__((always_inline)) {
+    i32x4_t r;
+    r[0] = (int)(unsigned)a; r[1] = (int)(unsigned)(a >> 32) & 0xffff; r[2] = bytes; r[3] = 0x00020000;
+    return r;
+  };
+  auto prep_issue = [&](bool real) __attribute__((always_inline)) {
+    const unsigned buf = lds0 + buf_n * BUFB, patch = lds0 + NB * BUFB + wave * 1024;
+    const int nb = real ? (int)(leftQ < 0x7fffffff ? leftQ : 0x7fffffff) : 0;
+    rsQ = mk(aQ, nb);
+    rsO = mk(aO, nb);
+    dmaQ = real ? buf + wave * 1024 : patch;
+    dmaO = real ? buf + TILE + wave * 1024 : patch;
+    dma_step_i = real ? 4096u : 0u;
+    if (wave == 0) { rsX = mk(aL, real ? rowsL * 4 : 0); dmaX = real ? buf + 2 * TILE : patch; }
+    else if (wave == 1) { rsX = mk(aD, real ? ((rowsL - 1) * p.H + 1) * 4 : 0); dmaX = real ? buf + 2 * TILE + 256 : patch; }
+    else { rsX = mk(aL, 0); dmaX = patch; }
+    if (real) {
+      if (++buf_n == NB) buf_n = 0;
+      if (++qi_n == n_it) {
+        qi_n = 0; ++rep_n;
+        const int64_t back = (int64_t)(n_it - 1) * 64;
+        aQ += (uint64_t)(HD * 2) - (uint64_t)(back * rstride * 2); aO += (uint64_t)(HD * 2) - (uint64_t)(back * rstride * 2);
+        aL += (uint64_t)((int64_t)p.S * 4) - (uint64_t)(back * 4); aD += 4 - (uint64_t)(back * p.H * 4);
+        leftQ += back * rstride * 2; rowsL += (int)back;
+      } else {
+        aQ += pairB; aO += pairB; aL += 256; aD += (uint64_t)(64 * p.H * 4);
+        leftQ -= (int64_t)pairB; rowsL -= 64;
+      }
+    }
+  };
+  auto piece = [&](auto i_) __attribute__((always_inline)) {
+    constexpr int i = decltype(i_)::value;
+    if constexpr (i < PP / 2) dma16_asm(rsQ, dmaQ + i * dma_step_i, qoff + i * qstep);
+    else if constexpr (i < PP) dma16_asm(rsO, dmaO + (i - PP / 2) * dma_step_i, qoff + (i - PP / 2) * qstep);
+    else dma4_asm(rsX, dmaX, voffX);
+  };
+  auto issue = [&](bool real) __attribute__((always_inline)) {
+    prep_issue(real);
+    sfor<0, PP + 1>([&](auto i_) { piece(i_); });
+  };
+
+  bf16x8 qa[NKS], da[NKS];
+  auto fetch = [&](const char* buf, int tb) __attribute__((always_inline)) {
+#pragma unroll
+    for (int ks = 0; ks < NKS; ++ks) {
+      qa[ks] = frag_rows<HD>(buf, fbase, tb, ks);
+      da[ks] = frag_rows<HD>(buf + TILE, fbase, tb, ks);
+    }
+  };
+  auto dead = [&](int qr0) { return qr0 >= p.S || (p.causal && qr0 + 31 < kv_lo); };
+  auto interior = [&](int qr0) { return qr0 + 32 <= p.S && kv_lo + 31 < p.S && (!p.causal || qr0 >= kv_lo + 31); };
+
+#ifdef AB_STAMP
+  unsigned long long* stamps = (p.stamps && blockIdx.x == AB_STAMP && tid == 0) ? p.stamps : nullptr;
+  int cur_it = 0;
+#endif
+  f32x16 dpv[2];
+  uint64_t ds_unit = 0;
+  const unsigned ds_voff = lane * 16;
+  auto step = [&](auto DA_, auto DBC_, auto MASK_, auto TBC_, const char* cb, int qr0, const char* fb, int tbf) __attribute__((always_inline)) {
+    constexpr bool DA = decltype(DA_)::value, DBC = decltype(DBC_)::value, MASK = decltype(MASK_)::value;
+    constexpr int tbc = decltype(TBC_)::value;
+    constexpr int RSC = RS + 16 * tbc, RSN = RS + 16 * (1 - tbc);
+    constexpr int EPK = 16 / NKS;
+    bf16x8 trO[2][NDB], trQ[2][NDB], bP[2], bS[2];
+    f32x4 l4[4], d4[4];
+    float ex[EPK], dd[EPK];
+    const float* sm = reinterpret_cast<const float*>(cb + 2 * TILE) + tbc * 32 + 4 * hh;
+    if constexpr (DBC) {
+      l4[0] = *reinterpret_cast<const f32x4*>(sm);
+      d4[0] = *reinterpret_cast<const f32x4*>(sm + 64);
+    }
+    auto finish = [&](auto kp_) __attribute__((always_inline)) {
+      constexpr int kp = decltype(kp_)::value;
+#pragma unroll
+      for (int j = 0; j < EPK; ++j) {
+        const int r = kp * EPK + j;
+        bP[r >> 3][r & 7] = f2bf(ex[j]);
+        bS[r >> 3][r & 7] = f2bf(ex[j] * dd[j]);
+      }
+      u32x4 wP, wS;
+      __builtin_memcpy(&wP, &bP[(kp * EPK) >> 3], 16);
+      __builtin_memcpy(&wS, &bS[(kp * EPK) >> 3], 16);
+      constexpr int w0 = ((kp * EPK) & 7) / 2;
+      if constexpr (EPK == 2) asm volatile("" : "+v"(wP[w0]), "+v"(wS[w0]));
+      else asm volatile("" : "+v"(wP[w0]), "+v"(wP[w0 + 1]), "+v"(wS[w0]), "+v"(wS[w0 + 1]));
+      __builtin_memcpy(&bP[(kp * EPK) >> 3], &wP, 16);
+      __builtin_memcpy(&bS[(kp * EPK) >> 3], &wS, 16);
+    };
+    sfor<0, NKS>([&](auto ks_) {
+      constexpr int ks = decltype(ks_)::value;
+      if constexpr (DA) mfma_va<RSN, RKF + 4 * ks, ks == 0>(qa[ks]);
+      if constexpr (tbc == 0) piece(ks_);
+      float en[EPK], dn[EPK];
+      if constexpr (DBC) {
+        constexpr int g4 = (ks * EPK) >> 2;
+        sfor<0, EPK>([&](auto j_) {
+          constexpr int j = decltype(j_)::value, r = ks * EPK + j, e = r & 3;
+          const float sv = agpr_read<RSC + r>();
+          const float dv = dpv[tbc][r];
+          float a = fmaf(sv, sl2, l4[g4][e]);
+          if constexpr (MASK) {
+            const int qg = qr0 + 8 * g4 + 4 * hh + e;
+            const bool ok = (qg < p.S) && (kvrow < p.S) && (!p.causal || kvrow <= qg);
+            a = ok ? a : -INFINITY;
+          }
+          en[j] = __builtin_amdgcn_exp2f(a);
+          dn[j] = dv - d4[g4][e];
+        });
+        if constexpr (EPK == 2) asm volatile("" : "+v"(en[0]), "+v"(en[1]), "+v"(dn[0]), "+v"(dn[1]));
+        else asm volatile("" : "+v"(en[0]), "+v"(en[1]), "+v"(en[2]), "+v"(en[3]), "+v"(dn[0]), "+v"(dn[1]), "+v"(dn[2]), "+v"(dn[3]));
+      }
+      if constexpr (DA) mfma_va_v<RVF + 4 * ks, ks == 0>(dpv[1 - tbc], da[ks]);
+      if constexpr (DBC) {
+        if constexpr (ks > 0) finish(std::integral_constant<int, ks - 1>{});
+#pragma unroll
+        for (int j = 0; j < EPK; ++j) { ex[j] = en[j]; dd[j] = dn[j]; }
+        if constexpr (ks < NDB) {
+          trO[0][ks] = frag_rows_tr2<HD>(cb + TILE, trb, ks, tbc, 0);
+          trQ[0][ks] = frag_rows_tr2<HD>(cb, trb, ks, tbc, 0);
+        }
+        constexpr int gn = ((ks * EPK) >> 2) + 1;
+        if constexpr (((ks * EPK) & 3) == 0 && gn < 4) {
+          l4[gn] = *reinterpret_cast<const f32x4*>(sm + 8 * gn);
+          d4[gn] = *reinterpret_cast<const f32x4*>(sm + 64 + 8 * gn);
+        }
+        asm volatile("" ::: "memory");
+      }
+    });
+    if constexpr (tbc == 0) piece(std::integral_constant<int, PP>{});
+    if constexpr (DBC) finish(std::integral_constant<int, NKS - 1>{});
+    if constexpr (EMIT_DS && DBC) {
+      ds_store16<0>(ds_unit + tbc * 4096, ds_voff, bS[0]);
+      ds_store16<1024>(ds_unit + tbc * 4096, ds_voff, bS[1]);
+    }
+    asm volatile("" ::: "memory");
+#ifdef AB_STAMP
+    if (stamps && cur_it < 64) stamps[(64 + cur_it) * 8 + 6 + tbc] = __builtin_amdgcn_s_memtime();
+#endif
+    constexpr int FPD = NKS / NDB;
+    sfor<0, NDB>([&](auto d_) {
+      constexpr int d = decltype(d_)::value;
+      if constexpr (DBC) {
+        mfma_vv<RV + 16 * d>(trO[0][d], bP[0]);
+        trO[1][d] = frag_rows_tr2<HD>(cb + TILE, trb, d, tbc, 1);
+      }
+      qa[d * FPD] = frag_rows<HD>(fb, fbase, tbf, d * FPD);
+      asm volatile("" ::: "memory");
+      if constexpr (DBC) {
+        mfma_vv<RK + 16 * d>(trQ[0][d], bS[0]);
+        trQ[1][d] = frag_rows_tr2<HD>(cb, trb, d, tbc, 1);
+      }
+      da[d * FPD] = frag_rows<HD>(fb + TILE, fbase, tbf, d * FPD);
+      asm volatile("" ::: "memory");
+    });
+    sfor<0, NDB>([&](auto d_) {
+      constexpr int d = decltype(d_)::value;
+      if constexpr (DBC) mfma_vv<RV + 16 * d>(trO[1][d], bP[1]);
+#pragma unroll
+      for (int ks = d * FPD + 1; ks < (d + 1) * FPD; ++ks) qa[ks] = frag_rows<HD>(fb, fbase, tbf, ks);
+      asm volatile("" ::: "memory");
+      if constexpr (DBC) mfma_vv<RK + 16 * d>(trQ[1][d], bS[1]);
+#pragma unroll
+      for (int ks = d * FPD + 1; ks < (d + 1) * FPD; ++ks) da[ks] = frag_rows<HD>(fb + TILE, fbase, tbf, ks);
+      asm volatile("" ::: "memory");
+    });
+    if constexpr (DA && !DBC) asm volatile("s_nop 15\n\ts_nop 15" ::: "memory", A3V_AGPR_0_255);
+  };
+  using T_ = std::true_type; using F_ = std::false_type;
+  auto run = [&](bool lc, bool ln, bool mk, auto tbc, const char* cb, int qr0, const char* fb, int tbf) __attribute__((always_inline)) {
+    if (lc) {
+      if (mk) step(T_{}, T_{}, T_{}, tbc, cb, qr0, fb, tbf);
+      else step(T_{}, T_{}, F_{}, tbc, cb, qr0, fb, tbf);
+    } else if (ln) {
+      step(T_{}, F_{}, F_{}, tbc, cb, qr0, fb, tbf);
+    } else {
+      step(F_{}, F_{}, F_{}, tbc, cb, qr0, fb, tbf);
+    }
+  };
+
+  auto prescale_lse = [&](const char* buf) __attribute__((always_inline)) {
+    if (wave == 3) {
+      float* sm = const_cast<float*>(reinterpret_cast<const float*>(buf + 2 * TILE));
+      sm[lane] = -1.4426950408889634f * sm[lane];
+    }
+  };
+#ifdef AB_STAMP
+#define AB_PE(k) do { if (stamps) stamps[2 * 64 * 8 + (k)] = __builtin_amdgcn_s_memtime(); } while (0)
+#else
+#define AB_PE(k) do {} while (0)
+#endif
+  AB_PE(0);
+#ifdef AB_STAMP
+  if (tl) tl[6] = __builtin_amdgcn_s_memrealtime();
+#endif
+  issue(true);
+#ifdef AB_STAMP
+  if (tl) tl[7] = __builtin_amdgcn_s_memrealtime();
+#endif
+  {
+    const bf16_t* Kb = p.k + b * p.k_sb + hk * p.k_sh;
+    const bf16_t* Vb = p.v + b * p.v_sb + hk * p.v_sh;
+    const unsigned kvoffK = dma_lane_offset0<HD>(HD, tid), kvoffV = dma_lane_offset0<HD>(p.v_ss, tid);
+#pragma unroll
+    for (int t = 0; t < 2; ++t) {
+      stage_rows_dma_asm<HD>(Kb, HD, kt_ * 128 + 64 * t, p.S, lds0 + 2 * BUFB + t * TILE, kvoffK, wave);
+      stage_rows_dma_asm<HD>(Vb, p.v_ss, kt_ * 128 + 64 * t, p.S, lds0 + 3 * BUFB + t * TILE, kvoffV, wave);
+    }
+    sfor<0, 128>([&](auto i) { agpr_write<decltype(i)::value>(0u); });
+    asm volatile("s_waitcnt vmcnt(0)" ::: "memory", A3V_AGPR_0_255);
+    __syncthreads();
+    prescale_lse(lds);
+    const char* Kt = lds + 2 * BUFB + (wave >> 1) * TILE;
+    const char* Vt = lds + 3 * BUFB + (wave >> 1) * TILE;
+    sfor<0, NKS>([&](auto ks_) {
+      constexpr int ks = decltype(ks_)::value;
+      const bf16x8 kq = frag_rows<HD>(Kt, fbase, wave & 1, ks), vq = frag_rows<HD>(Vt, fbase, wave & 1, ks);
+      u32x4 ku, vu;
+      __builtin_memcpy(&ku, &kq, 16);
+      __builtin_memcpy(&vu, &vq, 16);
+      sfor<0, 4>([&](auto j) {
+        agpr_write<RKF + 4 * ks + decltype(j)::value>(ku[decltype(j)::value]);
+        agpr_write<RVF + 4 * ks + decltype(j)::value>(vu[decltype(j)::value]);
+      });
+    });
+    __syncthreads();
+  }
+  AB_PE(1);
+  AB_PE(2);
+  issue(total > 1);
+  AB_PE(3);
+  fetch(lds, 0);
+  prep_issue(total > 2);
+  sfor<0, NKS>([&](auto ks_) {
+    constexpr int ks = decltype(ks_)::value;
+    mfma_va<RS, RKF + 4 * ks, ks == 0>(qa[ks]);
+    piece(ks_);
+    mfma_va_v<RVF + 4 * ks, ks == 0>(dpv[0], da[ks]);
+  });
+  piece(std::integral_constant<int, PP>{});
+  asm volatile("s_nop 15\n\ts_nop 15" ::: "memory", A3V_AGPR_0_255);
+  fetch(lds, 1);
+  AB_PE(4);
+  int qi_c = 0, buf_c = 0;
+  uint64_t ds_head = 0;
+  int ds_stores = 0;
+  if constexpr (EMIT_DS)
+    ds_head = (uint64_t)dsa.ws + (uint64_t)((int64_t)b * p.H + hk * nrep) * dsa.head_bytes + (uint64_t)(kt_ * 2 + (wave >> 1)) * 16384 + (wave & 1) * 2048;
+#ifdef AB_STAMP
+  if (tl) tl[1] = __builtin_amdgcn_s_memrealtime();
+#endif
+  for (int it = 0; it < total; ++it) {
+    const int q0 = (q_begin + qi_c) * 64;
+    if constexpr (EMIT_DS) ds_unit = ds_head + (uint64_t)(q0 >> 7) * dsa.qt_bytes + ((q0 >> 6) & 1) * 8192;
+    if (++qi_c == n_it) {
+      qi_c = 0;
+      if constexpr (EMIT_DS) ds_head += dsa.head_bytes;
+    }
+    const int q0x = (q_begin + qi_c) * 64;
+    const char* cb = lds + buf_c * BUFB;
+    if (++buf_c == NB) buf_c = 0;
+    const char* xb = lds + buf_c * BUFB;
+    const bool more = it + 1 < total;
+#ifdef AB_STAMP
+    cur_it = it;
+#endif
+    AB_ST(1, it, 0);
+    if constexpr (EMIT_DS) {
+      if (ds_stores == 4) asm volatile("s_waitcnt vmcnt(13)" ::: "memory", A3V_AGPR_0_255);
+      else if (ds_stores == 2) asm volatile("s_waitcnt vmcnt(11)" ::: "memory", A3V_AGPR_0_255);
+      else asm volatile("s_waitcnt vmcnt(9)" ::: "memory", A3V_AGPR_0_255);
+    } else if constexpr (PP == 8) asm volatile("s_waitcnt vmcnt(9)" ::: "memory", A3V_AGPR_0_255); else asm volatile("s_waitcnt vmcnt(5)" ::: "memory", A3V_AGPR_0_255);
+    AB_ST(1, it, 1);
+    __syncthreads();
+    AB_ST(1, it, 2);
+    prep_issue(it + 3 < total);
+    if (more) prescale_lse(xb);
+    AB_ST(1, it, 3);
+    const bool l0 = !dead(q0), l1 = !dead(q0 + 32), lx = more && !dead(q0x);
+    if constexpr (EMIT_DS) ds_stores = 2 * ((int)l0 + (int)l1);
+    run(l0, l1, !interior(q0), std::integral_constant<int, 0>{}, cb, q0, xb, 0);
+    AB_ST(1, it, 4);
+    run(l1, lx, !interior(q0 + 32), std::integral_constant<int, 1>{}, cb, q0 + 32, xb, 1);
+    AB_ST(1, it, 5);
+  }
+#ifdef AB_STAMP
+  if (tl) tl[2] = __builtin_amdgcn_s_memrealtime();
+#endif
+  asm volatile("s_nop 15\n\ts_nop 15" ::: "memory", A3V_AGPR_0_255);
+  AB_PE(5);
+  const float* CS = PACKED ? p.cos_sin + (int64_t)(p.rope_pos0 + kc) * HD : nullptr;
+  f32x4 cs[NDB][4];
+  if constexpr (PACKED) {
+#pragma unroll
+    for (int d = 0; d < NDB; ++d)
+#pragma unroll
+      for (int g4 = 0; g4 < 4; ++g4) cs[d][g4] = *reinterpret_cast<const f32x4*>(CS + d * 32 + g4 * 8 + hh * 4);
+  }
+  __syncthreads();
+  AB_PE(6);
+  char* patchV = lds + wave * (32 * HD * 2);
+  char* patchK = lds + 4 * (32 * HD * 2) + wave * (32 * HD * 2);
+  const int wx = (kl & (HD / 8 - 1)) << 1;
+  sfor<0, NDB>([&](auto d_) {
+    constexpr int d = decltype(d_)::value;
+    const f32x16 av = agpr_read16<RV + 16 * d>();
+#pragma unroll
+    for (int g4 = 0; g4 < 4; ++g4) {
+      bf16x4 ov;
+#pragma unroll
+      for (int e = 0; e < 4; ++e) ov[e] = f2bf(av[g4 * 4 + e]);
+      *reinterpret_cast<bf16x4*>(patchV + kl * (HD * 2) + (((d * 8 + g4 * 2 + hh) ^ wx) << 3)) = ov;
+    }
+  });
+  bf16_t* baseV = PACKED ? p.dqkv + (int64_t)b * p.S * p.ld_qkv + (int64_t)(p.H + p.Hkv + hk) * HD : p.dv + ((int64_t)b * p.Hkv + hk) * p.S * HD;
+  bf16_t* baseK = PACKED ? p.dqkv + (int64_t)b * p.S * p.ld_qkv + (int64_t)(p.H + hk) * HD : p.dk + ((int64_t)b * p.Hkv + hk) * p.S * HD;
+  const int64_t ldo = PACKED ? p.ld_qkv : HD;
+  store_patch_rows<HD>(patchV, baseV, ldo, kv_lo, p.S, lane);
+  AB_PE(7);
+  sfor<0, NDB>([&](auto d_) {
+    constexpr int d = decltype(d_)::value;
+    f32x16 ak = agpr_read16<RK + 16 * d>();
+#pragma unroll
+    for (int r = 0; r < 16; ++r) ak[r] *= p.scale;
+#pragma unroll
+    for (int g4 = 0; g4 < 4; ++g4) {
+      float v0 = ak[g4 * 4 + 0], v1 = ak[g4 * 4 + 1], v2 = ak[g4 * 4 + 2], v3 = ak[g4 * 4 + 3];
+      bf16x4 ok;
+      if constexpr (PACKED) {
+        const f32x4 c4 = cs[d][g4];
+        ok[0] = f2bf(v0 * c4[0] + v1 * c4[1]); ok[1] = f2bf(-v0 * c4[1] + v1 * c4[0]);
+        ok[2] = f2bf(v2 * c4[2] + v3 * c4[3]); ok[3] = f2bf(-v2 * c4[3] + v3 * c4[2]);
+      } else {
+        ok[0] = f2bf(v0); ok[1] = f2bf(v1); ok[2] = f2bf(v2); ok[3] = f2bf(v3);
+      }
+      *reinterpret_cast<bf16x4*>(patchK + kl * (HD * 2) + (((d * 8 + g4 * 2 + hh) ^ wx) << 3)) = ok;
+    }
+  });
+  store_patch_rows<HD>(patchK, baseK, ldo, kv_lo, p.S, lane);
+  AB_PE(8);
+#ifdef AB_STAMP
+  if (tl) { asm volatile("s_waitcnt vmcnt(0)" ::: "memory"); tl[3] = __builtin_amdgcn_s_memrealtime(); }
+#endif
diff --git a/a3vlm_amd/csrc/a3v_train.hip b/a3vlm_amd/csrc/a3v_train.hip
--- a/a3vlm_amd/csrc/a3v_train.hip
+++ b/a3vlm_amd/csrc/a3v_train.hip
@@ -877,13 +877,13 @@
 
 extern "C" __attribute__((visibility("hidden"))) int a3v_attention_bwd_mfma_packed(const void* q, const void* k, int64_t k_sb, int64_t k_sh, const void* v, int64_t v_sb,
                                              int64_t v_ss, int64_t v_sh, const void* dout, const float* lse, const float* D, void* dqkv,
-                                             int64_t ld_qkv, const float* cos_sin, int rope_pos0, int B, int S, int H, int Hkv, int hd,
+                                             int64_t ld_qkv, const float* cos_sin, int rope_pos0, void* workspace, int B, int S, int H, int Hkv, int hd,
                                              int causal, void* stream);
 
-extern "C" int a3v_attention_bwd_packed(const void* q, const void* k, int64_t k_sb, int64_t k_sh, const void* v, int64_t v_sb, int64_t v_ss,
+extern "C" int a3v_attention_bwd_packed_ws(const void* q, const void* k, int64_t k_sb, int64_t k_sh, const void* v, int64_t v_sb, int64_t v_ss,
                                         int64_t v_sh, const void* out, int64_t ld_out, const void* dout, const float* lse, float* D, void* dqkv,
                                         int64_t ld_qkv, const float* cos_sin, int rope_pos0, int B, int S, int H, int Hkv, int hd, int causal,
-                                        int dtype, void* stream) {
+                                        int dtype, void* workspace, void* stream) {
   if (!q || !k || !v || !out || !dout || !lse || !D || !dqkv || !cos_sin || B <= 0 || S <= 0) return A3V_ERR_ARG;
   if (dtype != A3V_BF16) return A3V_ERR_DTYPE;
   if ((hd != 64 && hd != 128) || (H % Hkv) || ld_out < (int64_t)H * hd || ld_out % 8) return A3V_ERR_SHAPE;
@@ -894,8 +894,16 @@
   else
     hipLaunchKernelGGL(attn_rowdot_vec_kernel<64>, dim3((unsigned)((rows + 31) / 32)), dim3(256), 0, ST, (const bf16_t*)out, (const bf16_t*)dout, D, rows, H, ld_out);
   A3V_LAUNCH_CHECK();
-  return a3v_attention_bwd_mfma_packed(q, k, k_sb, k_sh, v, v_sb, v_ss, v_sh, dout, lse, D, dqkv, ld_qkv, cos_sin, rope_pos0, B, S, H, Hkv, hd, causal,
+  return a3v_attention_bwd_mfma_packed(q, k, k_sb, k_sh, v, v_sb, v_ss, v_sh, dout, lse, D, dqkv, ld_qkv, cos_sin, rope_pos0, workspace, B, S, H, Hkv, hd, causal,
                                        stream);
+}
+
+extern "C" int a3v_attention_bwd_packed(const void* q, const void* k, int64_t k_sb, int64_t k_sh, const void* v, int64_t v_sb, int64_t v_ss,
+                                        int64_t v_sh, const void* out, int64_t ld_out, const void* dout, const float* lse, float* D, void* dqkv,
+                                        int64_t ld_qkv, const float* cos_sin, int rope_pos0, int B, int S, int H, int Hkv, int hd, int causal,
+                                        int dtype, void* stream) {
+  return a3v_attention_bwd_packed_ws(q, k, k_sb, k_sh, v, v_sb, v_ss, v_sh, out, ld_out, dout, lse, D, dqkv, ld_qkv, cos_sin, rope_pos0, B, S, H, Hkv, hd,
+                                     causal, dtype, nullptr, stream);
 }
 
 extern "C" int a3v_embed_bwd(const int64_t* tokens, int64_t ld_tok, const float* dh, float* dtable, int B, int T, int W, int dim,
diff --git a/a3vlm_amd/lib.py b/a3vlm_amd/lib.py
--- a/a3vlm_amd/lib.py
+++ b/a3vlm_amd/lib.py
@@ -26,6 +26,7 @@
     "a3v_quantize_rows_fp8": (I, [P, L, P, F, P, L, P, I, I, I, P]),
     "a3v_gemm_tn_splitk": (I, [P, L, P, L, P, I, I, I, I, P]),
     "a3v_attention_bwd_packed": (I, [P, P, L, L, P, L, L, L, P, L, P, P, P, P, L, P, I, I, I, I, I, I, I, I, P]),
+    "a3v_attention_bwd_packed_ws": (I, [P, P, L, L, P, L, L, L, P, L, P, P, P, P, L, P, I, I, I, I, I, I, I, I, P, P]),
     "a3v_lora_refresh": (I, [P, P, I, I, I, P, L, P, L, P, L, P, L, I, I, P]),
     "a3v_adamw": (I, [P, P, P, P, L, F, F, F, F, F, L, P, P]),
     "a3v_adamw_scaled": (I, [P, P, P, P, L, F, F, F, F, F, L, P, P, P]),
diff --git a/a3vlm_amd/ops.py b/a3vlm_amd/ops.py
--- a/a3vlm_amd/ops.py
+++ b/a3vlm_amd/ops.py
@@ -527,22 +527,29 @@
     return _l.load().a3v_attention_bwd_workspace_bytes(B, S, H, Hkv, hd)
 
 
+def _check_attn_bwd_ws(workspace, B, S, H, Hkv, hd) -> None:
+    if workspace is not None and workspace.numel() * workspace.element_size() < attention_bwd_workspace_bytes(B, S, H, Hkv, hd):
+        raise ValueError("attention backward workspace too small (a3v_attention_bwd_workspace_bytes)")
+
+
 def attention_bwd(q, k, k_sb, k_sh, v, v_sb, v_ss, v_sh, out, dout, lse, D, dq, dk, dv, B, S, H, Hkv, hd, causal: bool,
                   workspace=None):
     _dev(q, k, v, out, dout, lse, D, dq, dk, dv, workspace)
+    _check_attn_bwd_ws(workspace, B, S, H, Hkv, hd)
     rc = _l.load().a3v_attention_bwd(_p(q), _p(k), k_sb, k_sh, _p(v), v_sb, v_ss, v_sh, _p(out), _p(dout), _p(lse), _p(D),
                                      _p(dq), _p(dk), _p(dv), _p(workspace), B, S, H, Hkv, hd, 1 if causal else 0, dt(q), _stream())
     _l.check(rc, "a3v_attention_bwd")
 
 
 def attention_bwd_packed(q, k, k_sb, k_sh, v, v_sb, v_ss, v_sh, out, dout, lse, D, dqkv, cos_sin, B, S, H, Hkv, hd, causal: bool,
-                         rope_pos0: int = 0):
-    _dev(q, k, v, out, dout, lse, D, dqkv, cos_sin)
+                         rope_pos0: int = 0, workspace=None):
+    _dev(q, k, v, out, dout, lse, D, dqkv, cos_sin, workspace)
+    _check_attn_bwd_ws(workspace, B, S, H, Hkv, hd)
     ld_out = out.stride(-2) if out.dim() == 2 else out.stride(1)
-    rc = _l.load().a3v_attention_bwd_packed(_p(q), _p(k), k_sb, k_sh, _p(v), v_sb, v_ss, v_sh, _p(out), ld_out, _p(dout), _p(lse), _p(D),
-                                            _p(dqkv), dqkv.stride(0), _p(cos_sin), rope_pos0, B, S, H, Hkv, hd, 1 if causal else 0,
-                                            dt(q), _stream())
-    _l.check(rc, "a3v_attention_bwd_packed")
+    rc = _l.load().a3v_attention_bwd_packed_ws(_p(q), _p(k), k_sb, k_sh, _p(v), v_sb, v_ss, v_sh, _p(out), ld_out, _p(dout), _p(lse), _p(D),
+                                               _p(dqkv), dqkv.stride(0), _p(cos_sin), rope_pos0, B, S, H, Hkv, hd, 1 if causal else 0,
+                                               dt(q), _p(workspace), _stream())
+    _l.check(rc, "a3v_attention_bwd_packed_ws")
 
 
 def embed_bwd(tokens, dh, dtable, B, T, W, dim):
diff --git a/a3vlm_amd/train.py b/a3vlm_amd/train.py
--- a/a3vlm_amd/train.py
+++ b/a3vlm_amd/train.py
@@ -738,8 +738,9 @@
         else:
             dqkv = self._buf("dqkv", (rows, (H + 2 * Hkv) * hd))
         if self.act == torch.bfloat16 and hd in (64, 128) and self.packed_attn_bwd:
+            wsp = self._buf("attn_bwd_ws", (ops.attention_bwd_workspace_bytes(B, S, H, Hkv, hd),), torch.uint8)
             ops.attention_bwd_packed(k["qrot"], k["kc"], Hkv * spad * hd, spad * hd, vrows, S * ld, ld, hd, k["att"], datt, k["lse"], D,
-                                     dqkv, m._cos_sin_dev(), B, S, H, Hkv, hd, True, 0)
+                                     dqkv, m._cos_sin_dev(), B, S, H, Hkv, hd, True, 0, workspace=wsp)
         else:
             dq = self._buf("dq", (rows, H * hd))
             dk = self._buf("dk", (B, Hkv, S, hd))
@@ -1135,7 +1136,7 @@
 
 def hbm_budget(dim: int, n_layers: int, n_heads: int, ffn: int, vocab: int, batch: int, seq: int, text: int, n_kv_heads: Optional[int] = None,
                vit_params: int = 304_000_000, proj_in: int = 1024, world: int = 1, wire_bytes: int = 2, recompute: bool = False,
-               stream_bytes: int = 2, zero1: bool = False, transposed_images: bool = False) -> Dict[str, int]:
+               stream_bytes: int = 2, zero1: bool = False, transposed_images: bool = False, attn_bwd_ds: bool = False) -> Dict[str, int]:
     hkv = n_kv_heads or n_heads
     hd = dim // n_heads
     qkv = (n_heads + 2 * hkv) * hd
@@ -1147,6 +1148,9 @@
     sb = stream_bytes
     block = rows * (2 * dim * 2 + qkv * 2 + 2 * n_heads * hd * 2 + 3 * ffn * 2 + dim * sb) + batch * hkv * spad * hd * 2 + batch * n_heads * seq * 4
     bwd_ws = rows * ((dim * 2 if sb == 4 else 0) + ffn * 2 + 2 * ffn * 2 + dim * 2 + n_heads * hd * 2 + qkv * 2 + dim * sb) + batch * hkv * hd * spad * 2
+    if attn_bwd_ds and hd == 128:
+        nqt = (seq + 127) // 128
+        bwd_ws += batch * n_heads * nqt * 2 * nqt * 16384
     if zero1:
         p_big = p_mat + dim * vocab
         p_small = p_train - p_big
diff --git a/include/a3vlm_hip.h b/include/a3vlm_hip.h
--- a/include/a3vlm_hip.h
+++ b/include/a3vlm_hip.h
@@ -217,6 +217,10 @@
                              int64_t v_ss, int64_t v_sh, const void* out, int64_t ld_out, const void* dout, const float* lse, float* D,
                              void* dqkv, int64_t ld_qkv, const float* cos_sin, int rope_pos0, int B, int S, int H, int Hkv,
                              int hd, int causal, int dtype, void* stream);
+int a3v_attention_bwd_packed_ws(const void* q, const void* k, int64_t k_sb, int64_t k_sh, const void* v, int64_t v_sb,
+                                int64_t v_ss, int64_t v_sh, const void* out, int64_t ld_out, const void* dout, const float* lse, float* D,
+                                void* dqkv, int64_t ld_qkv, const float* cos_sin, int rope_pos0, int B, int S, int H, int Hkv,
+                                int hd, int causal, int dtype, void* workspace, void* stream);
 int64_t a3v_attention_bwd_workspace_bytes(int B, int S, int H, int Hkv, int hd);
 int a3v_attention_bwd_mfma(const void* q, const void* k, int64_t k_sb, int64_t k_sh, const void* v,
                            int64_t v_sb, int64_t v_ss, int64_t v_sh, const void* dout, const float* lse,
```

New measurement: 35.43 (median of 2 runs). No clear change (+0.1%).
